# acg-team/ProGraphMSA

Measured on AMD Instinct MI355X. Metric: DP cell-updates/sec (GCUPS) + wall-clock on 256 seqs × 1000 aa, WAG, higher is better.
Workload: dtype f32

## Files before the change

include/pgm_hip.h:

```cpp
#ifndef PGM_HIP_H_
#define PGM_HIP_H_

#include <stdint.h>
#include <stddef.h>

#ifdef __cplusplus
extern "C" {
#endif

#define PGM_OK 0
#define PGM_ERR_INVALID 1
#define PGM_ERR_DEVICE 2
#define PGM_ERR_BACKTRACK 3
#define PGM_ERR_NOMEM 4

#define PGM_GAP 0xFFFFFFFFu


typedef struct pgm_graph {
    uint32_t n;
    uint32_t dim;
    const double *sites;
    const int32_t *e_rowptr;
    const uint32_t *e_col;
    const float *e_val;
    const int32_t *r_rowptr;
    const uint32_t *r_col;
    const uint32_t *r_units;
} pgm_graph;

typedef struct pgm_model {
    const double *M;
    const double *pi;
} pgm_model;

typedef struct pgm_scores {
    float gap_init, gap_extend, match_init, end_match, end_gap, end_skip;
    float start_gap, start_init, repeat_init, repeat_ext;
} pgm_scores;

typedef struct pgm_align_out {
    float score;
    uint32_t n_tr_indels;
    uint32_t len;
    int32_t status;
    uint32_t *map1;
    uint32_t *map2;
} pgm_align_out;

typedef struct pgm_ctx pgm_ctx;
typedef struct pgm_align_batch pgm_align_batch;

int pgm_device_count(void);
int pgm_ctx_create(int device, pgm_ctx **out);
void pgm_ctx_destroy(pgm_ctx *ctx);
const char *pgm_last_error(void);
int pgm_ctx_device_info(pgm_ctx *ctx, char *name, size_t name_len, int *cu_count);

int pgm_align_graphs_batch(pgm_ctx *ctx, uint32_t njobs, const pgm_graph *const *g1,
                           const pgm_graph *const *g2, const pgm_model *const *model,
                           const pgm_scores *scores, pgm_align_out *out);

int pgm_align_batch_create(pgm_ctx *ctx, uint32_t njobs, const pgm_graph *const *g1,
                           const pgm_graph *const *g2, const pgm_model *const *model,
                           const pgm_scores *scores, pgm_align_batch **out);
#define PGM_BATCH_KEEP_MATRICES 1u
int pgm_align_batch_create_ex(pgm_ctx *ctx, uint32_t njobs, const pgm_graph *const *g1,
                              const pgm_graph *const *g2, const pgm_model *const *model,
                              const pgm_scores *scores, uint32_t flags, pgm_align_batch **out);
typedef struct pgm_site_ref {
    const double *dev_sites;
    const uint32_t *node_map;
    uint32_t ncols;
} pgm_site_ref;
int pgm_align_batch_create_res(pgm_ctx *ctx, uint32_t njobs, const pgm_graph *const *g1,
                               const pgm_graph *const *g2, const pgm_model *const *model,
                               const pgm_scores *scores, uint32_t flags, const pgm_site_ref *res1,
                               const pgm_site_ref *res2, pgm_align_batch **out);
int pgm_align_graphs_batch_res(pgm_ctx *ctx, uint32_t njobs, const pgm_graph *const *g1,
                               const pgm_graph *const *g2, const pgm_model *const *model,
                               const pgm_scores *scores, const pgm_site_ref *res1,
                               const pgm_site_ref *res2, pgm_align_out *out);
int pgm_align_batch_run(pgm_ctx *ctx, pgm_align_batch *b);
int pgm_align_batch_fetch(pgm_ctx *ctx, pgm_align_batch *b, pgm_align_out *out);
void pgm_align_batch_destroy(pgm_ctx *ctx, pgm_align_batch *b);
uint64_t pgm_align_batch_cells(const pgm_align_batch *b);
int pgm_align_batch_time(pgm_ctx *ctx, pgm_align_batch *b, int reps, float *ms_prep,
                         float *ms_emission, float *ms_fill, float *ms_traceback);
int pgm_align_batch_stage_times(pgm_align_batch *b, int reset, float *ms_prep, float *ms_emission, float *ms_fill,
                                uint32_t *launches);
int pgm_align_batch_job_times(pgm_ctx *ctx, pgm_align_batch *b, uint64_t *ticks);
int pgm_align_batch_test_stall(pgm_align_batch *b, uint32_t job, uint32_t band, uint32_t spin_limit);
int pgm_test_cu_shares(uint32_t cus, double lean_cost, uint32_t nlean, double band_cost, uint32_t nbands, double rest_cost,
                       uint32_t nrest, uint32_t ncrit, double longest_chain, uint32_t *out4);
#define PGM_PLAN_HEAD 23
#define PGM_PLAN_DHEAD 9
#define PGM_PLAN_JOB 19
int pgm_test_batch_plan(uint32_t njobs, const pgm_graph *const *g1, const pgm_graph *const *g2, const pgm_model *const *model,
                        const pgm_scores *scores, uint32_t flags, const pgm_site_ref *res1, const pgm_site_ref *res2, uint32_t cus,
                        uint32_t *head, double *dhead, uint32_t *job_fields, uint32_t *items, uint32_t *bands, uint32_t *lean_list, int32_t *tblist);
int pgm_align_batch_read_matrices(pgm_ctx *ctx, pgm_align_batch *b, uint32_t job, float *M,
                                  float *X, float *Y, float *W, float *S);

int pgm_nw_pairs_batch(pgm_ctx *ctx, uint32_t dim, const int32_t *score, int32_t gap_open,
                       int32_t gap_extend, uint32_t nseq, const int8_t *syms,
                       const uint32_t *offs, uint32_t npairs, const uint32_t *pi,
                       const uint32_t *pj, int32_t *counts, uint32_t *gaps);
#define PGM_NW_REDUCED 1u
int pgm_nw_pairs_submit(pgm_ctx *ctx, uint32_t dim, const int32_t *score, int32_t gap_open,
                        int32_t gap_extend, uint32_t nseq, const int8_t *syms,
                        const uint32_t *offs, uint32_t npairs, const uint32_t *pi,
                        const uint32_t *pj, uint32_t flags, int32_t *counts, uint32_t *gaps, int *ticket);
int pgm_nw_pairs_wait(pgm_ctx *ctx, int ticket);
float pgm_nw_last_kernel_ms(pgm_ctx *ctx);
void *pgm_host_alloc(size_t bytes);
void pgm_host_free(void *p);

int pgm_csprofile_load(pgm_ctx *ctx, uint32_t K, uint32_t ncols, const double *lprofiles,
                       const double *centre, const double *priors);
int pgm_csprofile_create_batch(pgm_ctx *ctx, uint32_t nseq, const int8_t *syms,
                               const uint32_t *offs, const double *tau, const double *pi,
                               const double *p_uniform, double *out, const uint64_t *out_offs);
int pgm_csprofile_create_batch_res(pgm_ctx *ctx, uint32_t nseq, const int8_t *syms,
                                   const uint32_t *offs, const double *tau, const double *pi,
                                   const double *p_uniform, const double **dev);
float pgm_csprofile_last_kernel_ms(pgm_ctx *ctx);

typedef struct pgm_mldist_model {
    uint32_t dim;
    const double *Q, *V, *Vi, *sigma;
    double dist_max, var_max, var_min, cutoff_dist, min_dist, max_dist, indel_rate;
    int32_t mldist, mldist_gap;
} pgm_mldist_model;
int pgm_mldist_batch(pgm_ctx *ctx, const pgm_mldist_model *model, uint32_t npairs, const int32_t *counts,
                     const uint32_t *gaps, const double *seqlen, double *dist, double *var);

int pgm_prealigned_counts_batch(pgm_ctx *ctx, uint32_t dim, uint32_t nrows, uint32_t ncols, const int8_t *rows,
                                uint32_t npairs, const uint32_t *pi, const uint32_t *pj, int32_t *counts,
                                uint32_t *gaps);
int pgm_kmer_cosine(pgm_ctx *ctx, uint32_t nseq, uint32_t ncols, const int32_t *counts, double *cosine);
int pgm_kmer_cosine_multi(pgm_ctx *ctx, uint32_t nfam, const uint32_t *nseq, uint32_t ncols, const int32_t *counts, double *cosine);
int pgm_prealigned_counts_multi(pgm_ctx *ctx, uint32_t dim, uint32_t nfam, const uint32_t *nrows, const uint32_t *ncols,
                                const int8_t *rows, uint32_t npairs, const uint32_t *fam, const uint32_t *pi, const uint32_t *pj,
                                int32_t *counts, uint32_t *gaps);
int pgm_prealigned_counts_resampled(pgm_ctx *ctx, uint32_t dim, uint32_t nrows, uint32_t ncols, const int8_t *rows, uint32_t nrep,
                                    const uint32_t *cols, uint32_t npairs, const uint32_t *pi, const uint32_t *pj, int32_t *counts,
                                    uint32_t *gaps);
float pgm_dist_last_kernel_ms(pgm_ctx *ctx);

typedef struct pgm_merge_job {
    uint32_t dim, n1, n2, nnodes;
    const double *sites1, *sites2;
    const double *P1, *P2;
    const uint32_t *k1, *k2;
    const uint8_t *g2_with_P1;
    double *profiles;
} pgm_merge_job;
int pgm_merge_profiles_batch(pgm_ctx *ctx, uint32_t njobs, const pgm_merge_job *jobs);
#define PGM_MERGE_RESIDENT 1u
int pgm_merge_profiles_batch_ex(pgm_ctx *ctx, uint32_t njobs, const pgm_merge_job *jobs, uint32_t flags,
                                const double **dev_profiles);
int pgm_resident_reset(pgm_ctx *ctx);
int pgm_resident_onehot(pgm_ctx *ctx, uint32_t dim, uint32_t nseq, const int8_t *syms, const uint32_t *offs,
                        const double **dev);
int pgm_resident_import(pgm_ctx *ctx, pgm_ctx *src_ctx, const double *src, uint64_t count, const double **dst);
float pgm_merge_last_kernel_ms(pgm_ctx *ctx);


typedef struct pgm_gapmask_job {
    const uint64_t *src;
    const uint32_t *mapping;
    uint64_t *dst;
    uint32_t nrows, ncols_in, ncols_out;
} pgm_gapmask_job;
int pgm_gapmask_extend_batch(pgm_ctx *ctx, uint32_t njobs, const pgm_gapmask_job *jobs);

typedef struct pgm_parsimony_job {
    const uint64_t *masks;
    const uint32_t *children;
    uint32_t nleaves, ncols;
} pgm_parsimony_job;
int pgm_gap_parsimony_batch(pgm_ctx *ctx, uint32_t njobs, const pgm_parsimony_job *jobs, uint32_t *scores);
float pgm_parsimony_last_kernel_ms(pgm_ctx *ctx);

#define PGM_WLS_MAX_N 32768
int pgm_wls_load(pgm_ctx *ctx, uint32_t n, const double *D, const double *W);

#define PGM_WLS_OUT 20
typedef struct pgm_wls_job {
    const int8_t *label;
    const double *offset;
    uint32_t nsub;
} pgm_wls_job;
int pgm_wls_pair_sums_batch(pgm_ctx *ctx, uint32_t njobs, const pgm_wls_job *jobs, double *out);
float pgm_wls_last_kernel_ms(pgm_ctx *ctx);
uint32_t pgm_wls_last_launches(pgm_ctx *ctx);

typedef struct pgm_bionj_join { uint32_t index1, index2; double dist1, dist2; } pgm_bionj_join;
#define PGM_BIONJ_MAX_N 32768
int pgm_bionj(pgm_ctx *ctx, uint32_t n, const double *D, const double *V, pgm_bionj_join *joins, double *final_d);
int pgm_bionj_multi(pgm_ctx *ctx, uint32_t nfam, const uint32_t *n, const double *D, const double *V,
                    pgm_bionj_join *joins, double *final_d);
uint32_t pgm_bionj_last_launches(pgm_ctx *ctx);
float pgm_bionj_last_kernel_ms(pgm_ctx *ctx);

typedef struct pgm_bionj_pair { uint32_t index1, index2; } pgm_bionj_pair;
int pgm_bionj_plan(pgm_ctx *ctx, uint32_t n, const double *D, const double *V, const pgm_bionj_pair *plan,
                   pgm_bionj_join *joins, double *final_d);
int pgm_bionj_plan_multi(pgm_ctx *ctx, uint32_t nfam, const uint32_t *n, const double *D, const double *V,
                         const pgm_bionj_pair *plan, pgm_bionj_join *joins, double *final_d);

int pgm_msa_agreement(pgm_ctx *ctx, uint32_t nrows, uint32_t ncols, uint32_t nrep, const int32_t *where,
                      uint32_t *res_hits , uint32_t *pair_hits );
float pgm_agreement_last_kernel_ms(pgm_ctx *ctx);

int pgm_transfer_min(pgm_ctx *ctx, uint32_t nleaves, uint32_t nref, const uint64_t *ref ,
                     uint32_t nrep, const uint32_t *rep_off ,
                     const uint64_t *rep , uint32_t *phi );
float pgm_transfer_last_kernel_ms(pgm_ctx *ctx);

#define PGM_TRANSFER_NONE 0xffffffffu
int pgm_transfer_taxa(pgm_ctx *ctx, uint32_t nleaves, uint32_t nref, const uint64_t *ref , const uint32_t *thr ,
                      uint32_t nrep, const uint32_t *rep_off , const uint64_t *rep ,
                      uint32_t *phi , uint32_t *arg , uint32_t *moved ,
                      uint32_t *counted );

#ifdef __cplusplus
}
#endif
#endif
```

prographmsa_amd/__init__.py:

```python
import ctypes as C
import os

_HERE = os.path.dirname(os.path.abspath(__file__))
LIB_PATH = os.path.join(_HERE, "lib", "libpgm_hip.so")
PGMSA_PATH = os.path.join(_HERE, "bin", "pgmsa")

PGM_OK, PGM_ERR_INVALID, PGM_ERR_DEVICE, PGM_ERR_BACKTRACK, PGM_ERR_NOMEM = 0, 1, 2, 3, 4
PGM_GAP = 0xFFFFFFFF
PGM_BATCH_KEEP_MATRICES = 1
PGM_NW_REDUCED = 1
PGM_MERGE_RESIDENT = 1


class pgm_graph(C.Structure):
    _fields_ = [("n", C.c_uint32), ("dim", C.c_uint32), ("sites", C.POINTER(C.c_double)),
                ("e_rowptr", C.POINTER(C.c_int32)), ("e_col", C.POINTER(C.c_uint32)), ("e_val", C.POINTER(C.c_float)),
                ("r_rowptr", C.POINTER(C.c_int32)), ("r_col", C.POINTER(C.c_uint32)), ("r_units", C.POINTER(C.c_uint32))]


class pgm_model(C.Structure):
    _fields_ = [("M", C.POINTER(C.c_double)), ("pi", C.POINTER(C.c_double))]


class pgm_scores(C.Structure):
    _fields_ = [(n, C.c_float) for n in ("gap_init", "gap_extend", "match_init", "end_match", "end_gap", "end_skip",
                                         "start_gap", "start_init", "repeat_init", "repeat_ext")]


class pgm_mldist_model(C.Structure):
    _fields_ = [("dim", C.c_uint32), ("Q", C.POINTER(C.c_double)), ("V", C.POINTER(C.c_double)), ("Vi", C.POINTER(C.c_double)),
                ("sigma", C.POINTER(C.c_double))] + [(n, C.c_double) for n in ("dist_max", "var_max", "var_min", "cutoff_dist", "min_dist", "max_dist", "indel_rate")] \
        + [("mldist", C.c_int32), ("mldist_gap", C.c_int32)]


class pgm_merge_job(C.Structure):
    _fields_ = [("dim", C.c_uint32), ("n1", C.c_uint32), ("n2", C.c_uint32), ("nnodes", C.c_uint32),
                ("sites1", C.POINTER(C.c_double)), ("sites2", C.POINTER(C.c_double)), ("P1", C.POINTER(C.c_double)), ("P2", C.POINTER(C.c_double)),
                ("k1", C.POINTER(C.c_uint32)), ("k2", C.POINTER(C.c_uint32)), ("g2_with_P1", C.POINTER(C.c_uint8)), ("profiles", C.POINTER(C.c_double))]


class pgm_site_ref(C.Structure):
    _fields_ = [("dev_sites", C.POINTER(C.c_double)), ("node_map", C.POINTER(C.c_uint32)), ("ncols", C.c_uint32)]


class pgm_gapmask_job(C.Structure):
    _fields_ = [("src", C.POINTER(C.c_uint64)), ("mapping", C.POINTER(C.c_uint32)), ("dst", C.POINTER(C.c_uint64)),
                ("nrows", C.c_uint32), ("ncols_in", C.c_uint32), ("ncols_out", C.c_uint32)]


class pgm_parsimony_job(C.Structure):
    _fields_ = [("masks", C.POINTER(C.c_uint64)), ("children", C.POINTER(C.c_uint32)), ("nleaves", C.c_uint32), ("ncols", C.c_uint32)]


class pgm_wls_job(C.Structure):
    _fields_ = [("label", C.POINTER(C.c_int8)), ("offset", C.POINTER(C.c_double)), ("nsub", C.c_uint32)]


class pgm_bionj_join(C.Structure):
    _fields_ = [("index1", C.c_uint32), ("index2", C.c_uint32), ("dist1", C.c_double), ("dist2", C.c_double)]


class pgm_bionj_pair(C.Structure):
    _fields_ = [("index1", C.c_uint32), ("index2", C.c_uint32)]


class pgm_align_out(C.Structure):
    _fields_ = [("score", C.c_float), ("n_tr_indels", C.c_uint32), ("len", C.c_uint32), ("status", C.c_int32),
                ("map1", C.POINTER(C.c_uint32)), ("map2", C.POINTER(C.c_uint32))]


EXPORTS = [
    "pgm_device_count", "pgm_ctx_create", "pgm_ctx_destroy", "pgm_last_error", "pgm_ctx_device_info",
    "pgm_align_graphs_batch", "pgm_align_batch_create", "pgm_align_batch_create_ex", "pgm_align_batch_create_res", "pgm_align_graphs_batch_res", "pgm_align_batch_run", "pgm_align_batch_fetch",
    "pgm_align_batch_destroy", "pgm_align_batch_cells", "pgm_align_batch_test_stall", "pgm_test_cu_shares", "pgm_test_batch_plan", "pgm_align_batch_stage_times", "pgm_align_batch_job_times", "pgm_align_batch_time", "pgm_align_batch_read_matrices",
    "pgm_nw_pairs_batch", "pgm_nw_pairs_submit", "pgm_nw_pairs_wait", "pgm_nw_last_kernel_ms", "pgm_host_alloc", "pgm_host_free", "pgm_csprofile_load", "pgm_csprofile_create_batch", "pgm_csprofile_create_batch_res",
    "pgm_csprofile_last_kernel_ms", "pgm_mldist_batch", "pgm_prealigned_counts_batch", "pgm_kmer_cosine", "pgm_dist_last_kernel_ms",
    "pgm_kmer_cosine_multi", "pgm_prealigned_counts_multi", "pgm_prealigned_counts_resampled",
    "pgm_merge_profiles_batch", "pgm_merge_profiles_batch_ex", "pgm_resident_reset", "pgm_resident_onehot", "pgm_resident_import", "pgm_merge_last_kernel_ms",
    "pgm_gapmask_extend_batch", "pgm_gap_parsimony_batch", "pgm_parsimony_last_kernel_ms",
    "pgm_wls_load", "pgm_wls_pair_sums_batch", "pgm_wls_last_kernel_ms", "pgm_wls_last_launches",
    "pgm_bionj", "pgm_bionj_multi", "pgm_bionj_last_launches", "pgm_bionj_last_kernel_ms",
    "pgm_bionj_plan", "pgm_bionj_plan_multi",
    "pgm_msa_agreement", "pgm_agreement_last_kernel_ms",
    "pgm_transfer_min", "pgm_transfer_last_kernel_ms", "pgm_transfer_taxa",
]


def _load():
    if not os.path.exists(LIB_PATH):
        raise ImportError("libpgm_hip.so is not built (%s); run `python -c 'import __graft_entry__ as g; g.build()'` "
                          "— there is no CPU fallback for the hot path" % LIB_PATH)
    lib = C.CDLL(LIB_PATH)
    vp, u32, i32 = C.c_void_p, C.c_uint32, C.c_int32
    PG, PM = C.POINTER(C.POINTER(pgm_graph)), C.POINTER(C.POINTER(pgm_model))
    sig = {
        "pgm_device_count": (C.c_int, []),
        "pgm_ctx_create": (C.c_int, [C.c_int, C.POINTER(vp)]),
        "pgm_ctx_destroy": (None, [vp]),
        "pgm_last_error": (C.c_char_p, []),
        "pgm_ctx_device_info": (C.c_int, [vp, C.c_char_p, C.c_size_t, C.POINTER(C.c_int)]),
        "pgm_align_graphs_batch": (C.c_int, [vp, u32, PG, PG, PM, C.POINTER(pgm_scores), C.POINTER(pgm_align_out)]),
        "pgm_align_batch_create": (C.c_int, [vp, u32, PG, PG, PM, C.POINTER(pgm_scores), C.POINTER(vp)]),
        "pgm_align_batch_create_ex": (C.c_int, [vp, u32, PG, PG, PM, C.POINTER(pgm_scores), u32, C.POINTER(vp)]),
        "pgm_align_batch_create_res": (C.c_int, [vp, u32, PG, PG, PM, C.POINTER(pgm_scores), u32, C.POINTER(pgm_site_ref), C.POINTER(pgm_site_ref), C.POINTER(vp)]),
        "pgm_align_graphs_batch_res": (C.c_int, [vp, u32, PG, PG, PM, C.POINTER(pgm_scores), C.POINTER(pgm_site_ref), C.POINTER(pgm_site_ref), C.POINTER(pgm_align_out)]),
        "pgm_align_batch_run": (C.c_int, [vp, vp]),
        "pgm_align_batch_fetch": (C.c_int, [vp, vp, C.POINTER(pgm_align_out)]),
        "pgm_align_batch_destroy": (None, [vp, vp]),
        "pgm_align_batch_cells": (C.c_uint64, [vp]),
        "pgm_align_batch_test_stall": (C.c_int, [vp, u32, u32, u32]),
        "pgm_test_cu_shares": (C.c_int, [u32, C.c_double, u32, C.c_double, u32, C.c_double, u32, u32, C.c_double, C.POINTER(C.c_uint32)]),
        "pgm_test_batch_plan": (C.c_int, [u32, PG, PG, PM, C.POINTER(pgm_scores), u32, C.POINTER(pgm_site_ref), C.POINTER(pgm_site_ref), u32,
                                          C.POINTER(u32), C.POINTER(C.c_double)] + [C.POINTER(u32)] * 4 + [C.POINTER(i32)]),
        "pgm_align_batch_stage_times": (C.c_int, [vp, C.c_int] + [C.POINTER(C.c_float)] * 3 + [C.POINTER(u32)]),
        "pgm_align_batch_job_times": (C.c_int, [vp, vp, C.POINTER(C.c_uint64)]),
        "pgm_align_batch_time": (C.c_int, [vp, vp, C.c_int] + [C.POINTER(C.c_float)] * 4),
        "pgm_align_batch_read_matrices": (C.c_int, [vp, vp, u32] + [C.POINTER(C.c_float)] * 5),
        "pgm_nw_pairs_batch": (C.c_int, [vp, u32, C.POINTER(i32), i32, i32, u32, C.POINTER(C.c_int8), C.POINTER(u32), u32,
                                         C.POINTER(u32), C.POINTER(u32), C.POINTER(i32), C.POINTER(u32)]),
        "pgm_nw_pairs_submit": (C.c_int, [vp, u32, C.POINTER(i32), i32, i32, u32, C.POINTER(C.c_int8), C.POINTER(u32), u32,
                                          C.POINTER(u32), C.POINTER(u32), u32, C.POINTER(i32), C.POINTER(u32), C.POINTER(C.c_int)]),
        "pgm_nw_pairs_wait": (C.c_int, [vp, C.c_int]),
        "pgm_host_alloc": (vp, [C.c_size_t]),
        "pgm_host_free": (None, [vp]),
        "pgm_nw_last_kernel_ms": (C.c_float, [vp]),
        "pgm_csprofile_load": (C.c_int, [vp, u32, u32] + [C.POINTER(C.c_double)] * 3),
        "pgm_csprofile_create_batch": (C.c_int, [vp, u32, C.POINTER(C.c_int8), C.POINTER(u32)] + [C.POINTER(C.c_double)] * 4
                                       + [C.POINTER(C.c_uint64)]),
        "pgm_csprofile_create_batch_res": (C.c_int, [vp, u32, C.POINTER(C.c_int8), C.POINTER(u32)] + [C.POINTER(C.c_double)] * 3
                                           + [C.POINTER(C.POINTER(C.c_double))]),
        "pgm_csprofile_last_kernel_ms": (C.c_float, [vp]),
        "pgm_mldist_batch": (C.c_int, [vp, C.POINTER(pgm_mldist_model), u32, C.POINTER(i32), C.POINTER(u32)] + [C.POINTER(C.c_double)] * 3),
        "pgm_prealigned_counts_batch": (C.c_int, [vp, u32, u32, u32, C.POINTER(C.c_int8), u32, C.POINTER(u32), C.POINTER(u32), C.POINTER(i32), C.POINTER(u32)]),
        "pgm_kmer_cosine": (C.c_int, [vp, u32, u32, C.POINTER(i32), C.POINTER(C.c_double)]),
        "pgm_dist_last_kernel_ms": (C.c_float, [vp]),
        "pgm_kmer_cosine_multi": (C.c_int, [vp, u32, C.POINTER(u32), u32, C.POINTER(i32), C.POINTER(C.c_double)]),
        "pgm_prealigned_counts_multi": (C.c_int, [vp, u32, u32, C.POINTER(u32), C.POINTER(u32), C.POINTER(C.c_int8), u32, C.POINTER(u32), C.POINTER(u32),
                                                  C.POINTER(u32), C.POINTER(i32), C.POINTER(u32)]),
        "pgm_prealigned_counts_resampled": (C.c_int, [vp, u32, u32, u32, C.POINTER(C.c_int8), u32, C.POINTER(u32), u32, C.POINTER(u32), C.POINTER(u32),
                                                      C.POINTER(i32), C.POINTER(u32)]),
        "pgm_merge_profiles_batch": (C.c_int, [vp, u32, C.POINTER(pgm_merge_job)]),
        "pgm_merge_profiles_batch_ex": (C.c_int, [vp, u32, C.POINTER(pgm_merge_job), u32, C.POINTER(C.POINTER(C.c_double))]),
        "pgm_resident_reset": (C.c_int, [vp]),
        "pgm_resident_onehot": (C.c_int, [vp, u32, u32, C.POINTER(C.c_int8), C.POINTER(u32), C.POINTER(C.POINTER(C.c_double))]),
        "pgm_resident_import": (C.c_int, [vp, vp, C.POINTER(C.c_double), C.c_uint64, C.POINTER(C.POINTER(C.c_double))]),
        "pgm_merge_last_kernel_ms": (C.c_float, [vp]),
        "pgm_gapmask_extend_batch": (C.c_int, [vp, u32, C.POINTER(pgm_gapmask_job)]),
        "pgm_gap_parsimony_batch": (C.c_int, [vp, u32, C.POINTER(pgm_parsimony_job), C.POINTER(u32)]),
        "pgm_parsimony_last_kernel_ms": (C.c_float, [vp]),
        "pgm_wls_load": (C.c_int, [vp, u32, C.POINTER(C.c_double), C.POINTER(C.c_double)]),
        "pgm_wls_pair_sums_batch": (C.c_int, [vp, u32, C.POINTER(pgm_wls_job), C.POINTER(C.c_double)]),
        "pgm_wls_last_kernel_ms": (C.c_float, [vp]),
        "pgm_wls_last_launches": (C.c_uint32, [vp]),
        "pgm_bionj": (C.c_int, [vp, u32, C.POINTER(C.c_double), C.POINTER(C.c_double), C.POINTER(pgm_bionj_join), C.POINTER(C.c_double)]),
        "pgm_bionj_multi": (C.c_int, [vp, u32, C.POINTER(u32), C.POINTER(C.c_double), C.POINTER(C.c_double), C.POINTER(pgm_bionj_join), C.POINTER(C.c_double)]),
        "pgm_bionj_last_launches": (C.c_uint32, [vp]),
        "pgm_bionj_last_kernel_ms": (C.c_float, [vp]),
        "pgm_bionj_plan": (C.c_int, [vp, u32, C.POINTER(C.c_double), C.POINTER(C.c_double), C.POINTER(pgm_bionj_pair), C.POINTER(pgm_bionj_join), C.POINTER(C.c_double)]),
        "pgm_bionj_plan_multi": (C.c_int, [vp, u32, C.POINTER(u32), C.POINTER(C.c_double), C.POINTER(C.c_double), C.POINTER(pgm_bionj_pair), C.POINTER(pgm_bionj_join), C.POINTER(C.c_double)]),
        "pgm_msa_agreement": (C.c_int, [vp, u32, u32, u32, C.POINTER(i32), C.POINTER(u32), C.POINTER(u32)]),
        "pgm_agreement_last_kernel_ms": (C.c_float, [vp]),
        "pgm_transfer_min": (C.c_int, [vp, u32, u32, C.POINTER(C.c_uint64), u32, C.POINTER(u32), C.POINTER(C.c_uint64), C.POINTER(u32)]),
        "pgm_transfer_last_kernel_ms": (C.c_float, [vp]),
        "pgm_transfer_taxa": (C.c_int, [vp, u32, u32, C.POINTER(C.c_uint64), C.POINTER(u32), u32, C.POINTER(u32), C.POINTER(C.c_uint64),
                                        C.POINTER(u32), C.POINTER(u32), C.POINTER(u32), C.POINTER(u32)]),
    }
    for name, (res, args) in sig.items():
        fn = getattr(lib, name)
        fn.restype = res
        fn.argtypes = args
    return lib


lib = _load()


class PgmError(RuntimeError):
    pass


def check(rc, what="libpgm_hip"):
    if rc != PGM_OK:
        raise PgmError("%s failed (%d): %s" % (what, rc, lib.pgm_last_error().decode()))


class Context:

    def __init__(self, device=0):
        self.handle = C.c_void_p()
        check(lib.pgm_ctx_create(device, C.byref(self.handle)), "pgm_ctx_create")

    def device_info(self):
        buf = C.create_string_buffer(256)
        cu = C.c_int()
        check(lib.pgm_ctx_device_info(self.handle, buf, 256, C.byref(cu)))
        return buf.value.decode(), cu.value

    def prealigned_counts_resampled(self, dim, rows, cols, pi, pj):
        import numpy as np
        rows = np.ascontiguousarray(rows, np.int8)
        cols = np.ascontiguousarray(cols, np.uint32)
        pi = np.ascontiguousarray(pi, np.uint32)
        pj = np.ascontiguousarray(pj, np.uint32)
        nrep, npairs = cols.shape[0], len(pi)
        counts = np.zeros((nrep, npairs, dim * dim), np.int32)
        gaps = np.zeros((nrep, npairs), np.uint32)
        P = lambda a, t: a.ctypes.data_as(C.POINTER(t))
        check(lib.pgm_prealigned_counts_resampled(self.handle, dim, rows.shape[0], rows.shape[1], P(rows, C.c_int8), nrep, P(cols, C.c_uint32), npairs,
                                                  P(pi, C.c_uint32), P(pj, C.c_uint32), P(counts, C.c_int32), P(gaps, C.c_uint32)), "pgm_prealigned_counts_resampled")
        return counts, gaps

    def msa_agreement(self, where, res_hits=None, pair_hits=None):
        import numpy as np
        where = np.ascontiguousarray(where, np.int32)
        nrep, nrows, ncols = where.shape
        if res_hits is None: res_hits = np.zeros((nrows, ncols), np.uint32)
        if pair_hits is None: pair_hits = np.zeros((nrows, nrows), np.uint32)
        for o, shape in ((res_hits, (nrows, ncols)), (pair_hits, (nrows, nrows))):
            if o.dtype != np.uint32 or o.shape != shape or not o.flags.c_contiguous: raise ValueError("msa_agreement: output array of the wrong kind")
        P = lambda a, t: a.ctypes.data_as(C.POINTER(t))
        check(lib.pgm_msa_agreement(self.handle, nrows, ncols, nrep, P(where, C.c_int32), P(res_hits, C.c_uint32), P(pair_hits, C.c_uint32)), "pgm_msa_agreement")
        return res_hits, pair_hits

    def transfer_min(self, nleaves, ref, rep_off, rep, phi=None):
        import numpy as np
        words = (nleaves + 63) // 64
        ref = np.ascontiguousarray(ref, np.uint64)
        rep_off = np.ascontiguousarray(rep_off, np.uint32)
        rep = np.ascontiguousarray(rep, np.uint64).reshape(-1, words)
        if ref.ndim != 2 or ref.shape[1] != words or rep_off.ndim != 1 or len(rep_off) < 1 or rep.shape[0] != int(rep_off[-1]):
            raise ValueError("transfer_min: input array of the wrong shape")
        nref, nrep = ref.shape[0], len(rep_off) - 1
        if phi is None: phi = np.zeros((nref, nrep), np.uint32)
        if phi.dtype != np.uint32 or phi.shape != (nref, nrep) or not phi.flags.c_contiguous: raise ValueError("transfer_min: output array of the wrong kind")
        P = lambda a, t: a.ctypes.data_as(C.POINTER(t))
        check(lib.pgm_transfer_min(self.handle, nleaves, nref, P(ref, C.c_uint64), nrep, P(rep_off, C.c_uint32), P(rep, C.c_uint64) if rep.size else None,
                                   P(phi, C.c_uint32)), "pgm_transfer_min")
        return phi

    def transfer_taxa(self, nleaves, ref, thr, rep_off, rep, out=None):
        import numpy as np
        words = (nleaves + 63) // 64
        ref = np.ascontiguousarray(ref, np.uint64)
        thr = np.ascontiguousarray(thr, np.uint32)
        rep_off = np.ascontiguousarray(rep_off, np.uint32)
        rep = np.ascontiguousarray(rep, np.uint64).reshape(-1, words)
        if ref.ndim != 2 or ref.shape[1] != words or thr.shape != (ref.shape[0],) or rep_off.ndim != 1 or len(rep_off) < 1 or rep.shape[0] != int(rep_off[-1]):
            raise ValueError("transfer_taxa: input array of the wrong shape")
        nref, nrep = ref.shape[0], len(rep_off) - 1
        shapes = [(nref, nrep), (nref, nrep), (nref, nleaves), (nref,)]
        if out is None: out = tuple(np.zeros(s, np.uint32) for s in shapes)
        if len(out) != 4 or any(a.dtype != np.uint32 or a.shape != s or not a.flags.c_contiguous for a, s in zip(out, shapes)):
            raise ValueError("transfer_taxa: output array of the wrong kind")
        P = lambda a, t: a.ctypes.data_as(C.POINTER(t))
        check(lib.pgm_transfer_taxa(self.handle, nleaves, nref, P(ref, C.c_uint64), P(thr, C.c_uint32), nrep, P(rep_off, C.c_uint32),
                                    P(rep, C.c_uint64) if rep.size else None, *[P(a, C.c_uint32) for a in out]), "pgm_transfer_taxa")
        return tuple(out)

    def close(self):
        if self.handle:
            lib.pgm_ctx_destroy(self.handle)
            self.handle = C.c_void_p()

    def __del__(self):
        try:
            self.close()
        except Exception:
            pass
```

prographmsa_amd/csrc/pgm_align_kernels.h:

```cpp
#ifndef PGM_ALIGN_KERNELS_H_
#define PGM_ALIGN_KERNELS_H_

#include <hip/hip_runtime.h>
#include <math.h>
#include <type_traits>
#include "pgm_device.h"

#define PGM_NEG_INF (-INFINITY)

__device__ __forceinline__ float pgm_ls_log_add(float x, float add) {
    const float a = 2.44247459618085927548717403238913328776812604856113966238617812902399112761292613763080658235564f;
    const float b = -4.2040783745848554315883301529007786406310628696382695994938550046831869207082846248658671f;
    const float c = -0.72123729809042963774358701619456664388406302428056983119308906451199556380646306f;
    const uint32_t bits = __float_as_uint(x);
    const float e = (float)((int32_t)(bits >> 23) - 126);
    const float d = __uint_as_float(((bits << 9) >> 9) ^ 0x3f000000u);
    float t = __fdiv_rn(b, __fsub_rn(d, c));
    const float u = __fadd_rn(e, a);
    t = __fadd_rn(t, add);
    t = __fadd_rn(t, u);
    return t;
}

__device__ __forceinline__ float pgm_emission_finish(float num, float ay, float bx, float match_init) {
    float q = __fdiv_rn(num, __fmul_rn(ay, bx));
    if (q != q) q = __uint_as_float(0xFFC00000u);
    return pgm_ls_log_add(q, match_init);
}

template <int DMAX, int NODES>
__global__ void __launch_bounds__(NODES) pgm_prep_kernel(const PgmJob *__restrict__ jobs, int *__restrict__ sync, uint32_t sync_ints) {
    extern __shared__ float prep_lds[];
    {
        const uint32_t nthreads = gridDim.x * gridDim.y * gridDim.z * NODES;
        const uint32_t gid = ((blockIdx.z * gridDim.y + blockIdx.y) * gridDim.x + blockIdx.x) * NODES + threadIdx.x;
        for (uint32_t i = gid; i < sync_ints; i += nthreads) sync[i] = 0;
    }
    const PgmJob &J = jobs[blockIdx.x];
    const bool first = blockIdx.y == 0;
    const uint32_t n = first ? J.n1 : J.n2;
    const uint32_t v0 = blockIdx.z * NODES;
    if (v0 >= n) return;
    if (J.tabhdr && J.tabhdr[0] == 0) {
        const uint32_t nc = J.dim + 2u;
        bool any = n - 1u >= v0 && n - 1u < v0 + (uint32_t)NODES;
        for (uint32_t c = 0; c < nc; ++c) {
            const uint32_t r = (uint32_t)J.tabhdr[1u + (first ? 0u : nc) + c];
            any = any || (r != 0u && r - 1u >= v0 && r - 1u < v0 + (uint32_t)NODES);
        }
        if (!any) return;
    }
    const uint32_t D = J.dim, DP = J.dp, ST = D + 1;
    float *Mf = prep_lds;
    float *pif = prep_lds + D * D;
    float *nl = pif + D;
    const uint32_t nn = min((uint32_t)NODES, n - v0);
    {
        const int32_t *pp = first ? J.pp1 : J.pp2;
        const uint32_t *pc = first ? J.pc1 : J.pc2, *pu = first ? J.pu1 : J.pu2;
        const float *pv = first ? J.pv1 : J.pv2;
        PgmTbNode *rec = (first ? J.tb1 : J.tb2) + v0;
        for (uint32_t i = threadIdx.x; i < nn * PGM_TB_PK; i += NODES) {
            const uint32_t node = i / PGM_TB_PK, k = i % PGM_TB_PK;
            const int32_t eb = pp[v0 + node];
            const uint32_t cnt = (uint32_t)(pp[v0 + node + 1] - eb);
            const int32_t e = cnt == 0u ? 0 : eb + (int32_t)min(k, cnt - 1u);
            if (k == 0) rec[node].cnt = cnt;
            rec[node].c[k] = pc[e]; rec[node].v[k] = pv[e]; rec[node].u[k] = pu[e];
        }
    }
    if (!first) for (uint32_t i = threadIdx.x; i < D * D; i += NODES) Mf[i] = (float)J.M[i];
    for (uint32_t i = threadIdx.x; i < D; i += NODES) pif[i] = (float)J.pi[i];
    const double *sites = first ? J.sites1 : J.sites2;
    const uint32_t *smap = first ? J.smap1 : J.smap2;
    float *dst = (first ? J.g1f : J.t2) + (size_t)DP * v0;
    for (uint32_t i = threadIdx.x; i < nn * D; i += NODES) {
        const uint32_t node = v0 + i / D;
        const float g = (float)sites[(size_t)D * (smap ? smap[node] : node) + i % D];
        nl[(i / D) * ST + (i % D)] = g;
        if (first && DP == D) dst[i] = g;
    }
    __syncthreads();
    const uint32_t v = threadIdx.x;
    float g[DMAX];
    float acc = 0.0f;
    if (v < nn) {
#pragma unroll
        for (int k = 0; k < DMAX; ++k) g[k] = ((uint32_t)k < D) ? nl[v * ST + k] : 0.0f;
        float l0 = 0.0f, l1 = 0.0f, l2 = 0.0f, l3 = 0.0f;
        const uint32_t aligned = D / 4u * 4u;
#pragma unroll
        for (int k = 0; k + 3 < DMAX; k += 4) {
            if ((uint32_t)k < aligned) {
                l0 = __fadd_rn(l0, __fmul_rn(g[k], pif[k]));
                l1 = __fadd_rn(l1, __fmul_rn(g[k + 1], pif[k + 1]));
                l2 = __fadd_rn(l2, __fmul_rn(g[k + 2], pif[k + 2]));
                l3 = __fadd_rn(l3, __fmul_rn(g[k + 3], pif[k + 3]));
            }
        }
        acc = __fadd_rn(0.0f, __fadd_rn(__fadd_rn(l0, l2), __fadd_rn(l1, l3)));
#pragma unroll
        for (int k = 0; k < DMAX; ++k)
            if ((uint32_t)k >= aligned && (uint32_t)k < D) acc = __fadd_rn(acc, __fmul_rn(g[k], pif[k]));
        (first ? J.a1 : J.b2)[v0 + v] = acc;
    }
    if (first) {
        if (DP != D && v < nn) {
#pragma unroll
            for (int k = 0; k < DMAX; ++k) if ((uint32_t)k < DP) dst[(size_t)DP * v + k] = g[k];
        }
        return;
    }
    __syncthreads();
    if (v < nn) {
        for (uint32_t k = 0; k < D; ++k) {
            float t = 0.0f;
#pragma unroll
            for (int j = 0; j < DMAX; ++j)
                if ((uint32_t)j < D) t = __fadd_rn(t, __fmul_rn(Mf[j + D * k], g[j]));
            nl[v * ST + k] = t;
        }
    }
    __syncthreads();
    for (uint32_t i = threadIdx.x; i < nn * DP; i += NODES) {
        const uint32_t node = i / DP, k = i % DP;
        dst[i] = k < D ? nl[node * ST + k] : 0.0f;
    }
}

#define PGM_TAB_HDR 136
__global__ void __launch_bounds__(256) pgm_classify_kernel(const PgmJob *__restrict__ jobs) {
    const PgmJob &J = jobs[blockIdx.x];
    if (!J.tabhdr) return;
    const bool first = blockIdx.y == 0;
    const uint32_t n = first ? J.n1 : J.n2, D = J.dim;
    const double *sites = first ? J.sites1 : J.sites2;
    const uint32_t *smap = first ? J.smap1 : J.smap2;
    uint8_t *cls = (uint8_t *)(first ? J.cls1 : J.cls2);
    const float uni = (float)(1.0 / (double)D);
    for (uint32_t v = blockIdx.z * blockDim.x + threadIdx.x; v < n; v += gridDim.z * blockDim.x) {
        const double *col = sites + (size_t)D * (smap ? smap[v] : v);
        uint32_t nz = 0, sym = 0;
        bool same = true;
        float vs = 0.f;
        const float g0 = (float)col[0];
        for (uint32_t k = 0; k < D; ++k) {
            const float g = (float)col[k];
            if (g != 0.0f) { ++nz; sym = k; vs = g; }
            same = same && g == g0;
        }
        uint32_t c = 255u;
        if (nz == 0u) c = D + 1u;
        else if (nz == 1u && vs == 1.0f) c = sym;
        else if (same && g0 == uni) c = D;
        cls[v] = (uint8_t)c;
        if (c == 255u) atomicOr(J.tabhdr, 1);
        else atomicCAS(J.tabhdr + 1 + (first ? 0u : D + 2u) + c, 0, (int)v + 1);
    }
}

__device__ __forceinline__ size_t pgm_cell_index(const PgmJob &J, uint32_t y, uint32_t x) {
    const uint32_t b = y / PGM_ROWS, l = PGM_HALO + (y - b * PGM_ROWS);
    return ((size_t)b * J.tsteps + (x + l)) * 64u + l;
}
__device__ __forceinline__ float4 pgm_load_cell(const PgmJob &J, uint32_t y, uint32_t x) {
    return J.cells[pgm_cell_index(J, y, x)];
}

__device__ __forceinline__ float pgm_dpp_wave_shr1(float src, float lane0_value) {
    return __int_as_float(__builtin_amdgcn_update_dpp(__float_as_int(lane0_value), __float_as_int(src), 0x138, 0xf, 0xf, false));
}

#define PGM_GLOBAL __attribute__((address_space(1)))
typedef float pgm_v4f __attribute__((ext_vector_type(4)));
template <class T> __device__ __forceinline__ T pgm_gld(const T *p) { return *(const PGM_GLOBAL T *)(uintptr_t)p; }
#define PGM_EM_TB 4
template <int DP, int RB>
__global__ void __launch_bounds__(4 * PGM_ROWS) pgm_emission_skew_kernel(const PgmJob *__restrict__ jobs) {
    typedef float pgm_v2f __attribute__((ext_vector_type(2)));
    constexpr int NT = DP / 4;
    constexpr int COLS = 64 + PGM_EM_TB * PGM_BLOCK - PGM_HALO - 1;
    constexpr int STR = DP + 1;
    __shared__ pgm_v2f tp[(COLS + 1) * STR];
    __shared__ float bq[COLS];
    const PgmJob &J = jobs[blockIdx.z];
    const uint32_t tb0 = blockIdx.x * PGM_EM_TB;
    const uint32_t rsh = J.rshift, nvb = J.nb << rsh;
    if (tb0 >= J.nblk || 4u * RB * blockIdx.y >= nvb) return;
    if (J.tabhdr && pgm_gld(J.tabhdr) == 0) return;
    auto row_of = [&](uint32_t v, uint32_t lane_) { return ((((v >> rsh) << 6) + lane_) << rsh) | (v & ((1u << rsh) - 1u)); };
    auto sblock_of = [&](uint32_t v, uint32_t tb_) { return ((((size_t)(v >> rsh) * J.nblk + tb_) << rsh) | (v & ((1u << rsh) - 1u))); };
    const uint32_t t0 = tb0 * PGM_BLOCK;
    const int cbase = (int)t0 - 63;
    if ((DP == 20 || DP == 4) && RB == 1) {
        constexpr int TE = DP + 1;
        float *const tab = (float *)tp;
        static_assert(COLS * TE <= (COLS + 1) * STR * 2, "score table must fit the column staging area");
        static_assert(DP > 20 || TE <= 32, "row classes must fit As");
        __shared__ float As[32];
        const uint32_t fb0 = 4u * blockIdx.y + threadIdx.x / PGM_ROWS;
        const uint32_t fl = threadIdx.x % PGM_ROWS;
        const bool active = fb0 < nvb;
        int sym = DP;
        bool plain = true;
        float a_row = 0.f;
        if (active) {
            const uint32_t y = row_of(fb0, fl);
            const uint32_t yc = (y + 1 < J.n1) ? y : 0u;
            const float4 *src = (const float4 *)(J.g1f + (size_t)DP * yc);
            int nz = 0;
#pragma unroll
            for (int q = 0; q < NT; ++q) {
                const float4 v = src[q];
                const float vv[4] = {v.x, v.y, v.z, v.w};
#pragma unroll
                for (int u = 0; u < 4; ++u)
                    if (vv[u] != 0.0f) { ++nz; sym = 4 * q + u; plain = plain && vv[u] == 1.0f; }
            }
            plain = plain && nz <= 1;
            a_row = J.a1[yc];
        }
        if (threadIdx.x < 32) As[threadIdx.x] = 0.f;
        if (__syncthreads_and(plain ? 1 : 0)) {
            if (active) As[sym] = a_row;
            __syncthreads();
            const float mi = J.sc.match_init;
            constexpr int NE = (COLS * TE + 4 * PGM_ROWS - 1) / (4 * PGM_ROWS);
            float tt[NE], tb2[NE];
#pragma unroll
            for (int e = 0; e < NE; ++e) {
                const int i = (int)threadIdx.x + e * 4 * PGM_ROWS;
                const int ci = i / TE, k = i % TE, c = cbase + ci;
                const bool in = i < COLS * TE && c >= 0 && c <= (int)J.ncol;
                tb2[e] = in ? J.b2[c] : 0.f;
                tt[e] = (in && k < DP) ? J.t2[(size_t)DP * c + k] : 0.f;
            }
#pragma unroll
            for (int e = 0; e < NE; ++e) {
                const int i = (int)threadIdx.x + e * 4 * PGM_ROWS;
                if (i < COLS * TE) tab[i] = pgm_emission_finish(0.0f + tt[e], As[i % TE], tb2[e], mi);
            }
            __syncthreads();
            if (!active) return;
            PGM_GLOBAL pgm_v4f *const Sq = (PGM_GLOBAL pgm_v4f *)(uintptr_t)J.S;
            const int l = PGM_HALO + (int)fl;
#pragma unroll 1
            for (int w = 0; w < PGM_EM_TB; ++w) {
                const uint32_t tb = tb0 + w;
                if (tb >= J.nblk) break;
                float out[PGM_BLOCK];
#pragma unroll
                for (int i = 0; i < PGM_BLOCK; ++i) out[i] = tab[((int)(tb * PGM_BLOCK) + i - l - cbase) * TE + sym];
                PGM_GLOBAL pgm_v4f *dst = Sq + (sblock_of(fb0, tb) * 64u + (uint32_t)l) * (PGM_BLOCK / 4);
#pragma unroll
                for (int q = 0; q < PGM_BLOCK / 4; ++q) dst[q] = pgm_v4f{out[4 * q], out[4 * q + 1], out[4 * q + 2], out[4 * q + 3]};
            }
            return;
        }
    }
    const float4 *t2q = (const float4 *)J.t2;
    float *tpf = (float *)tp;
    for (int i = threadIdx.x; i < (COLS + 1) * NT; i += 4 * PGM_ROWS) {
        const int ci = i / NT, q = i % NT, c = cbase + ci;
        float4 v = make_float4(0.f, 0.f, 0.f, 0.f);
        if (c >= 0 && c <= (int)J.ncol) v = t2q[(size_t)NT * c + q];
        const float vv[4] = {v.x, v.y, v.z, v.w};
#pragma unroll
        for (int u = 0; u < 4; ++u) {
            const int k = 4 * q + u;
            if (ci < COLS) tpf[2 * (ci * STR + k)] = vv[u];
            if (ci > 0) tpf[2 * ((ci - 1) * STR + k) + 1] = vv[u];
        }
    }
    for (int i = threadIdx.x; i < COLS; i += 4 * PGM_ROWS) {
        const int col = cbase + i;
        bq[i] = (col >= 0 && col <= (int)J.ncol) ? J.b2[col] : 0.f;
    }
    __syncthreads();
    const uint32_t b0 = (4u * blockIdx.y + threadIdx.x / PGM_ROWS) * RB;
    const int l = PGM_HALO + (int)(threadIdx.x % PGM_ROWS);
    if (b0 >= nvb) return;
    float gy[RB][DP], ay[RB];
#pragma unroll
    for (int r = 0; r < RB; ++r) {
        const uint32_t y = row_of(b0 + (uint32_t)r, (uint32_t)(l - PGM_HALO));
        const uint32_t yc = (y + 1 < J.n1) ? y : 0u;
        const float4 *src = (const float4 *)(J.g1f + (size_t)DP * yc);
#pragma unroll
        for (int q = 0; q < NT; ++q) {
            const float4 v = src[q];
            gy[r][4 * q] = v.x; gy[r][4 * q + 1] = v.y; gy[r][4 * q + 2] = v.z; gy[r][4 * q + 3] = v.w;
        }
        ay[r] = J.a1[yc];
    }
    const float mi = J.sc.match_init;
    const uint32_t nblk = J.nblk;
    PGM_GLOBAL pgm_v4f *const Sq = (PGM_GLOBAL pgm_v4f *)(uintptr_t)J.S;
#pragma unroll 1
    for (int w = 0; w < PGM_EM_TB; ++w) {
        const uint32_t tb = tb0 + w;
        if (tb >= nblk) break;
        float out[RB][PGM_BLOCK];
#pragma unroll
        for (int i = 0; i < PGM_BLOCK; i += 2) {
            const int ci = (int)(tb * PGM_BLOCK) + i - l - cbase;
            const pgm_v2f *tc = tp + ci * STR;
            pgm_v2f acc[RB];
#pragma unroll
            for (int r = 0; r < RB; ++r) acc[r] = pgm_v2f{0.0f, 0.0f};
#pragma unroll
            for (int k = 0; k < DP; ++k) {
                const pgm_v2f tk = tc[k];
#pragma unroll
                for (int r = 0; r < RB; ++r) {
                    const pgm_v2f g = {gy[r][k], gy[r][k]};
                    acc[r] = acc[r] + g * tk;
                }
            }
#pragma unroll
            for (int r = 0; r < RB; ++r) {
                out[r][i] = pgm_emission_finish(acc[r].x, ay[r], bq[ci], mi);
                out[r][i + 1] = pgm_emission_finish(acc[r].y, ay[r], bq[ci + 1], mi);
            }
        }
#pragma unroll
        for (int r = 0; r < RB; ++r) {
            if (b0 + (uint32_t)r < nvb) {
                PGM_GLOBAL pgm_v4f *dst = Sq + (sblock_of(b0 + (uint32_t)r, tb) * 64u + (uint32_t)l) * (PGM_BLOCK / 4);
#pragma unroll
                for (int q = 0; q < PGM_BLOCK / 4; ++q) dst[q] = pgm_v4f{out[r][4 * q], out[r][4 * q + 1], out[r][4 * q + 2], out[r][4 * q + 3]};
            }
        }
    }
}

__device__ __forceinline__ int pgm_wave_max8(uint32_t v) {
    int m = __builtin_amdgcn_ballot_w64(v >= 8u) != 0 ? 8 : 0;
    m += __builtin_amdgcn_ballot_w64(v >= (uint32_t)(m + 4)) != 0 ? 4 : 0;
    m += __builtin_amdgcn_ballot_w64(v >= (uint32_t)(m + 2)) != 0 ? 2 : 0;
    m += __builtin_amdgcn_ballot_w64(v >= (uint32_t)(m + 1)) != 0 ? 1 : 0;
    return m;
}

__device__ __forceinline__ __amdgpu_buffer_rsrc_t pgm_band_rsrc(float4 *base, uint32_t bytes) {
    const uint64_t p = (uint64_t)base;
    const uint32_t lo = __builtin_amdgcn_readfirstlane((uint32_t)p), hi = __builtin_amdgcn_readfirstlane((uint32_t)(p >> 32));
    return __builtin_amdgcn_make_buffer_rsrc((void *)(((uint64_t)hi << 32) | lo), 0, __builtin_amdgcn_readfirstlane(bytes), 0x00020000);
}
__device__ __forceinline__ void pgm_store_cell_masked(__amdgpu_buffer_rsrc_t rsrc, uint32_t t, int lane, bool on, float Mv, float Xv, float Wv, float Yv) {
    typedef uint32_t pgm_v4u __attribute__((ext_vector_type(4)));
    pgm_v4u v;
    v.x = __float_as_uint(Mv); v.y = __float_as_uint(Xv); v.z = __float_as_uint(Wv); v.w = __float_as_uint(Yv);
    __builtin_amdgcn_raw_buffer_store_b128(v, rsrc, (on ? (uint32_t)lane * 16u : 0x80000000u) + t * 1024u, 0, 16);
}
__device__ __forceinline__ float4 pgm_gload4(const float4 *p) {
    const pgm_v4f v = *(const PGM_GLOBAL pgm_v4f *)(uintptr_t)p;
    return make_float4(v.x, v.y, v.z, v.w);
}
__device__ __forceinline__ float2 pgm_gload_cell_wy(const float4 *p) {
    const unsigned long long v = __hip_atomic_load((const PGM_GLOBAL unsigned long long *)(uintptr_t)p + 1, __ATOMIC_RELAXED, __HIP_MEMORY_SCOPE_AGENT);
    return make_float2(__uint_as_float((uint32_t)v), __uint_as_float((uint32_t)(v >> 32)));
}
__device__ __forceinline__ float2 pgm_load_cell_mx(const float4 *p) {
    const unsigned long long v = __hip_atomic_load((const PGM_GLOBAL unsigned long long *)(uintptr_t)p, __ATOMIC_RELAXED, __HIP_MEMORY_SCOPE_AGENT);
    return make_float2(__uint_as_float((uint32_t)v), __uint_as_float((uint32_t)(v >> 32)));
}
__device__ __forceinline__ float2 pgm_load_cell_wy(const float4 *p) {
    const unsigned long long v = __hip_atomic_load((const PGM_GLOBAL unsigned long long *)(uintptr_t)p + 1, __ATOMIC_RELAXED, __HIP_MEMORY_SCOPE_AGENT);
    return make_float2(__uint_as_float((uint32_t)v), __uint_as_float((uint32_t)(v >> 32)));
}

struct PgmPred {
    const int32_t *pp; const uint32_t *pc; const float *pv; const uint32_t *pu;
};
__device__ __forceinline__ float pgm_mark_value(const PgmPred &P, int32_t e) {
    const uint32_t u = P.pu[e];
    if (u == 0) return P.pv[e];
    const uint32_t units = u & 0x7fffffffu;
    if (units == 0) return INFINITY;
    return __fadd_rn(INFINITY, __fmul_rn(INFINITY, (float)(units - 1)));
}

struct PgmMapOut {
    uint32_t *m1, *m2;
    uint32_t len, cap;
    __device__ __forceinline__ void push(uint32_t y, uint32_t x) {
        if (len < cap) { m1[len] = y; m2[len] = x; }
        ++len;
    }
};

__device__ static void pgm_mark_alternative_path(const PgmJob &J, uint32_t start, uint32_t end, const PgmPred &P, PgmMapOut &mo, bool first) {
    const uint32_t len = end - start + 1;
    float *score = J.mark_score;
    uint32_t *prev = J.mark_prev;
    for (uint32_t i = 0; i < len; ++i) { score[i] = PGM_NEG_INF; prev[i] = 0xFFFFFFFFu; }
    score[0] = 0.0f;
    for (uint32_t i = 1; i < len; ++i) {
        const uint32_t real_ix = i + start;
        for (int32_t e = P.pp[real_ix]; e < P.pp[real_ix + 1]; ++e) {
            const uint32_t p = P.pc[e];
            if (p >= start && p <= end) {
                const uint32_t i2 = p - start;
                const float cand = __fsub_rn(score[i2], pgm_mark_value(P, e));
                if (score[i] <= cand) { score[i] = cand; prev[i] = i2; }
            }
        }
    }
    if (score[len - 1] > PGM_NEG_INF) {
        uint32_t i = prev[len - 1];
        while (i != 0) {
            if (first) mo.push(i + start, 0xFFFFFFFFu); else mo.push(0xFFFFFFFFu, i + start);
            i = prev[i];
        }
    }
}

__device__ __forceinline__ float pgm_emission_at(const PgmJob &J, uint32_t y, uint32_t x) {
    const uint32_t b = y / PGM_ROWS, l = PGM_HALO + (y - b * PGM_ROWS), t = x + l;
    return J.S[(((size_t)b * J.nblk + (t / PGM_BLOCK)) * 64u + l) * PGM_BLOCK + (t % PGM_BLOCK)];
}

#define PGM_TB_T 32
#define PGM_TB_BAND 6
#define PGM_TB_LK 4
struct PgmTbLds {
    float4 cell[PGM_TB_T * PGM_TB_T];
    float S[PGM_TB_T * PGM_TB_T];
    uint32_t p_cnt[2 * PGM_TB_T];
    uint32_t p_c[2 * PGM_TB_T * PGM_TB_PK];
    float p_v[2 * PGM_TB_T * PGM_TB_PK];
    uint32_t p_u[2 * PGM_TB_T * PGM_TB_PK];
    uint16_t succ[3 * PGM_TB_T * PGM_TB_T];
    uint32_t ty0, tx0;
    uint32_t ay, ax;
    int req;
    uint32_t len;
    int nbig;
    uint16_t big[128];
    uint16_t gtab[PGM_LK_NR][PGM_LK_W * PGM_LK_TAB] __attribute__((aligned(16)));
    uint2 mbuf[64];
    uint32_t grow, gcnt;
    uint32_t gnext[PGM_LK_NR];
};

#define PGM_LK_HW (PGM_LK_T + PGM_LK_H)
struct PgmLkLds {
    float4 cell[PGM_LK_HW * PGM_LK_HW];
    float S[PGM_LK_T * PGM_LK_T];
    uint32_t p_cnt[2 * PGM_LK_T];
    uint32_t p_c[2 * PGM_LK_T * PGM_TB_PK];
    float p_v[2 * PGM_LK_T * PGM_TB_PK];
    uint32_t p_u[2 * PGM_LK_T * PGM_TB_PK];
    uint16_t tab[PGM_LK_TAB] __attribute__((aligned(16)));
    int nbig;
    uint16_t big[PGM_LK_T * PGM_LK_T];
};
__device__ __forceinline__ uint16_t pgm_lk_code(uint32_t st, uint32_t dy, uint32_t dx) { return (uint16_t)(0x8000u | (st << 12) | (dy << 6) | dx); }

struct PgmPredView {
    uint32_t cnt;
    bool lds;
    uint32_t base;
};

__device__ static void pgm_traceback_publish(const PgmJob &J, const uint32_t len, const int tid, const int nthreads) {
    for (uint32_t i = (uint32_t)tid; i < len; i += (uint32_t)nthreads) {
        const uint32_t j = len - 1 - i;
        J.hmap1[i] = J.map1[j];
        J.hmap2[i] = J.map2[j];
    }
    __threadfence_system();
    __syncthreads();
    if (tid == 0) {
        const PgmJob::Result r = *J.result;
        J.hresult->score = r.score; J.hresult->n_tr_indels = r.n_tr_indels; J.hresult->len = r.len;
        __threadfence_system();
        __hip_atomic_store(&J.hresult->status, r.status, __ATOMIC_RELEASE, __HIP_MEMORY_SCOPE_SYSTEM);
    }
}

__device__ __attribute__((noinline)) static void pgm_traceback_job(const PgmJob &J, PgmTbLds &T, const int tid, const int nthreads,
                                         int *lq, int *lq_ids, const uint32_t jid) {
    constexpr uint32_t TT = PGM_TB_T;
    const uint32_t n1 = J.n1, n2 = J.n2;

    const PgmPred P1 = {J.pp1, J.pc1, J.pv1, J.pu1};
    const PgmPred P2 = {J.pp2, J.pc2, J.pv2, J.pu2};

    const bool loader = tid >= 64;
    auto stage = [&]() {
        const uint32_t ty0 = T.ty0, tx0 = T.tx0;
        constexpr uint32_t NT = 64u * PGM_WAVES;
        constexpr int NC = (int)((TT * TT) / NT), NP = (int)((2 * TT * PGM_TB_PK) / NT);
        static_assert(NC * NT == TT * TT && NP * NT == 2 * TT * PGM_TB_PK, "tile staging: whole rounds of the workgroup");
        float4 cv[NC];
        float sv[NC];
        uint32_t cslot[NC];
#pragma unroll
        for (int u = 0; u < NC; ++u) {
            const uint32_t i = (uint32_t)tid + NT * u;
            const uint32_t half = TT * (TT + 1u) / 2u;
            const bool up = i < half;
            const uint32_t m = up ? i : TT * TT - 1u - i;
            uint32_t d = (uint32_t)((sqrtf(8.0f * (float)m + 1.0f) - 1.0f) * 0.5f);
            while (d * (d + 1u) / 2u > m) --d;
            while ((d + 1u) * (d + 2u) / 2u <= m) ++d;
            const uint32_t k = m - d * (d + 1u) / 2u;
            const uint32_t ly = up ? k : TT - 1u - k, lx = up ? d - k : TT - 1u - (d - k);
            cslot[u] = ly * TT + lx;
            const uint32_t yy = min(ty0 + ly, n1 - 2), xx = min(tx0 + lx, n2 - 2);
            cv[u] = J.cells[pgm_cell_index(J, yy, xx)];
            const uint32_t ys = min(ty0 + i / TT, n1 - 2), xs = min(tx0 + i % TT, n2 - 2);
            sv[u] = pgm_emission_at(J, ys, xs);
        }
        uint32_t cnt[NP], ec[NP], eu[NP];
        float ev[NP];
#pragma unroll
        for (int u = 0; u < NP; ++u) {
            const uint32_t i = (uint32_t)tid + NT * u, slot = i / PGM_TB_PK, k = i % PGM_TB_PK;
            const bool row = slot < TT;
            const uint32_t v = min(row ? ty0 + slot : tx0 + (slot - TT), (row ? n1 : n2) - 1);
            const PgmTbNode *r = (row ? J.tb1 : J.tb2) + v;
            cnt[u] = r->cnt; ec[u] = r->c[k]; ev[u] = r->v[k]; eu[u] = r->u[k];
        }
#pragma unroll
        for (int u = 0; u < NC; ++u) {
            const uint32_t i = (uint32_t)tid + NT * u;
            T.cell[cslot[u]] = cv[u];
            T.S[i] = sv[u];
        }
        for (uint32_t i = (uint32_t)tid; i < 3u * TT * TT / 2u; i += NT) ((uint32_t *)T.succ)[i] = 0u;
        if (tid == 0) T.nbig = 0;
#pragma unroll
        for (int u = 0; u < NP; ++u) {
            const uint32_t i = (uint32_t)tid + NT * u, slot = i / PGM_TB_PK, k = i % PGM_TB_PK;
            const bool row = slot < TT;
            const bool inr = (row ? ty0 + slot : tx0 + (slot - TT)) < (row ? n1 : n2);
            if (k == 0) T.p_cnt[slot] = inr ? cnt[u] : 0xFFFFFFFFu;
            T.p_c[i] = ec[u]; T.p_v[i] = ev[u]; T.p_u[i] = eu[u];
        }
    };
    const pgm_scores sc = J.sc;
    const int band = J.has_extras ? PGM_TB_BAND : PGM_TB_BAND / 2;
    auto links = [&]() {
        const uint32_t ty0 = T.ty0, tx0 = T.tx0;
        const int adiag = (int)(T.ay - ty0) - (int)(T.ax - tx0);
        const uint32_t NDIAG = 2u * (uint32_t)band + 1u;
        for (uint32_t task = (uint32_t)tid; task < 3u * NDIAG * TT; task += (uint32_t)nthreads) {
            const uint32_t lx = task % TT, st_task = task / (NDIAG * TT);
            const int lyi = (int)lx + adiag + (int)((task / TT) % NDIAG) - band;
            if (lyi < 0 || lyi >= (int)TT) continue;
            const uint32_t ly = (uint32_t)lyi, ci = ly * TT + lx, y = ty0 + ly, x = tx0 + lx;
            uint16_t lm = 0, lxs = 0, lys = 0;
            if (y + 1 < n1 && x + 1 < n2 && (y | x) != 0u) {
                const float4 c0 = T.cell[ci];
                const uint32_t cy = T.p_cnt[ly], cx = T.p_cnt[TT + lx];
                auto pick = [&](const float4 &c, uint32_t yp, uint32_t xp) -> uint16_t {
                    uint32_t st;
                    if ((yp | xp) == 0u) st = 0u;
                    else if (c.z == c.x) st = 0u;
                    else if (c.z == c.w) st = 2u;
                    else if (c.z == c.y) st = 1u;
                    else return (uint16_t)0;
                    return (uint16_t)(0x8000u | (st << 10) | ((yp - ty0) << 5) | (xp - tx0));
                };
                const int doff = (int)((task / TT) % NDIAG) - band;
                if (st_task == 0u && doff >= -1 && doff <= 1 && (cy > PGM_TB_LK || cx > PGM_TB_LK) && cy <= PGM_TB_PK && cx <= PGM_TB_PK && cy != 0u && cx != 0u && c0.x > PGM_NEG_INF) {
                    const int slot = __hip_atomic_fetch_add(&T.nbig, 1, __ATOMIC_RELAXED, __HIP_MEMORY_SCOPE_WORKGROUP);
                    if (slot < 128) T.big[slot] = (uint16_t)ci;
                }
                if (st_task == 0u && cy <= PGM_TB_LK && cx <= PGM_TB_LK && cy != 0u && cx != 0u && c0.x > PGM_NEG_INF) {
                    const float S = T.S[ci];
                    uint32_t yp[PGM_TB_LK], xp[PGM_TB_LK];
                    float yv[PGM_TB_LK], xv[PGM_TB_LK];
                    bool ok = true;
#pragma unroll
                    for (int k = 0; k < PGM_TB_LK; ++k) {
                        yp[k] = T.p_c[ly * PGM_TB_PK + k]; yv[k] = T.p_v[ly * PGM_TB_PK + k];
                        xp[k] = T.p_c[(TT + lx) * PGM_TB_PK + k]; xv[k] = T.p_v[(TT + lx) * PGM_TB_PK + k];
                        ok = ok && ((uint32_t)k >= cy || yp[k] >= ty0) && ((uint32_t)k >= cx || xp[k] >= tx0);
                    }
                    float wz[PGM_TB_LK][PGM_TB_LK];
#pragma unroll
                    for (int ky = 0; ky < PGM_TB_LK; ++ky)
#pragma unroll
                        for (int kx = 0; kx < PGM_TB_LK; ++kx)
                            wz[ky][kx] = T.cell[min((yp[ky] - ty0) * TT + (xp[kx] - tx0), TT * TT - 1u)].z;
                    float best = INFINITY;
                    uint32_t wy = 0, wx = 0, wky = 0, wkx = 0;
#pragma unroll
                    for (int ky = 0; ky < PGM_TB_LK; ++ky)
#pragma unroll
                        for (int kx = 0; kx < PGM_TB_LK; ++kx) {
                            const float d = fabsf(__fsub_rn(c0.x, __fsub_rn(__fsub_rn(__fadd_rn(wz[ky][kx], S), yv[ky]), xv[kx])));
                            if ((uint32_t)ky < cy && (uint32_t)kx < cx && best > d) { best = d; wy = yp[ky]; wx = xp[kx]; wky = ky; wkx = kx; }
                        }
                    bool rep_edge = false;
                    float4 wc = c0;
                    if (ok && best < INFINITY) {
                        rep_edge = (T.p_u[ly * PGM_TB_PK + wky] | T.p_u[(TT + lx) * PGM_TB_PK + wkx]) != 0u;
                        wc = T.cell[(wy - ty0) * TT + (wx - tx0)];
                    }
                    if (ok && best < INFINITY && !rep_edge) lm = pick(wc, wy, wx);
                }
                if (st_task == 2u && cy == 1u && c0.w > PGM_NEG_INF) {
                    float best = INFINITY;
                    bool ok = true, rep_edge = false, open = false;
                    uint32_t wy = 0;
                    float4 wc = c0;
                    for (uint32_t k = 0; k < cy; ++k) {
                        const uint32_t yp = T.p_c[ly * PGM_TB_PK + k];
                        if (yp < ty0) { ok = false; break; }
                        const float yv = T.p_v[ly * PGM_TB_PK + k];
                        const float4 c = T.cell[(yp - ty0) * TT + lx];
                        const bool ru = T.p_u[ly * PGM_TB_PK + k] != 0u;
                        float d = fabsf(__fsub_rn(c0.w, __fsub_rn(__fadd_rn(c.w, sc.gap_extend), yv)));
                        if (best > d) { best = d; wy = yp; wc = c; rep_edge = ru; open = false; }
                        d = fabsf(__fsub_rn(c0.w, __fsub_rn(__fadd_rn(c.z, sc.gap_init), yv)));
                        if (best > d) { best = d; wy = yp; wc = c; rep_edge = ru; open = true; }
                    }
                    if (ok && best < INFINITY && !rep_edge)
                        lys = open ? pick(wc, wy, x) : (uint16_t)(0x8000u | (2u << 10) | ((wy - ty0) << 5) | lx);
                }
                if (st_task == 1u && cx == 1u && c0.y > PGM_NEG_INF) {
                    float best = INFINITY;
                    bool ok = true, rep_edge = false, open = false;
                    uint32_t wx = 0;
                    float4 wc = c0;
                    for (uint32_t k = 0; k < cx; ++k) {
                        const uint32_t xp = T.p_c[(TT + lx) * PGM_TB_PK + k];
                        if (xp < tx0) { ok = false; break; }
                        const float xv = T.p_v[(TT + lx) * PGM_TB_PK + k];
                        const float4 c = T.cell[ly * TT + (xp - tx0)];
                        const bool ru = T.p_u[(TT + lx) * PGM_TB_PK + k] != 0u;
// ... 1960 lines not shown
```

prographmsa_amd/csrc/pgm_capi.hip:

```cpp
#include <hip/hip_runtime.h>

#include <algorithm>
#include <cmath>
#include <cstdio>
#include <thread>
#include <atomic>
#include <chrono>
#include <queue>
#include <cstdlib>
#include <cstring>
#include <numeric>
#include <mutex>
#include <string>
#include <unordered_set>
#include <vector>
#include <sys/mman.h>

#include "pgm_align_kernels.h"
#include "pgm_crit_kernels.h"
#include "pgm_nw_kernels.h"
#include "pgm_csprofile_kernels.h"
#include "pgm_dist_kernels.h"
#include "pgm_merge_kernels.h"
#include "pgm_parsimony_kernels.h"
#include "pgm_wls_kernels.h"
#include "pgm_bionj_kernels.h"
#include "pgm_agreement_kernels.h"
#include "pgm_transfer_kernels.h"
#include "pgm_pool.h"
#include "pgm_plan.h"
static_assert(kC3Bytes == PGM_C3_BYTES, "pgm_plan.h plans the LDS of a crit3 sweep with PGM_C3_BYTES");

static thread_local std::string g_err;
static int fail(int code, const std::string &m) { g_err = m; return code; }
#define HIPCHK(x)                                                                                   \
    do {                                                                                            \
        hipError_t e_ = (x);                                                                        \
        if (e_ != hipSuccess)                                                                       \
            return fail(PGM_ERR_DEVICE, std::string(#x) + ": " + hipGetErrorString(e_));            \
    } while (0)

struct PgmNwState;
struct pgm_ctx {
    int device = 0;
    PgmNwState *nw = nullptr;
    int nw_per_cu = 0;
    struct ResChunk { uint8_t *p; size_t cap; };
    std::vector<ResChunk> res_chunks;
    size_t res_chunk = 0, res_off = 0;
    hipStream_t stream = nullptr;
    hipStream_t stream2 = nullptr;
    hipStream_t stream3 = nullptr;
    hipStream_t stream4 = nullptr;
    enum { C_IN, C_WORK, C_CELLS, C_OUT, C_S, C_HOST, C_HIN, C_SMALL, C_SLOTS };
    void *cache_ptr[C_SLOTS] = {};
    size_t cache_bytes[C_SLOTS] = {};
    hipDeviceProp_t prop;
    float nw_ms = 0, cs_ms = 0, ml_ms = 0, merge_ms = 0, pars_ms = 0, wls_ms = 0;
    uint32_t wls_n = 0, wls_launches = 0;
    float bionj_ms = 0;
    float agree_ms = 0;
    float transfer_ms = 0;
    uint32_t bionj_launches = 0;
    enum { SC_DEV = 36, SC_HOST = 4 };
    void *sc_dev[SC_DEV] = {};
    size_t sc_dev_bytes[SC_DEV] = {};
    void *sc_host[SC_HOST] = {};
    size_t sc_host_bytes[SC_HOST] = {};
    hipEvent_t sc_ev[2] = {nullptr, nullptr};
    uint32_t csK = 0, csC = 0;
    double *cs_lprofiles = nullptr, *cs_centre = nullptr, *cs_priors = nullptr;
};

static pgm_pool::Pool &lib_pool() {
    static pgm_pool::Pool pool(std::max(1u, std::min(16u, std::thread::hardware_concurrency())));
    return pool;
}

static std::mutex g_pinned_mu;
static std::unordered_set<void *> g_pinned_registered;
static hipError_t pinned_alloc(size_t bytes, void **out) {
    const size_t H = (size_t)2 << 20, len = (std::max<size_t>(bytes, 1) + H - 1) / H * H;
    void *p = getenv("PGM_PINNED_MALLOC") ? nullptr : aligned_alloc(H, len);
    if (p) {
        (void)madvise(p, len, MADV_HUGEPAGE);
        (void)lib_pool().run(len / H, len >= 8 * H ? 16u : 1u, [&](size_t c) { for (size_t o = 0; o < H; o += 4096) ((volatile char *)p)[c * H + o] = 0; });
        if (hipHostRegister(p, len, hipHostRegisterDefault) == hipSuccess) {
            std::lock_guard<std::mutex> g(g_pinned_mu);
            g_pinned_registered.insert(p);
            *out = p;
            return hipSuccess;
        }
        (void)hipGetLastError();
        free(p);
    }
    return hipHostMalloc(out, bytes, hipHostMallocDefault);
}
static void pinned_free(void *p) {
    if (!p) return;
    bool reg;
    { std::lock_guard<std::mutex> g(g_pinned_mu); reg = g_pinned_registered.erase(p) != 0; }
    if (reg) { (void)hipHostUnregister(p); free(p); }
    else (void)hipHostFree(p);
}
static void slot_free(int slot, void *p) {
    if (slot == pgm_ctx::C_HIN) pinned_free(p);
    else if (slot == pgm_ctx::C_HOST) (void)hipHostFree(p);
    else (void)hipFree(p);
}

struct pgm_align_batch {
    uint32_t njobs = 0;
    uint64_t cells = 0;
    uint32_t maxdim = 0, maxnb = 0, maxn = 0, maxnblk = 0;
    std::vector<PgmJob> jobs;
    std::vector<uint32_t> order;
    BatchSchedule sched;
    uint8_t *d_in = nullptr;
    uint8_t *d_work = nullptr;
    uint8_t *d_cells = nullptr;
    uint8_t *d_out = nullptr;
    uint8_t *d_S = nullptr;
    uint8_t *d_small = nullptr;
    size_t in_bytes = 0, work_bytes = 0, cell_bytes = 0, out_bytes = 0, s_bytes = 0, small_bytes = 0;
    size_t cap[8] = {0, 0, 0, 0, 0, 0, 0, 0};
    uint8_t *h_out = nullptr;
    uint8_t *h_in = nullptr;
    int *h_flag = nullptr;
    int *d_sync = nullptr;
    size_t sync_ints = 0;
    uint32_t lq_off = 0;
    PgmJob *d_jobs = nullptr;
    uint32_t *d_order = nullptr;
    PgmItem *d_items = nullptr;
    uint32_t *d_lean = nullptr;
    PgmItem *d_bands = nullptr;
    int2 *d_tblist = nullptr;
    unsigned long long *d_times = nullptr;
    int *d_tabhdr = nullptr;
    hipEvent_t ev_fork = nullptr, ev_join = nullptr;
    hipEvent_t ev_join_b = nullptr, ev_join_c = nullptr;
    uint32_t test_spin_limit = 0, test_stall_job = 0xFFFFFFFFu, test_stall_band = 0;
    double acc_ms[3] = {0, 0, 0};
    uint32_t acc_n = 0;
    bool ev_pending = false;
    std::vector<size_t> res_off, map1_off, map2_off;
    hipEvent_t ev[5] = {nullptr, nullptr, nullptr, nullptr, nullptr};
};
static const struct BatchBuffer { int slot; size_t reserve_mb; uint8_t *pgm_align_batch::*ptr; size_t pgm_align_batch::*bytes; } kBatchBuffers[6] = {
    {pgm_ctx::C_IN, 128, &pgm_align_batch::d_in, &pgm_align_batch::in_bytes}, {pgm_ctx::C_WORK, 256, &pgm_align_batch::d_work, &pgm_align_batch::work_bytes},
    {pgm_ctx::C_CELLS, 2048, &pgm_align_batch::d_cells, &pgm_align_batch::cell_bytes}, {pgm_ctx::C_OUT, 8, &pgm_align_batch::d_out, &pgm_align_batch::out_bytes},
    {pgm_ctx::C_S, 1024, &pgm_align_batch::d_S, &pgm_align_batch::s_bytes}, {pgm_ctx::C_SMALL, 4, &pgm_align_batch::d_small, &pgm_align_batch::small_bytes}};

extern "C" {

const char *pgm_last_error(void) { return g_err.c_str(); }

int pgm_device_count(void) {
    int n = 0;
    if (hipGetDeviceCount(&n) != hipSuccess) return 0;
    return n;
}

__global__ void pgm_warm_kernel() {}

int pgm_ctx_create(int device, pgm_ctx **out) {
    if (!out) return fail(PGM_ERR_INVALID, "null out");
    *out = nullptr;
    int n = 0;
    HIPCHK(hipGetDeviceCount(&n));
    if (device < 0 || device >= n) return fail(PGM_ERR_DEVICE, "no such HIP device");
    HIPCHK(hipSetDevice(device));
    pgm_ctx *c = new pgm_ctx;
    c->device = device;
    HIPCHK(hipGetDeviceProperties(&c->prop, device));
    HIPCHK(hipStreamCreateWithFlags(&c->stream, hipStreamNonBlocking));
    HIPCHK(hipStreamCreateWithFlags(&c->stream2, hipStreamNonBlocking));
    HIPCHK(hipStreamCreateWithFlags(&c->stream3, hipStreamNonBlocking));
    {
        int lo = 0, hi = 0;
        if (hipDeviceGetStreamPriorityRange(&lo, &hi) != hipSuccess) { (void)hipGetLastError(); lo = hi = 0; }
        if (hipStreamCreateWithPriority(&c->stream4, hipStreamNonBlocking, hi) != hipSuccess) {
            (void)hipGetLastError();
            HIPCHK(hipStreamCreateWithFlags(&c->stream4, hipStreamNonBlocking));
        }
    }
    hipLaunchKernelGGL(pgm_warm_kernel, dim3(1), dim3(64), 0, c->stream);
    HIPCHK(hipGetLastError());
    HIPCHK(hipStreamSynchronize(c->stream));
    {
        void *h = nullptr, *d = nullptr;
        const size_t wb = (size_t)1 << 20;
        if (hipHostMalloc(&h, wb, hipHostMallocDefault) == hipSuccess && hipMalloc(&d, wb) == hipSuccess) {
            (void)hipMemcpyAsync(d, h, wb, hipMemcpyHostToDevice, c->stream);
            (void)hipMemcpyAsync(h, d, wb, hipMemcpyDeviceToHost, c->stream);
            (void)hipStreamSynchronize(c->stream);
        }
        if (h) (void)hipHostFree(h);
        if (d) (void)hipFree(d);
    }
    (void)lib_pool().run(64, 16u, [](size_t) {});
    {
        void *p = nullptr;
        const size_t sb = (size_t)128 << 20;
        if (!getenv("PGM_NO_STAGING_RESERVE") && pinned_alloc(sb, &p) == hipSuccess) { c->cache_ptr[pgm_ctx::C_HIN] = p; c->cache_bytes[pgm_ctx::C_HIN] = sb; }
        else (void)hipGetLastError();
        const size_t rb = (size_t)8 << 20;
        if (!getenv("PGM_NO_STAGING_RESERVE") && hipHostMalloc(&p, rb, hipHostMallocDefault) == hipSuccess) { c->cache_ptr[pgm_ctx::C_HOST] = p; c->cache_bytes[pgm_ctx::C_HOST] = rb; }
        else (void)hipGetLastError();
        if (!getenv("PGM_NO_STAGING_RESERVE") && !getenv("PGM_NO_DEVICE_RESERVE")) {
            for (const BatchBuffer &e : kBatchBuffers) {
                void *d = nullptr;
                if (hipMalloc(&d, e.reserve_mb << 20) == hipSuccess) { c->cache_ptr[e.slot] = d; c->cache_bytes[e.slot] = e.reserve_mb << 20; }
                else { (void)hipGetLastError(); break; }
            }
        }
    }
    *out = c;
    return PGM_OK;
}

static void nw_state_free(PgmNwState *st);
void pgm_ctx_destroy(pgm_ctx *ctx) {
    if (!ctx) return;
    (void)hipSetDevice(ctx->device);
    nw_state_free(ctx->nw);
    for (auto &c : ctx->res_chunks) if (c.p) (void)hipFree(c.p);
    if (ctx->cs_lprofiles) (void)hipFree(ctx->cs_lprofiles);
    if (ctx->cs_centre) (void)hipFree(ctx->cs_centre);
    if (ctx->cs_priors) (void)hipFree(ctx->cs_priors);
    for (int k = 0; k < pgm_ctx::SC_DEV; ++k) if (ctx->sc_dev[k]) (void)hipFree(ctx->sc_dev[k]);
    for (int k = 0; k < pgm_ctx::SC_HOST; ++k) if (ctx->sc_host[k]) pinned_free(ctx->sc_host[k]);
    for (int k = 0; k < 2; ++k) if (ctx->sc_ev[k]) (void)hipEventDestroy(ctx->sc_ev[k]);
    for (int k = 0; k < pgm_ctx::C_SLOTS; ++k)
        if (ctx->cache_ptr[k]) slot_free(k, ctx->cache_ptr[k]);
    if (ctx->stream4) (void)hipStreamDestroy(ctx->stream4);
    if (ctx->stream3) (void)hipStreamDestroy(ctx->stream3);
    if (ctx->stream2) (void)hipStreamDestroy(ctx->stream2);
    if (ctx->stream) (void)hipStreamDestroy(ctx->stream);
    delete ctx;
}

int pgm_ctx_device_info(pgm_ctx *ctx, char *name, size_t name_len, int *cu_count) {
    if (!ctx) return fail(PGM_ERR_INVALID, "null ctx");
    if (name && name_len) snprintf(name, name_len, "%s (%s)", ctx->prop.name, ctx->prop.gcnArchName);
    if (cu_count) *cu_count = ctx->prop.multiProcessorCount;
    return PGM_OK;
}

}

namespace {
static hipError_t cache_take(pgm_ctx *ctx, int slot, size_t bytes, void **out, size_t *got) {
    if (ctx->cache_ptr[slot] && ctx->cache_bytes[slot] >= bytes) {
        *out = ctx->cache_ptr[slot]; *got = ctx->cache_bytes[slot];
        ctx->cache_ptr[slot] = nullptr; ctx->cache_bytes[slot] = 0;
        return hipSuccess;
    }
    if (ctx->cache_ptr[slot]) {
        slot_free(slot, ctx->cache_ptr[slot]);
        ctx->cache_ptr[slot] = nullptr; ctx->cache_bytes[slot] = 0;
    }
    *got = bytes;
    if (slot == pgm_ctx::C_HIN) return pinned_alloc(bytes, out);
    return slot == pgm_ctx::C_HOST ? hipHostMalloc(out, bytes, hipHostMallocDefault) : hipMalloc(out, bytes);
}
static void cache_give(pgm_ctx *ctx, int slot, void *p, size_t bytes) {
    if (!p) return;
    if (ctx && (!ctx->cache_ptr[slot] || ctx->cache_bytes[slot] < bytes)) {
        if (ctx->cache_ptr[slot]) slot_free(slot, ctx->cache_ptr[slot]);
        ctx->cache_ptr[slot] = p; ctx->cache_bytes[slot] = bytes;
    } else {
        slot_free(slot, p);
    }
}

static hipError_t scratch_dev(pgm_ctx *ctx, int slot, size_t bytes, void **out) {
    bytes = std::max<size_t>(bytes, 16);
    if (ctx->sc_dev_bytes[slot] < bytes) {
        if (ctx->sc_dev[slot]) (void)hipFree(ctx->sc_dev[slot]);
        ctx->sc_dev[slot] = nullptr; ctx->sc_dev_bytes[slot] = 0;
        const size_t want = bytes + bytes / 4;
        hipError_t e = hipMalloc(&ctx->sc_dev[slot], want);
        if (e != hipSuccess) return e;
        ctx->sc_dev_bytes[slot] = want;
    }
    *out = ctx->sc_dev[slot];
    return hipSuccess;
}
static hipError_t scratch_host(pgm_ctx *ctx, int slot, size_t bytes, void **out) {
    bytes = std::max<size_t>(bytes, 16);
    if (ctx->sc_host_bytes[slot] < bytes) {
        if (ctx->sc_host[slot]) pinned_free(ctx->sc_host[slot]);
        ctx->sc_host[slot] = nullptr; ctx->sc_host_bytes[slot] = 0;
        const size_t want = bytes + bytes / 4;
        hipError_t e = pinned_alloc(want, &ctx->sc_host[slot]);
        if (e != hipSuccess) return e;
        ctx->sc_host_bytes[slot] = want;
    }
    *out = ctx->sc_host[slot];
    return hipSuccess;
}
static hipError_t scratch_events(pgm_ctx *ctx) {
    for (int k = 0; k < 2; ++k)
        if (!ctx->sc_ev[k]) { hipError_t e = hipEventCreate(&ctx->sc_ev[k]); if (e != hipSuccess) return e; }
    return hipSuccess;
}

static hipError_t classify_lean_jobs(pgm_ctx *ctx, pgm_align_batch *b) {
    if (!b->d_tabhdr || b->njobs == 0) return hipSuccess;
    hipError_t e = hipMemsetAsync(b->d_tabhdr, 0, 4 * (size_t)PGM_TAB_HDR * b->njobs, ctx->stream);
    if (e != hipSuccess) return e;
    hipLaunchKernelGGL(pgm_classify_kernel, dim3(b->njobs, 2, (b->maxn + 1023) / 1024), dim3(256), 0, ctx->stream, b->d_jobs);
    return hipGetLastError();
}

#define PGM_STATUS_PENDING 0x7ffffff0
struct PrepTier { uint32_t tier, threads; size_t lds; };
static PrepTier prep_tier(uint32_t maxdim) {
    const uint32_t tier = alphabet_tier(maxdim), threads = tier == 64u ? 64u : 256u;
    return {tier, threads, ((size_t)maxdim * maxdim + maxdim + threads * ((size_t)maxdim + 1)) * sizeof(float)};
}
static hipError_t launch_all(pgm_ctx *ctx, pgm_align_batch *b, bool timed) {
    hipStream_t s = ctx->stream;
    const BatchSchedule &S = b->sched;
    hipError_t e;
    for (uint32_t i = 0; i < b->njobs; ++i) ((PgmJob::Result *)(b->h_out + b->res_off[i]))->status = PGM_STATUS_PENDING;
    if (timed && (e = hipEventRecord(b->ev[0], s)) != hipSuccess) return e;
    const PrepTier T = prep_tier(b->maxdim);
    const dim3 pg(b->njobs, 2, (b->maxn + T.threads - 1) / T.threads);
    if (T.tier == 4) hipLaunchKernelGGL((pgm_prep_kernel<4, 256>), pg, dim3(256), T.lds, s, b->d_jobs, b->d_sync, (uint32_t)b->sync_ints);
    else if (T.tier == 20) hipLaunchKernelGGL((pgm_prep_kernel<20, 256>), pg, dim3(256), T.lds, s, b->d_jobs, b->d_sync, (uint32_t)b->sync_ints);
    else hipLaunchKernelGGL((pgm_prep_kernel<64, 64>), pg, dim3(64), T.lds, s, b->d_jobs, b->d_sync, (uint32_t)b->sync_ints);
    if ((e = hipGetLastError()) != hipSuccess) return e;
    if (timed && (e = hipEventRecord(b->ev[1], s)) != hipSuccess) return e;
    const dim3 eg((b->maxnblk + PGM_EM_TB - 1) / PGM_EM_TB, (b->maxnb + 3) / 4, b->njobs);
    if (T.tier == 4) hipLaunchKernelGGL((pgm_emission_skew_kernel<4, 1>), eg, dim3(4 * PGM_ROWS), 0, s, b->d_jobs);
    else if (T.tier == 20) hipLaunchKernelGGL((pgm_emission_skew_kernel<20, 1>), eg, dim3(4 * PGM_ROWS), 0, s, b->d_jobs);
    else hipLaunchKernelGGL((pgm_emission_skew_kernel<64, 1>), eg, dim3(4 * PGM_ROWS), 0, s, b->d_jobs);
    if ((e = hipGetLastError()) != hipSuccess) return e;
    if (timed && (e = hipEventRecord(b->ev[2], s)) != hipSuccess) return e;
    const uint32_t spin_limit = b->test_spin_limit ? b->test_spin_limit : PGM_SPIN_LIMIT, stall_job = b->test_stall_job, stall_band = b->test_stall_band;
    const bool fork = S.nlean != 0;
    const bool bandk = S.nbands != 0;
    const bool tbk = (S.nitems != 0 || bandk) && (S.ntb + S.ntb_c + S.ntb_b) != 0;
    const bool critk = S.ncrit != 0;
    if ((fork || bandk || critk) && (e = hipEventRecord(b->ev_fork, s)) != hipSuccess) return e;
    if (critk && (e = hipStreamWaitEvent(ctx->stream4, b->ev_fork, 0)) != hipSuccess) return e;
    if (fork && (e = hipStreamWaitEvent(ctx->stream2, b->ev_fork, 0)) != hipSuccess) return e;
    if (bandk && (e = hipStreamWaitEvent(ctx->stream3, b->ev_fork, 0)) != hipSuccess) return e;
    const uint32_t nrest = S.nitems - S.ncrit;
    hipStream_t sc = critk ? s : ctx->stream4, sr = critk ? ctx->stream4 : s;
    auto sweep = [&](hipStream_t st, uint32_t workers, const PgmItem *list, uint32_t n, bool c3, uint32_t ticket_off) {
        if (c3) hipLaunchKernelGGL(pgm_crit_kernel, dim3(workers), dim3(64 * PGM_C3_WAVES), 0, st, b->d_jobs, list, n, b->d_sync, spin_limit, stall_job, stall_band, ticket_off);
        else hipLaunchKernelGGL(pgm_fill_kernel, dim3(workers), dim3(64 * PGM_WAVES), 0, st, b->d_jobs, list, n, b->d_sync, spin_limit, stall_job, stall_band, ticket_off);
    };
    auto tracebacks = [&](hipStream_t st, uint32_t workers, uint32_t first, uint32_t n, uint32_t lq_off, uint32_t sybase) {
        hipLaunchKernelGGL(pgm_tb_kernel, dim3(workers), dim3(64 * PGM_WAVES), 0, st, b->d_jobs, b->d_tblist + first, n, b->d_sync, b->test_spin_limit, lq_off, sybase, 1u);
    };
    if (critk) sweep(sc, S.ncrit_workers, b->d_items, S.ncrit, S.crit_c3, (uint32_t)PGM_SY_CRIT_TICKET);
    if (nrest != 0) sweep(sr, S.nworkers, b->d_items + S.ncrit, nrest, S.rest_c3, 1u);
    if ((e = hipGetLastError()) != hipSuccess) return e;
    if (fork) {
        hipLaunchKernelGGL((pgm_lean_kernel<2>), dim3(S.nlean_workers), dim3(64 * PGM_WAVES), 0, ctx->stream2, b->d_jobs, b->d_lean, S.nlean, b->d_sync, spin_limit);
        if ((e = hipGetLastError()) != hipSuccess) return e;
    }
    const uint32_t njp = (b->njobs + 3u) / 4u * 4u;
    if (bandk) {
        hipLaunchKernelGGL(pgm_band_kernel, dim3(S.nband_workers), dim3(64 * PGM_WAVES), 0, ctx->stream3, b->d_jobs, b->d_bands, S.nbands_narrow, S.nbands, S.nband_workers - S.nwide_workers, b->d_sync, spin_limit, stall_job, stall_band);
        if ((e = hipGetLastError()) != hipSuccess) return e;
        if (tbk && S.ntb_b) tracebacks(ctx->stream3, S.ntb_b_workers, S.ntb + S.ntb_c, S.ntb_b, b->lq_off + njp, 8u);
        if ((e = hipGetLastError()) != hipSuccess) return e;
        if ((e = hipEventRecord(b->ev_join_b, ctx->stream3)) != hipSuccess) return e;
    }
    if (critk) {
        if (tbk && S.ntb_c) tracebacks(sc, S.ncrit_workers, S.ntb, S.ntb_c, b->lq_off + 2 * njp, 16u);
        if ((e = hipGetLastError()) != hipSuccess) return e;
    }
    if (tbk && S.ntb) {
        tracebacks(sr, S.ntb_workers, 0u, S.ntb, b->lq_off, 0u);
        if ((e = hipGetLastError()) != hipSuccess) return e;
    }
    if (critk && (e = hipEventRecord(b->ev_join_c, ctx->stream4)) != hipSuccess) return e;
    if (bandk && (e = hipStreamWaitEvent(s, b->ev_join_b, 0)) != hipSuccess) return e;
    if (critk && (e = hipStreamWaitEvent(s, b->ev_join_c, 0)) != hipSuccess) return e;
    if (fork && ((e = hipEventRecord(b->ev_join, ctx->stream2)) != hipSuccess || (e = hipStreamWaitEvent(s, b->ev_join, 0)) != hipSuccess)) return e;
    if (timed && (e = hipEventRecord(b->ev[3], s)) != hipSuccess) return e;
    if (timed && (e = hipEventRecord(b->ev[4], s)) != hipSuccess) return e;
    return hipSuccess;
}
struct SmallLayout { size_t sync, jobs, order, items, lean, tblist, bands, times, tabhdr, total_bands; bool any_lean; };
static SmallLayout layout_small(pgm_align_batch *b) {
    SmallLayout s;
    const uint32_t njobs = b->njobs;
    s.total_bands = 0; s.any_lean = false;
    for (const PgmJob &J : b->jobs) { s.total_bands += J.nb; s.any_lean = s.any_lean || (J.lean && !J.keep_cells); }
    DevLayout SM;
    s.sync = SM.take(b->sync_ints * sizeof(int)); s.jobs = SM.take(sizeof(PgmJob) * std::max(1u, njobs));
    s.order = SM.take(4 * (size_t)std::max(1u, njobs)); s.items = SM.take(sizeof(PgmItem) * std::max<size_t>(1, s.total_bands));
    s.lean = SM.take(4 * (size_t)std::max(1u, njobs)); s.tblist = SM.take(8 * (size_t)std::max(1u, njobs));
    s.bands = SM.take(sizeof(PgmItem) * std::max<size_t>(1, s.total_bands)); s.times = SM.take(16 * (size_t)std::max(1u, njobs) + 16);
    s.tabhdr = SM.take(s.any_lean ? 4 * (size_t)PGM_TAB_HDR * njobs : 16);
    b->small_bytes = SM.bytes;
    return s;
}

static double now_ms() { return std::chrono::duration<double, std::milli>(std::chrono::steady_clock::now().time_since_epoch()).count(); }

struct BatchAlloc {
    std::atomic<int> state{0};
    hipError_t err = hipSuccess, host_err = hipSuccess;
    uint8_t *h_out_dev = nullptr;
    double ms_dev = 0, ms_host = 0, ms_slot[6] = {0, 0, 0, 0, 0, 0};
};
static void take_batch_buffers(pgm_ctx *ctx, pgm_align_batch *b, SmallLayout sm, BatchAlloc *A) {
    const double ta0 = now_ms();
    hipError_t e2 = hipSetDevice(ctx->device);
    double tprev = ta0;
    for (int k = 0; k < 6 && e2 == hipSuccess; ++k) {
        const BatchBuffer &s = kBatchBuffers[k];
        e2 = cache_take(ctx, s.slot, b->*s.bytes, (void **)&(b->*s.ptr), &b->cap[s.slot]);
        const double t = now_ms(); A->ms_slot[k] = t - tprev; tprev = t;
    }
    if (e2 == hipSuccess) {
        b->d_sync = (int *)(b->d_small + sm.sync);
        b->d_jobs = (PgmJob *)(b->d_small + sm.jobs);
        b->d_order = (uint32_t *)(b->d_small + sm.order);
        b->d_items = (PgmItem *)(b->d_small + sm.items);
        b->d_lean = (uint32_t *)(b->d_small + sm.lean);
        b->d_tblist = (int2 *)(b->d_small + sm.tblist);
        b->d_bands = (PgmItem *)(b->d_small + sm.bands);
        b->d_times = (unsigned long long *)(b->d_small + sm.times);
        b->d_tabhdr = sm.any_lean ? (int *)(b->d_small + sm.tabhdr) : nullptr;
    }
    A->err = e2;
    A->state.store(e2 == hipSuccess ? 1 : -1, std::memory_order_release);
    A->ms_dev = now_ms() - ta0;
    if (e2 == hipSuccess) {
        hipError_t e3 = cache_take(ctx, pgm_ctx::C_HOST, b->out_bytes + 64, (void **)&b->h_out, &b->cap[pgm_ctx::C_HOST]);
        if (e3 == hipSuccess) b->h_flag = (int *)(b->h_out + (b->out_bytes + 15) / 16 * 16);
        if (e3 == hipSuccess) e3 = hipHostGetDevicePointer((void **)&A->h_out_dev, b->h_out, 0);
        A->host_err = e3;
    }
    A->ms_host = now_ms() - ta0 - A->ms_dev;
}

struct CreateGuard {
    pgm_ctx *ctx;
    pgm_align_batch *b;
    std::thread alloc;
    ~CreateGuard() { if (alloc.joinable()) alloc.join(); if (b) pgm_align_batch_destroy(ctx, b); }
    pgm_align_batch *release() { pgm_align_batch *r = b; b = nullptr; return r; }
};

static void bind_job_pointers(pgm_align_batch *b, const std::vector<JobOff> &off, const pgm_site_ref *res1, const pgm_site_ref *res2, uint8_t *h_out_dev) {
    for (uint32_t i = 0; i < b->njobs; ++i) {
        PgmJob &J = b->jobs[i];
        const JobOff &o = off[i];
        uint8_t *in = b->d_in, *w = b->d_work, *ob = b->d_out;
        J.sites1 = site_ref_of(res1, i) ? res1[i].dev_sites : (const double *)(in + o.s1.sites);
        J.sites2 = site_ref_of(res2, i) ? res2[i].dev_sites : (const double *)(in + o.s2.sites);
        J.smap1 = o.s1.has_smap ? (const uint32_t *)(in + o.s1.smap) : nullptr;
        J.smap2 = o.s2.has_smap ? (const uint32_t *)(in + o.s2.smap) : nullptr;
        J.M = (const double *)(in + o.M); J.pi = (const double *)(in + o.pi);
        J.ni1 = (const PgmNode2 *)(in + o.s1.ni); J.ni2 = (const PgmNode2 *)(in + o.s2.ni);
        J.xp1 = (const int32_t *)(in + o.s1.xp); J.xp2 = (const int32_t *)(in + o.s2.xp);
        J.xc1 = (const uint32_t *)(in + o.s1.xc); J.xc2 = (const uint32_t *)(in + o.s2.xc);
        J.xv1 = (const float *)(in + o.s1.xv); J.xv2 = (const float *)(in + o.s2.xv);
        J.fp1 = (const int32_t *)(in + o.s1.fp); J.fe1 = (const uint2 *)(in + o.s1.fe);
        J.ov2 = (const uint2 *)(in + o.s2.ov);
        J.pp1 = (const int32_t *)(in + o.s1.pp); J.pp2 = (const int32_t *)(in + o.s2.pp);
        J.pc1 = (const uint32_t *)(in + o.s1.pc); J.pc2 = (const uint32_t *)(in + o.s2.pc);
        J.pv1 = (const float *)(in + o.s1.pv); J.pv2 = (const float *)(in + o.s2.pv);
        J.pu1 = (const uint32_t *)(in + o.s1.pu); J.pu2 = (const uint32_t *)(in + o.s2.pu);
        J.g1f = (float *)(w + o.g1f); J.a1 = (float *)(w + o.a1);
        J.t2 = (float *)(w + o.t2); J.b2 = (float *)(w + o.aux2);
        J.map1 = (uint32_t *)(ob + o.map1); J.map2 = (uint32_t *)(ob + o.map2);
        J.mark_score = (float *)(w + o.ms); J.mark_prev = (uint32_t *)(w + o.mp);
        J.tb1 = (PgmTbNode *)(w + o.tb1); J.tb2 = (PgmTbNode *)(w + o.tb2);
        J.result = (PgmJob::Result *)(ob + o.res);
        J.hmap1 = (uint32_t *)(h_out_dev + o.map1); J.hmap2 = (uint32_t *)(h_out_dev + o.map2);
        J.hresult = (PgmJob::Result *)(h_out_dev + o.res);
        J.cells = (float4 *)(b->d_cells + o.cells);
        J.codes = (uint32_t *)(w + o.codes);
        J.endcell = (float4 *)(w + o.endcell);
        if (J.lean && !J.keep_cells && b->d_tabhdr) { J.cls1 = w + o.cls; J.cls2 = w + o.cls + J.n1; J.tabhdr = b->d_tabhdr + (size_t)PGM_TAB_HDR * i; }
        else { J.cls1 = nullptr; J.cls2 = nullptr; J.tabhdr = nullptr; }
        J.S = (float *)(b->d_S + o.S);
        J.prog = b->d_sync + o.prog;
        J.ltab = (uint16_t *)(w + o.ltab); J.lready = b->d_sync + o.lready; J.lrows = o.lrows; J.lcols = o.lcols;
        J.times = b->d_times + 2 * (size_t)i;
    }
}

static std::vector<uint32_t> size_order(const std::vector<PgmJob> &jobs) {
    std::vector<uint32_t> order(jobs.size());
    std::iota(order.begin(), order.end(), 0u);
    std::stable_sort(order.begin(), order.end(), [&](uint32_t x, uint32_t y) { return (uint64_t)jobs[x].n1 * jobs[x].n2 > (uint64_t)jobs[y].n1 * jobs[y].n2; });
    return order;
}
}

extern "C" {

int pgm_test_cu_shares(uint32_t cus, double lean_cost, uint32_t nlean, double band_cost, uint32_t nbands, double rest_cost, uint32_t nrest,
                       uint32_t ncrit, double longest_chain, uint32_t *out4) {
    if (!out4) return fail(PGM_ERR_INVALID, "null argument");
    const CuShares r = cu_shares(cus, lean_cost, nlean, band_cost, nbands, rest_cost, nrest, ncrit, longest_chain);
    out4[0] = r.lean; out4[1] = r.band; out4[2] = r.crit; out4[3] = r.rest;
    return PGM_OK;
}

int pgm_test_batch_plan(uint32_t njobs, const pgm_graph *const *g1, const pgm_graph *const *g2, const pgm_model *const *model,
                        const pgm_scores *scores, uint32_t flags, const pgm_site_ref *res1, const pgm_site_ref *res2, uint32_t cus,
                        uint32_t *head, double *dhead, uint32_t *job_fields, uint32_t *items, uint32_t *bands, uint32_t *lean_list, int32_t *tblist) {
    if (!head || !dhead || !items || !bands || (njobs && (!g1 || !g2 || !model || !scores || !job_fields || !lean_list || !tblist))) return fail(PGM_ERR_INVALID, "null argument");
    std::vector<char> two_chains(njobs, 0);
    for (uint32_t i = 0; i < njobs; ++i) two_chains[i] = job_is_two_chains(g1[i], g2[i]) ? 1 : 0;
    std::vector<PgmJob> jobs;
    BatchSizes Z;
    const int invalid = plan_sizes(njobs, g1, g2, model, scores, flags, res1, res2, two_chains, cus, jobs, Z);
    if (invalid >= 0) return fail(PGM_ERR_INVALID, "invalid job " + std::to_string(invalid));
    std::vector<uint8_t> image(std::max<size_t>(Z.in_base[njobs], 16));
    for (uint32_t i = 0; i < njobs; ++i)
        if (!plan_flatten_job(image.data(), Z.in_base[i], Z.in_base[i + 1], g1[i], g2[i], model[i], site_ref_of(res1, i), site_ref_of(res2, i), Z.pro, jobs[i], Z.off[i]))
            return fail(PGM_ERR_INVALID, "invalid graph in job " + std::to_string(i));
    const BatchSchedule S = plan_schedule(jobs, size_order(jobs), cus);
    const uint32_t h[PGM_PLAN_HEAD] = {njobs ? Z.pro.batch_dp : 0u, Z.pro.promote_bands, S.nitems, S.ncrit, S.nbands, S.nbands_narrow, S.nlean, S.ntb, S.ntb_c, S.ntb_b,
                                       S.nworkers, S.nlean_workers, S.nband_workers, S.nwide_workers, S.ncrit_workers, S.ntb_workers, S.ntb_b_workers,
                                       S.crit_c3, S.rest_c3, S.capacity, (uint32_t)S.total_b, (uint32_t)S.total, (uint32_t)S.total_c};
    const double d[PGM_PLAN_DHEAD] = {S.rsweep, S.t_goal, S.lean_cost, S.band_cost, S.band_end, S.other_cost, S.fill_end, S.crit_end, Z.pro.longest_crit_chain};
    memcpy(head, h, sizeof h);
    memcpy(dhead, d, sizeof d);
    for (uint32_t i = 0; i < njobs; ++i) {
        const PgmJob &J = jobs[i];
        const uint32_t f[PGM_PLAN_JOB] = {J.lean, J.has_extras, J.mode2, J.hD, J.hDX, J.slot_bytes, J.aux_off, J.ov_off, J.rh_off, J.c3_off, J.nov2, J.has_far, J.long1, J.long2,
                                          J.crit3, J.far_slack, J.nslots, Z.off[i].s1.ngeneric + Z.off[i].s2.ngeneric, Z.off[i].s1.nkill + Z.off[i].s2.nkill};
        memcpy(job_fields + (size_t)PGM_PLAN_JOB * i, f, sizeof f);
    }
    if (S.nitems) memcpy(items, S.items.data(), sizeof(PgmItem) * S.nitems);
    if (S.nbands) memcpy(bands, S.bands.data(), sizeof(PgmItem) * S.nbands);
    if (S.nlean) memcpy(lean_list, S.lean_list.data(), 4 * (size_t)S.nlean);
    if (S.ntb + S.ntb_c + S.ntb_b) memcpy(tblist, S.tblist.data(), 8 * (size_t)(S.ntb + S.ntb_c + S.ntb_b));
    return PGM_OK;
}

int pgm_align_batch_create(pgm_ctx *ctx, uint32_t njobs, const pgm_graph *const *g1, const pgm_graph *const *g2,
                           const pgm_model *const *model, const pgm_scores *scores, pgm_align_batch **out) {
    return pgm_align_batch_create_ex(ctx, njobs, g1, g2, model, scores, 0u, out);
}

int pgm_align_batch_create_ex(pgm_ctx *ctx, uint32_t njobs, const pgm_graph *const *g1, const pgm_graph *const *g2,
                              const pgm_model *const *model, const pgm_scores *scores, uint32_t flags, pgm_align_batch **out) {
    return pgm_align_batch_create_res(ctx, njobs, g1, g2, model, scores, flags, nullptr, nullptr, out);
}

int pgm_align_batch_create_res(pgm_ctx *ctx, uint32_t njobs, const pgm_graph *const *g1, const pgm_graph *const *g2,
                               const pgm_model *const *model, const pgm_scores *scores, uint32_t flags,
                               const pgm_site_ref *res1, const pgm_site_ref *res2, pgm_align_batch **out) {
    if (!ctx || !out || (njobs && (!g1 || !g2 || !model || !scores))) return fail(PGM_ERR_INVALID, "null argument");
    *out = nullptr;
    HIPCHK(hipSetDevice(ctx->device));
    const double tcs = now_ms();
    const bool cprof = getenv("PGM_HOST_PROFILE") != nullptr;
    const uint32_t cus = (uint32_t)ctx->prop.multiProcessorCount;
    BatchAlloc A;
    CreateGuard G{ctx, new pgm_align_batch, {}};
    pgm_align_batch *b = G.b;
    b->njobs = njobs;
    std::vector<char> two_chains(njobs, 0);
    (void)lib_pool().run(njobs, njobs >= 16 ? 16u : 1u, [&](size_t i) { two_chains[i] = job_is_two_chains(g1[i], g2[i]) ? 1 : 0; });
    BatchSizes Z;
    const int invalid = plan_sizes(njobs, g1, g2, model, scores, flags, res1, res2, two_chains, cus, b->jobs, Z);
    if (invalid >= 0) return fail(PGM_ERR_INVALID, "invalid job " + std::to_string(invalid));
    const std::vector<size_t> &in_base = Z.in_base;
    b->maxdim = Z.maxdim; b->maxnb = Z.maxnb; b->maxn = Z.maxn; b->maxnblk = Z.maxnblk; b->cells = Z.cells;
    b->res_off.resize(njobs); b->map1_off.resize(njobs); b->map2_off.resize(njobs);
    for (uint32_t i = 0; i < njobs; ++i) { b->res_off[i] = Z.off[i].res; b->map1_off[i] = Z.off[i].map1; b->map2_off[i] = Z.off[i].map2; }
    b->in_bytes = std::max<size_t>(in_base[njobs], 16);
    b->work_bytes = std::max<size_t>(Z.L.W.bytes, 16);
    b->cell_bytes = std::max<size_t>(Z.L.C.bytes, 16);
    b->out_bytes = std::max<size_t>(Z.L.O.bytes, 16);
    b->s_bytes = std::max<size_t>(Z.L.SL.bytes, 16);
    b->lq_off = (uint32_t)Z.L.sync_ints;
    b->sync_ints = Z.L.sync_ints + 3 * (((size_t)njobs + 3) / 4 * 4);
    const double tc0 = now_ms();
    const SmallLayout sm = layout_small(b);
    G.alloc = std::thread(take_batch_buffers, ctx, b, sm, &A);
    hipError_t e;
    if ((e = cache_take(ctx, pgm_ctx::C_HIN, b->in_bytes, (void **)&b->h_in, &b->cap[pgm_ctx::C_HIN])) != hipSuccess)
        return fail(PGM_ERR_DEVICE, std::string("hipHostMalloc: ") + hipGetErrorString(e));
    const double tc1 = now_ms();
    std::atomic<int> bad(-1), upload_err((int)hipSuccess);
    const uint32_t chunk_jobs = (uint32_t)std::max<size_t>(1, ((size_t)8 << 20) / std::max<size_t>(1, in_base[njobs] / std::max(1u, njobs)));
    std::vector<std::atomic<uint32_t>> chunk_done((njobs + chunk_jobs - 1) / chunk_jobs + 1);
    for (auto &cd : chunk_done) cd.store(0);
    (void)lib_pool().run(njobs, 16, [&](size_t job_index) {
        const uint32_t i = (uint32_t)job_index;
        if (!plan_flatten_job(b->h_in, in_base[i], in_base[i + 1], g1[i], g2[i], model[i], site_ref_of(res1, i), site_ref_of(res2, i), Z.pro, b->jobs[i], Z.off[i])) { bad.store((int)i); return; }
        const uint32_t c = i / chunk_jobs, c0 = c * chunk_jobs, c1 = std::min(njobs, c0 + chunk_jobs);
        if (chunk_done[c].fetch_add(1, std::memory_order_acq_rel) + 1 == c1 - c0) {
            int st;
            while ((st = A.state.load(std::memory_order_acquire)) == 0) std::this_thread::yield();
            if (st == 1) {
                (void)hipSetDevice(ctx->device);
                const hipError_t eu = hipMemcpyAsync(b->d_in + in_base[c0], b->h_in + in_base[c0], in_base[c1] - in_base[c0], hipMemcpyHostToDevice, ctx->stream);
                if (eu != hipSuccess) upload_err.store((int)eu);
            }
        }
    });
    if (bad.load() >= 0) return fail(PGM_ERR_INVALID, "invalid graph in job " + std::to_string(bad.load()));
    const double tc2 = now_ms();
    G.alloc.join();
    const double tc3 = now_ms();
    if (A.err != hipSuccess) return fail(A.err == hipErrorOutOfMemory ? PGM_ERR_NOMEM : PGM_ERR_DEVICE, std::string("hipMalloc: ") + hipGetErrorString(A.err));
    if (A.host_err != hipSuccess) return fail(PGM_ERR_DEVICE, std::string("hipHostMalloc: ") + hipGetErrorString(A.host_err));
    bind_job_pointers(b, Z.off, res1, res2, A.h_out_dev);
    b->order = size_order(b->jobs);
    b->sched = plan_schedule(b->jobs, b->order, cus);
    const BatchSchedule &S = b->sched;
    if (cprof && njobs)
        fprintf(stderr, "    work lists: longest chain of sweeps %.0f us, goal %.0f us; lean %zu jobs %.0f us-worker on %u CUs; bands %zu, %.0f us-worker on %u CUs (simulated end %.0f us); items %zu, %.0f us-worker on %u CUs (simulated end %.0f us), of the longest chains %zu on %u CUs (%.0f us)\n",
                S.rsweep, S.t_goal, (size_t)S.nlean, S.lean_cost, S.nlean_workers, S.total_b, S.band_cost, S.nband_workers, S.band_end, S.total, S.other_cost, S.capacity, S.fill_end, S.total_c, S.ncrit_workers, S.crit_end);
    const double tc4 = now_ms();
    if (S.nitems > std::max<size_t>(1, sm.total_bands)) return fail(PGM_ERR_DEVICE, "work list longer than the number of bands");
    if ((e = (hipError_t)upload_err.load()) != hipSuccess ||
        (e = hipMemcpyAsync(b->d_tblist, S.tblist.data(), 8 * S.tblist.size(), hipMemcpyHostToDevice, ctx->stream)) != hipSuccess ||
        (e = hipMemcpyAsync(b->d_jobs, b->jobs.data(), sizeof(PgmJob) * njobs, hipMemcpyHostToDevice, ctx->stream)) != hipSuccess ||
        (e = hipMemcpyAsync(b->d_order, b->order.data(), 4 * (size_t)njobs, hipMemcpyHostToDevice, ctx->stream)) != hipSuccess ||
        (e = hipMemcpyAsync(b->d_items, S.items.data(), sizeof(PgmItem) * S.items.size(), hipMemcpyHostToDevice, ctx->stream)) != hipSuccess ||
        (e = hipMemcpyAsync(b->d_lean, S.lean_list.data(), 4 * S.lean_list.size(), hipMemcpyHostToDevice, ctx->stream)) != hipSuccess ||
        (e = hipMemcpyAsync(b->d_bands, S.bands.data(), sizeof(PgmItem) * S.bands.size(), hipMemcpyHostToDevice, ctx->stream)) != hipSuccess ||
        (e = classify_lean_jobs(ctx, b)) != hipSuccess ||
        (e = hipStreamSynchronize(ctx->stream)) != hipSuccess)
        return fail(PGM_ERR_DEVICE, std::string("upload: ") + hipGetErrorString(e));
    for (int k = 0; k < 5; ++k) (void)hipEventCreate(&b->ev[k]);
    (void)hipEventCreateWithFlags(&b->ev_fork, hipEventDisableTiming);
    (void)hipEventCreateWithFlags(&b->ev_join, hipEventDisableTiming);
    (void)hipEventCreateWithFlags(&b->ev_join_b, hipEventDisableTiming);
    (void)hipEventCreateWithFlags(&b->ev_join_c, hipEventDisableTiming);
    if (cprof)
        fprintf(stderr, "    create: sizes %.2f ms, pinned input block %.2f, flatten %.2f, wait for the allocations %.2f (device %.2f, pinned results %.2f), work list %.2f, upload of %.1f MB %.2f\n",
                tc0 - tcs, tc1 - tc0, tc2 - tc1, tc3 - tc2, A.ms_dev, A.ms_host, tc4 - tc3, b->in_bytes / 1e6, now_ms() - tc4);
    if (cprof)
        fprintf(stderr, "    device buffers: inputs %.1f MB %.2f ms, work %.1f MB %.2f, cells %.1f MB %.2f, results %.1f MB %.2f, S %.1f MB %.2f, small %.2f\n",
                b->in_bytes / 1e6, A.ms_slot[0], b->work_bytes / 1e6, A.ms_slot[1], b->cell_bytes / 1e6, A.ms_slot[2], b->out_bytes / 1e6, A.ms_slot[3], b->s_bytes / 1e6, A.ms_slot[4], A.ms_slot[5]);
    *out = G.release();
    return PGM_OK;
}

int pgm_align_batch_run(pgm_ctx *ctx, pgm_align_batch *b) {
    if (!ctx || !b) return fail(PGM_ERR_INVALID, "null argument");
    if (b->njobs == 0) return PGM_OK;
    HIPCHK(hipSetDevice(ctx->device));
    HIPCHK(launch_all(ctx, b, true));
    b->ev_pending = true;
    return PGM_OK;
}

int pgm_align_batch_time(pgm_ctx *ctx, pgm_align_batch *b, int reps, float *ms_prep, float *ms_emission, float *ms_fill,
                         float *ms_traceback) {
    if (!ctx || !b || reps <= 0) return fail(PGM_ERR_INVALID, "bad argument");
    HIPCHK(hipSetDevice(ctx->device));
    double acc[4] = {0, 0, 0, 0};
    for (int r = 0; r < reps && b->njobs; ++r) {
        HIPCHK(launch_all(ctx, b, true));
        b->ev_pending = false;
        HIPCHK(hipEventSynchronize(b->ev[4]));
        for (int k = 0; k < 4; ++k) {
            float ms = 0;
            HIPCHK(hipEventElapsedTime(&ms, b->ev[k], b->ev[k + 1]));
            acc[k] += ms;
        }
    }
    if (ms_prep) *ms_prep = (float)(acc[0] / reps);
    if (ms_emission) *ms_emission = (float)(acc[1] / reps);
    if (ms_fill) *ms_fill = (float)(acc[2] / reps);
    if (ms_traceback) *ms_traceback = (float)(acc[3] / reps);
    return PGM_OK;
}

int pgm_align_batch_job_times(pgm_ctx *ctx, pgm_align_batch *b, uint64_t *ticks) {
    if (!ctx || !b || !ticks) return fail(PGM_ERR_INVALID, "null argument");
    HIPCHK(hipSetDevice(ctx->device));
    HIPCHK(hipStreamSynchronize(ctx->stream));
    if (b->njobs) HIPCHK(hipMemcpy(ticks, b->d_times, 16 * (size_t)b->njobs, hipMemcpyDeviceToHost));
    return PGM_OK;
}

int pgm_align_batch_fetch(pgm_ctx *ctx, pgm_align_batch *b, pgm_align_out *out) {
    if (!ctx || !b || (b->njobs && !out)) return fail(PGM_ERR_INVALID, "null argument");
    HIPCHK(hipSetDevice(ctx->device));
    if (b->njobs == 0) { HIPCHK(hipStreamSynchronize(ctx->stream)); return PGM_OK; }
    int rc = PGM_OK;
    HIPCHK(hipMemcpyAsync(b->h_flag, b->d_sync, sizeof(int), hipMemcpyDeviceToHost, ctx->stream));
    std::vector<uint8_t> copied(b->njobs, 0);
    auto collect = [&]() -> int {
        uint32_t n = 0;
        for (uint32_t i = 0; i < b->njobs; ++i) {
            if (copied[i]) { ++n; continue; }
            const PgmJob::Result *hr = (const PgmJob::Result *)(b->h_out + b->res_off[i]);
            const int32_t st = __atomic_load_n(&hr->status, __ATOMIC_ACQUIRE);
            if (st == PGM_STATUS_PENDING) continue;
            if (!out[i].map1 || !out[i].map2) return -1;
            const uint32_t len = hr->len;
            if (len > b->jobs[i].n1 + b->jobs[i].n2) return -2;
            out[i].score = hr->score; out[i].n_tr_indels = hr->n_tr_indels; out[i].len = len; out[i].status = st;
            memcpy(out[i].map1, b->h_out + b->map1_off[i], 4 * (size_t)len);
            memcpy(out[i].map2, b->h_out + b->map2_off[i], 4 * (size_t)len);
            copied[i] = 1; ++n;
        }
        return (int)n;
    };
    for (;;) {
        const int n = collect();
        if (n < 0) { (void)hipStreamSynchronize(ctx->stream); return fail(n == -1 ? PGM_ERR_INVALID : PGM_ERR_DEVICE, n == -1 ? "null mapping buffer" : "corrupt result length"); }
        if ((uint32_t)n == b->njobs) break;
        const hipError_t q = hipStreamQuery(ctx->stream);
        if (q == hipSuccess) break;
        if (q != hipErrorNotReady) return fail(PGM_ERR_DEVICE, std::string("fill kernel: ") + hipGetErrorString(q));
    }
    HIPCHK(hipStreamSynchronize(ctx->stream));
    if (b->ev_pending) {
        b->ev_pending = false;
        float ms[3] = {0, 0, 0};
        bool ok = true;
        for (int k = 0; k < 3; ++k) ok = ok && hipEventElapsedTime(&ms[k], b->ev[k], b->ev[k + 1]) == hipSuccess;
        if (ok) { for (int k = 0; k < 3; ++k) b->acc_ms[k] += ms[k]; ++b->acc_n; }
        else (void)hipGetLastError();
    }
    const int aborted = *b->h_flag;
    if (aborted) return fail(PGM_ERR_DEVICE, "fill kernel: a band hand-off timed out");
    for (uint32_t i = 0; i < b->njobs; ++i) {
        PgmJob::Result res;
        memcpy(&res, b->h_out + b->res_off[i], sizeof res);
        if (res.status == PGM_STATUS_PENDING) return fail(PGM_ERR_DEVICE, "fill kernel: a job's result record was never written");
        if (res.status != PGM_OK) rc = res.status;
        if (copied[i]) continue;
        out[i].score = res.score;
        out[i].n_tr_indels = res.n_tr_indels;
        out[i].len = res.len;
        out[i].status = res.status;
        if (res.status != PGM_OK) rc = res.status;
        if (!out[i].map1 || !out[i].map2) return fail(PGM_ERR_INVALID, "null mapping buffer");
        if (res.len > b->jobs[i].n1 + b->jobs[i].n2) return fail(PGM_ERR_DEVICE, "corrupt result length");
        memcpy(out[i].map1, b->h_out + b->map1_off[i], 4 * (size_t)res.len);
        memcpy(out[i].map2, b->h_out + b->map2_off[i], 4 * (size_t)res.len);
    }
    if (rc != PGM_OK) g_err = "backtracking failed";
    return rc;
}

void pgm_align_batch_destroy(pgm_ctx *ctx, pgm_align_batch *b) {
    if (!b) return;
    if (ctx) { (void)hipSetDevice(ctx->device); (void)hipStreamSynchronize(ctx->stream); }
    if (ctx && ctx->stream2) (void)hipStreamSynchronize(ctx->stream2);
    if (ctx && ctx->stream3) (void)hipStreamSynchronize(ctx->stream3);
    if (ctx && ctx->stream4) (void)hipStreamSynchronize(ctx->stream4);
    for (int k = 0; k < 5; ++k)
        if (b->ev[k]) (void)hipEventDestroy(b->ev[k]);
    if (b->ev_fork) (void)hipEventDestroy(b->ev_fork);
    if (b->ev_join) (void)hipEventDestroy(b->ev_join);
    if (b->ev_join_b) (void)hipEventDestroy(b->ev_join_b);
    if (b->ev_join_c) (void)hipEventDestroy(b->ev_join_c);
    for (const BatchBuffer &e : kBatchBuffers) cache_give(ctx, e.slot, b->*e.ptr, b->cap[e.slot]);
    cache_give(ctx, pgm_ctx::C_HOST, b->h_out, b->cap[pgm_ctx::C_HOST]);
    cache_give(ctx, pgm_ctx::C_HIN, b->h_in, b->cap[pgm_ctx::C_HIN]);
    delete b;
}

uint64_t pgm_align_batch_cells(const pgm_align_batch *b) { return b ? b->cells : 0; }

int pgm_align_batch_stage_times(pgm_align_batch *b, int reset, float *ms_prep, float *ms_emission, float *ms_fill, uint32_t *launches) {
    if (!b) return fail(PGM_ERR_INVALID, "null batch");
    const double n = b->acc_n ? (double)b->acc_n : 1.0;
    if (ms_prep) *ms_prep = (float)(b->acc_ms[0] / n);
    if (ms_emission) *ms_emission = (float)(b->acc_ms[1] / n);
    if (ms_fill) *ms_fill = (float)(b->acc_ms[2] / n);
    if (launches) *launches = b->acc_n;
    if (reset) { b->acc_ms[0] = b->acc_ms[1] = b->acc_ms[2] = 0; b->acc_n = 0; }
    return PGM_OK;
}

int pgm_align_batch_test_stall(pgm_align_batch *b, uint32_t job, uint32_t band, uint32_t spin_limit) {
    if (!b) return fail(PGM_ERR_INVALID, "null batch");
    b->test_stall_job = job; b->test_stall_band = band; b->test_spin_limit = spin_limit;
    return PGM_OK;
}

int pgm_align_graphs_batch(pgm_ctx *ctx, uint32_t njobs, const pgm_graph *const *g1, const pgm_graph *const *g2,
                           const pgm_model *const *model, const pgm_scores *scores, pgm_align_out *out) {
    return pgm_align_graphs_batch_res(ctx, njobs, g1, g2, model, scores, nullptr, nullptr, out);
}

int pgm_align_graphs_batch_res(pgm_ctx *ctx, uint32_t njobs, const pgm_graph *const *g1, const pgm_graph *const *g2,
                               const pgm_model *const *model, const pgm_scores *scores, const pgm_site_ref *res1, const pgm_site_ref *res2,
                               pgm_align_out *out) {
    pgm_align_batch *b = nullptr;
    const bool prof = getenv("PGM_HOST_PROFILE") != nullptr;
    const auto t0 = std::chrono::steady_clock::now();
    int rc = pgm_align_batch_create_res(ctx, njobs, g1, g2, model, scores, 0u, res1, res2, &b);
    if (rc != PGM_OK) return rc;
    const auto t1 = std::chrono::steady_clock::now();
    {
        static std::mutex device_turn[64];
        std::lock_guard<std::mutex> turn(device_turn[(unsigned)ctx->device % 64u]);
        rc = pgm_align_batch_run(ctx, b);
        if (rc == PGM_OK) rc = pgm_align_batch_fetch(ctx, b, out);
    }
    const auto t2 = std::chrono::steady_clock::now();
    pgm_align_batch_destroy(ctx, b);
    if (prof)
        fprintf(stderr, "  pgm_align_graphs_batch: %u jobs, create (flatten, allocate, upload, work list) %.2f ms, run + fetch %.2f ms, destroy %.2f ms\n", njobs,
                std::chrono::duration<double, std::milli>(t1 - t0).count(), std::chrono::duration<double, std::milli>(t2 - t1).count(),
                std::chrono::duration<double, std::milli>(std::chrono::steady_clock::now() - t2).count());
    return rc;
}

int pgm_align_batch_read_matrices(pgm_ctx *ctx, pgm_align_batch *b, uint32_t job, float *M, float *X, float *Y, float *W, float *S) {
    if (!ctx || !b || job >= b->njobs) return fail(PGM_ERR_INVALID, "bad argument");
    HIPCHK(hipSetDevice(ctx->device));
    HIPCHK(hipStreamSynchronize(ctx->stream));
    const PgmJob &J = b->jobs[job];
    const size_t N = (size_t)J.n1 * J.n2;
    if ((M || X || Y || W) && !J.keep_cells)
        return fail(PGM_ERR_INVALID, "the DP matrices of a chain-only job are only kept for a batch created with PGM_BATCH_KEEP_MATRICES");
    if (S && J.tabhdr) {
        int bad = 1;
        HIPCHK(hipMemcpy(&bad, J.tabhdr, sizeof(int), hipMemcpyDeviceToHost));
        if (bad == 0) return fail(PGM_ERR_INVALID, "the score matrix of a job of two sequence graphs is only stored for a batch created with PGM_BATCH_KEEP_MATRICES");
    }
    if (M || X || Y || W) {
        const uint32_t sh = J.rshift, R = 1u << sh;
        const size_t ncell = (size_t)J.nb * J.tsteps * 64u * R;
        std::vector<float4> cells(ncell);
        HIPCHK(hipMemcpy(cells.data(), J.cells, ncell * sizeof(float4), hipMemcpyDeviceToHost));
        float *dst[4] = {M, X, Y, W};
        for (int k = 0; k < 4; ++k)
            if (dst[k]) std::fill(dst[k], dst[k] + N, -INFINITY);
        for (uint32_t y = 0; y + 1 < J.n1; ++y)
            for (uint32_t x = 0; x < J.ncol; ++x) {
                const uint32_t bb = y >> (6u + sh), w = y & ((64u << sh) - 1u), l = w >> sh, r = w & (R - 1u);
                const float4 c = cells[((((size_t)bb * J.tsteps + (x + l)) << sh) | r) * 64u + l];
                const size_t i = (size_t)y + (size_t)J.n1 * x;
                if (M) M[i] = c.x;
                if (X) X[i] = c.y;
                if (Y) Y[i] = c.w;
                if (W) W[i] = c.z;
            }
    }
    if (S) {
        const uint32_t sh = J.rshift, R = 1u << sh;
        const size_t ns = (size_t)J.nb * J.nblk * 64u * PGM_BLOCK * R;
        std::vector<float> sk(ns);
        HIPCHK(hipMemcpy(sk.data(), J.S, ns * sizeof(float), hipMemcpyDeviceToHost));
        std::fill(S, S + N, 0.0f);
        for (uint32_t y = 0; y + 1 < J.n1; ++y)
            for (uint32_t x = 0; x < J.ncol; ++x) {
                const uint32_t bb = y >> (6u + sh), w = y & ((64u << sh) - 1u), l = w >> sh, r = w & (R - 1u), t = x + l;
                S[(size_t)y + (size_t)J.n1 * x] = sk[(((((size_t)bb * J.nblk + t / PGM_BLOCK) << sh) | r) * 64u + l) * PGM_BLOCK + t % PGM_BLOCK];
            }
    }
    return PGM_OK;
}

}

#include "pgm_nw_capi.inc"
#include "pgm_csprofile_capi.inc"
#include "pgm_dist_capi.inc"
#include "pgm_merge_capi.inc"
#include "pgm_parsimony_capi.inc"
#include "pgm_wls_capi.inc"
#include "pgm_bionj_capi.inc"
#include "pgm_agreement_capi.inc"
#include "pgm_transfer_capi.inc"
#include "pgm_transfer_taxa_capi.inc"
```

prographmsa_amd/csrc/pgm_device.h:

```cpp
#ifndef PGM_DEVICE_H_
#define PGM_DEVICE_H_

#include <stdint.h>
#include "../../include/pgm_hip.h"

#define PGM_MAX_DIM 64
#define PGM_HALO 0
#define PGM_ROWS 64
#define PGM_VL 16
#define PGM_BLOCK 8
#define PGM_NRING 128
#define PGM_KF 4
#define PGM_KF8 8
#define PGM_DCAP 28
#define PGM_PF 4
#define PGM_REMOTE_MAX 128
#define PGM_WAVES 8
#define PGM_WIDE_WAVES 4
#define PGM_POOL 163584
#define PGM_CPARTS 3
#define PGM_AUX_RES 0
#define PGM_AUX_SBLK 3072
#define PGM_AUX_EL 9216
#define PGM_AUX_CNT 13312
#define PGM_AUX_BYTES 13328

#define PGM_NF_COUNT 15u
#define PGM_NF_GENERIC 16u
#define PGM_NF_KILL 32u
#define PGM_NF_NLONG(f) (((f) >> 16) & 3u)
#define PGM_NF_NOV(f) (((f) >> 20) & 31u)
#define PGM_NF_OVI(f) (((f) >> 25) & 127u)
#define PGM_OV_ENT 16
#define PGM_OV_REC 128
#define PGM_NLONG 3
struct PgmNode2 {
    float cc, c2, c3;
    uint32_t flags;
    uint32_t fd[PGM_KF8];
    float fc[PGM_KF8];
};

#define PGM_TB_PK 8
struct PgmTbNode {
    uint32_t cnt;
    uint32_t c[PGM_TB_PK];
    float v[PGM_TB_PK];
    uint32_t u[PGM_TB_PK];
    uint32_t pad[7];
};

struct PgmJob {
    uint32_t n1, n2;
    uint32_t dim, dp;
    uint32_t nb;
    uint32_t ncol;
    uint32_t tsteps;
    uint32_t maxn;
    uint32_t has_extras;
    uint32_t has_far;
    uint32_t mode2;
    uint32_t far_slack;
    uint32_t aux_off;
    uint32_t hD, hDX;
    uint32_t slot_bytes;
    uint32_t nslots;
    uint32_t rshift;
    uint32_t lean;
    uint32_t crit3;
    uint32_t c3_off;
    uint32_t long1, long2;
    pgm_scores sc;

    const double *sites1, *sites2;
    const uint32_t *smap1, *smap2;
    const double *M, *pi;
    const PgmNode2 *ni1, *ni2;
    const int32_t *xp1, *xp2;
    const uint32_t *xc1, *xc2;
    const float *xv1, *xv2;
    const int32_t *fp1;
    const uint2 *fe1;
    const uint2 *ov2;
    uint32_t nov2, ov_off;
    uint32_t rh_off;
    const int32_t *pp1, *pp2;
    const uint32_t *pc1, *pc2;
    const float *pv1, *pv2;
    const uint32_t *pu1, *pu2;

    PgmTbNode *tb1, *tb2;
    float *g1f;
    float *a1;
    float *t2;
    float *b2;

    float *S;
    uint32_t nblk;
    const uint8_t *cls1, *cls2;
    int *tabhdr;

    uint32_t *codes;
    float4 *endcell;
    uint32_t keep_cells;

    uint16_t *ltab;
    int *lready;
    uint32_t lrows, lcols;

    unsigned long long *times;

    float4 *cells;
    int *prog;

    uint32_t *map1, *map2;
    float *mark_score;
    uint32_t *mark_prev;
    struct Result { float score; uint32_t n_tr_indels; uint32_t len; int32_t status; } *result;
    uint32_t *hmap1, *hmap2;
    Result *hresult;
};


#define PGM_SY_BAND_TICKET 3
#define PGM_SY_CRIT_TICKET 4
#define PGM_SY_WIDE_TICKET 5
#define PGM_SY_LQ_N 32
#define PGM_SY_TB_DONE 33
#define PGM_SY_TBQ_N 34
#define PGM_LK_W 4u
#define PGM_LK_T 32u
#define PGM_LK_NR 4u
#define PGM_LK_MIN_ROWS 1216u
#define PGM_LK_H 16u
#define PGM_LK_TAB (3u * PGM_LK_T * PGM_LK_T)
__host__ __device__ inline uint32_t pgm_lk_first(uint32_t n1, uint32_t n2, uint32_t lcols, uint32_t r) {
    const uint32_t w = lcols < PGM_LK_W ? lcols : PGM_LK_W;
    const uint64_t xc = ((uint64_t)(PGM_LK_T * r + PGM_LK_T / 2u) * (n2 - 1u)) / (n1 - 1u);
    const uint32_t g = (uint32_t)(xc / PGM_LK_T);
    const uint32_t lo = g >= w / 2u ? g - w / 2u : 0u;
    return lo + w > lcols ? lcols - w : lo;
}

struct PgmItem {
    uint32_t job, band;
    uint32_t prio, count;
};

#endif
```

prographmsa_amd/csrc/pgm_plan.h:

```cpp
#ifndef PGM_PLAN_H_
#define PGM_PLAN_H_

#include <hip/hip_vector_types.h>

#include <algorithm>
#include <cmath>
#include <cstring>
#include <numeric>
#include <queue>
#include <vector>

#include "pgm_device.h"

namespace {

constexpr double kTauChain = 0.45;
constexpr double kTauExtras = 0.65;
constexpr double kTauMode2 = 0.6;
constexpr double kTauCrit = 0.42;
constexpr double kTauLean = 0.34;
constexpr double kEager = 0.7;
constexpr double kLag = PGM_ROWS + 3.0 * PGM_BLOCK;
constexpr double kLagCritEst = 80.0;
constexpr double kLagWideEst = 78.0;
constexpr uint32_t kNarrowSlot = PGM_POOL / PGM_WAVES / 16 * 16;
constexpr uint32_t kWideSlot = PGM_POOL / PGM_WIDE_WAVES / 16 * 16;
constexpr uint32_t kMode2MinBands = 20u, kMode2MinHd = 32u;
constexpr uint32_t kC3Bytes = 4096 + 6 * 2048;
constexpr uint32_t kOvBytes = 8u * PGM_OV_REC * PGM_OV_ENT;
inline uint32_t row_bands(uint32_t n) { return (n - 1 + PGM_ROWS - 1) / PGM_ROWS; }
inline uint32_t alphabet_tier(uint32_t dim) { return dim <= 4 ? 4u : dim <= 20 ? 20u : 64u; }

struct Arena {
    uint8_t *base = nullptr;
    size_t off = 0, end = 0;
    bool overflow = false;
    size_t put(const void *src, size_t bytes, size_t align = 16) {
        const size_t o = (off + align - 1) / align * align;
        if (o + bytes > end) { overflow = true; return 0; }
        off = o + bytes;
        if (src && bytes) memcpy(base + o, src, bytes);
        return o;
    }
};
struct DevLayout {
    size_t bytes = 0;
    size_t take(size_t b, size_t align = 256) {
        size_t off = (bytes + align - 1) / align * align;
        bytes = off + b;
        return off;
    }
};

struct SideOff {
    size_t sites, ni, xp, xc, xv, pp, pc, pv, pu, fp, fe, ov;
    size_t smap = 0;
    bool has_smap = false;
    uint32_t nodes_with_extras;
    uint32_t has_long;
    uint32_t maxd_cap;
    uint32_t maxd_kf8;
    uint32_t far_nodes;
    uint32_t maxd;
    uint32_t far_dmin;
    uint32_t remote;
    uint32_t nov;
    uint32_t ngeneric;
    uint32_t nkill;
    std::vector<uint32_t> cp, cd;
    std::vector<float> cv;
};

static int flatten_side(const pgm_graph *g, const pgm_scores &sc, Arena &A, SideOff &o, const pgm_site_ref *res = nullptr) {
    const uint32_t n = g->n;
    const bool resident = res && res->dev_sites;
    if (n < 2 || (!g->sites && !resident) || !g->e_rowptr) return PGM_ERR_INVALID;
    static thread_local std::vector<float> xv, pv;
    static thread_local std::vector<int32_t> xp, pp;
    static thread_local std::vector<uint32_t> xc, pc, pu;
    static thread_local std::vector<PgmNode2> ni;
    xv.clear(); pv.clear(); xc.clear(); pc.clear(); pu.clear();
    xp.assign(n + 1, 0); pp.assign(n + 1, 0);
    ni.resize(n);
    o.nodes_with_extras = 0; o.has_long = 0; o.maxd_cap = 1; o.maxd_kf8 = 1; o.nkill = 0;
    o.cp.assign(n + 1, 0); o.cd.clear(); o.cv.clear();
    for (uint32_t v = 0; v < n; ++v) {
        PgmNode2 &I = ni[v];
        memset(&I, 0, sizeof I);
        I.cc = I.c2 = I.c3 = INFINITY;
        for (int k = 0; k < PGM_KF8; ++k) I.fc[k] = INFINITY;
        auto place = [&](uint32_t from, float val) {
            const uint32_t d = v - from;
            if (d == 1 && I.cc == INFINITY && val != INFINITY) { I.cc = val; return; }
            xc.push_back(from); xv.push_back(val);
            if (val == INFINITY) return;
            if (d <= (uint32_t)PGM_DCAP) o.maxd_cap = std::max(o.maxd_cap, d); else o.has_long = 1;
            if (d == 2 && I.c2 == INFINITY) { I.c2 = val; return; }
            if (d == 3 && I.c3 == INFINITY) { I.c3 = val; return; }
            o.cd.push_back(d); o.cv.push_back(val);
        };
        const int32_t eb = g->e_rowptr[v], ee = g->e_rowptr[v + 1];
        if (eb > ee || eb < 0) return PGM_ERR_INVALID;
        for (int32_t e = eb; e < ee; ++e) {
            const uint32_t from = g->e_col[e];
            if (from >= v) return PGM_ERR_INVALID;
            const float c = g->e_val[e];
            const float val = (c == 0) ? INFINITY : c + 10000.0f;
            pc.push_back(from); pv.push_back(val); pu.push_back(0u);
            place(from, val);
        }
        if (g->r_rowptr) {
            if (g->r_rowptr[v] > g->r_rowptr[v + 1] || g->r_rowptr[v] < 0) return PGM_ERR_INVALID;
            for (int32_t e = g->r_rowptr[v]; e < g->r_rowptr[v + 1]; ++e) {
                const uint32_t from = g->r_col[e];
                if (from >= v) return PGM_ERR_INVALID;
                const uint32_t units = g->r_units[e];
                const float val = (units == 0) ? INFINITY : sc.repeat_init + sc.repeat_ext * (float)(units - 1);
                pc.push_back(from); pv.push_back(val); pu.push_back(0x80000000u | units);
                place(from, val);
            }
        }
        xp[v + 1] = (int32_t)xc.size();
        pp[v + 1] = (int32_t)pc.size();
        o.cp[v + 1] = (uint32_t)o.cd.size();
        {
            uint32_t dm = I.c3 != INFINITY ? 3u : (I.c2 != INFINITY ? 2u : 1u);
            bool small = o.cp[v + 1] - o.cp[v] <= (uint32_t)PGM_KF8;
            for (uint32_t k = o.cp[v]; k < o.cp[v + 1] && small; ++k) { if (o.cd[k] > (uint32_t)PGM_DCAP) small = false; else dm = std::max(dm, o.cd[k]); }
            if (small) o.maxd_kf8 = std::max(o.maxd_kf8, dm);
        }
        if (v > 0 && v + 1 < n && pp[v + 1] == pp[v]) { I.flags |= PGM_NF_KILL; ++o.nkill; }
        o.nodes_with_extras += (xp[v + 1] > xp[v]);
    }
    if (xc.empty()) { xc.push_back(0); xv.push_back(0); }
    if (pc.empty()) { pc.push_back(0); pv.push_back(0); pu.push_back(0); }
    o.smap = 0; o.has_smap = false;
    if (resident) {
        if (res->ncols == 0 || (!res->node_map && n > res->ncols)) return PGM_ERR_INVALID;
        if (res->node_map) for (uint32_t v = 0; v < n; ++v) if (res->node_map[v] >= res->ncols) return PGM_ERR_INVALID;
        o.sites = 0;
        if (res->node_map) { o.smap = A.put(res->node_map, 4 * (size_t)n); o.has_smap = true; }
    } else o.sites = A.put(g->sites, sizeof(double) * (size_t)g->dim * n);
    o.ni = A.put(ni.data(), sizeof(PgmNode2) * ni.size());
    o.xp = A.put(xp.data(), 4 * xp.size());
    o.xc = A.put(xc.data(), 4 * xc.size());
    o.xv = A.put(xv.data(), 4 * xv.size());
    o.pp = A.put(pp.data(), 4 * pp.size());
    o.pc = A.put(pc.data(), 4 * pc.size());
    o.pv = A.put(pv.data(), 4 * pv.size());
    o.pu = A.put(pu.data(), 4 * pu.size());
    o.fp = A.put(nullptr, 4 * ((size_t)n + 1));
    o.fe = A.put(nullptr, 8 * std::max<size_t>(1, o.cd.size()));
    o.ov = A.put(nullptr, 8 * (size_t)PGM_OV_REC * PGM_OV_ENT);
    return PGM_OK;
}

static void finalize_side(uint8_t *base, uint32_t n, SideOff &o, int side, bool mode2, bool allow_long, bool allow_ov) {
    PgmNode2 *ni = (PgmNode2 *)(base + o.ni);
    int32_t *fp = (int32_t *)(base + o.fp);
    uint2 *fe = (uint2 *)(base + o.fe), *ov = (uint2 *)(base + o.ov);
    o.nov = 0;
    o.far_nodes = 0; o.maxd = 1; o.far_dmin = PGM_DCAP + 1; o.remote = 0; o.ngeneric = 0;
    uint32_t band_entries = 0, band_remote = 0, nfe = 0;
    fp[0] = 0;
    for (uint32_t v = 0; v < n; ++v) {
        PgmNode2 &I = ni[v];
        const uint32_t kill = I.flags & PGM_NF_KILL;
        const uint32_t c0 = o.cp[v], c1 = o.cp[v + 1], nc = c1 - c0;
        if (side == 0 && (v & 63u) == 0) { band_entries = 0; band_remote = 0; }
        uint32_t dmax = 1, nloc = 0, nrem = 0, novf = 0, ovi = 0;
        if (I.c2 != INFINITY) dmax = 2;
        if (I.c3 != INFINITY) dmax = 3;
        bool generic = false;
        if (!mode2) {
            if (nc > (uint32_t)PGM_KF) generic = true;
            for (uint32_t k = c0; k < c1 && !generic; ++k) {
                if (o.cd[k] > (uint32_t)PGM_DCAP) { generic = true; break; }
                I.fd[nloc] = o.cd[k]; I.fc[nloc] = o.cv[k]; ++nloc;
                dmax = std::max(dmax, o.cd[k]);
                o.far_dmin = std::min(o.far_dmin, o.cd[k]);
            }
        } else if (side == 0) {
            const uint32_t lane = v & 63u;
            for (uint32_t k = c0; k < c1; ++k) nrem += (o.cd[k] > (uint32_t)PGM_DCAP || o.cd[k] > lane + (uint32_t)PGM_VL);
            if (band_entries + nc > 512u || band_remote + nrem > (uint32_t)PGM_REMOTE_MAX || nc > 255u || (nrem && !allow_long)) generic = true;
            else {
                for (uint32_t k = c0; k < c1; ++k) {
                    const uint32_t d = o.cd[k];
                    const bool rem = d > (uint32_t)PGM_DCAP || d > lane + (uint32_t)PGM_VL;
                    fe[nfe++] = make_uint2(d | (rem ? 0x80000000u : 0u), __builtin_bit_cast(uint32_t, o.cv[k]));
                    if (!rem) { dmax = std::max(dmax, d); o.far_dmin = std::min(o.far_dmin, d); ++nloc; }
                }
                band_entries += nc; band_remote += nrem;
            }
        } else {
            for (uint32_t k = c0; k < c1; ++k) nrem += o.cd[k] > (uint32_t)PGM_DCAP;
            const uint32_t nl_all = nc - nrem, ring_cap = (uint32_t)PGM_KF8 - std::min(nrem, (uint32_t)PGM_KF8);
            novf = nl_all > ring_cap ? nl_all - ring_cap : 0u;
            if (nrem > (uint32_t)PGM_NLONG || (nrem && !allow_long) || novf > (uint32_t)PGM_OV_ENT || (novf && (o.nov >= (uint32_t)PGM_OV_REC || !allow_ov))) generic = true;
            else {
                uint2 *rec = ov + (size_t)o.nov * PGM_OV_ENT;
                uint32_t nl = 0, no = 0;
                for (uint32_t k = c0; k < c1; ++k) {
                    const uint32_t d = o.cd[k];
                    if (d > (uint32_t)PGM_DCAP) { I.fd[PGM_KF8 - 1 - nl] = d; I.fc[PGM_KF8 - 1 - nl] = o.cv[k]; ++nl; continue; }
                    if (nloc < ring_cap) { I.fd[nloc] = d; I.fc[nloc] = o.cv[k]; ++nloc; }
                    else rec[no++] = make_uint2(d, __builtin_bit_cast(uint32_t, o.cv[k]));
                    dmax = std::max(dmax, d); o.far_dmin = std::min(o.far_dmin, d);
                }
                if (novf) { ovi = o.nov++; for (; no < (uint32_t)PGM_OV_ENT; ++no) rec[no] = make_uint2(1u, __builtin_bit_cast(uint32_t, (float)INFINITY)); }
            }
        }
        fp[v + 1] = (int32_t)nfe;
        if (generic) {
            I.c2 = I.c3 = INFINITY;
            for (int k = 0; k < PGM_KF8; ++k) { I.fd[k] = 0; I.fc[k] = INFINITY; }
            I.flags = PGM_NF_GENERIC | (1u << 8) | kill;
            ++o.ngeneric;
        } else {
            const bool rows2 = mode2 && side == 0;
            I.flags = (rows2 ? 0u : nloc) | (dmax << 8) | kill | ((mode2 && side == 1) ? (nrem << 16) | (novf << 20) | (ovi << 25) : 0u);
            o.maxd = std::max(o.maxd, dmax);
            o.far_nodes += (nloc + nrem) != 0;
            o.remote += nrem;
        }
    }
}

struct JobOff { SideOff s1, s2; size_t M, pi, g1f, a1, t2, aux2, map1, map2, ms, mp, res, cells, tb1, tb2, S, prog, codes, endcell, ltab, lready, cls; uint32_t lrows, lcols; };
struct BatchLayout { DevLayout W, C, O, SL; size_t sync_ints = 64; };
static void layout_job(BatchLayout &L, uint32_t n1, uint32_t n2, uint32_t dp, uint32_t rshift, bool lean, bool keep, JobOff &o) {
    const uint32_t R = 1u << rshift, rows = PGM_ROWS * R;
    const uint32_t nb = (n1 - 1 + rows - 1) / rows, tsteps = (n2 - 1) + 63;
    const uint32_t nblk = (tsteps + PGM_BLOCK - 1) / PGM_BLOCK, maxn = std::max(n1, n2);
    o.g1f = L.W.take(sizeof(float) * (size_t)dp * n1);
    o.a1 = L.W.take(sizeof(float) * n1);
    o.t2 = L.W.take(sizeof(float) * (size_t)dp * n2);
    o.aux2 = L.W.take(sizeof(float) * (size_t)n2);
    o.map1 = L.O.take(4 * (size_t)(n1 + n2), 16);
    o.map2 = L.O.take(4 * (size_t)(n1 + n2), 16);
    o.tb1 = L.W.take(sizeof(PgmTbNode) * (size_t)n1);
    o.tb2 = L.W.take(sizeof(PgmTbNode) * (size_t)n2);
    o.ms = L.W.take(4 * (size_t)maxn);
    o.mp = L.W.take(4 * (size_t)maxn);
    o.res = L.O.take(sizeof(PgmJob::Result), 16);
    o.cells = L.C.take(keep ? sizeof(float4) * (size_t)nb * tsteps * 64u * R : 16, 1024);
    o.codes = L.W.take(lean ? 4 * (size_t)nb * nblk * 64u * R : 16);
    o.endcell = L.W.take(16, 16);
    o.cls = L.W.take((lean && !keep) ? (size_t)n1 + n2 : 16, 16);
    o.S = L.SL.take(sizeof(float) * (size_t)nb * nblk * 64u * PGM_BLOCK * R, 1024);
    o.prog = L.sync_ints;
    L.sync_ints += (nb + 3) / 4 * 4;
    o.lrows = (!lean && n1 - 1 >= PGM_LK_MIN_ROWS && n2 - 1 >= 4 * PGM_LK_T) ? (n1 - 1 + PGM_LK_T - 1) / PGM_LK_T : 0u;
    o.lcols = (n2 - 1 + PGM_LK_T - 1) / PGM_LK_T;
    o.ltab = L.W.take(std::max<size_t>((size_t)o.lrows * PGM_LK_W * PGM_LK_TAB * 2, 16), 256);
    o.lready = L.sync_ints;
    L.sync_ints += ((size_t)o.lrows + 2 + 3) / 4 * 4;
}
static bool graph_is_chain(const pgm_graph *g) {
    if (g->r_rowptr && g->r_rowptr[g->n] != 0) return false;
    if (g->e_rowptr[0] != 0 || g->e_rowptr[1] != 0) return false;
    for (uint32_t v = 1; v < g->n; ++v) {
        const int32_t eb = g->e_rowptr[v], ee = g->e_rowptr[v + 1];
        if (eb < 0 || ee - eb != 1 || g->e_col[eb] != v - 1 || g->e_val[eb] == 0.0f) return false;
    }
    return true;
}


static size_t side_bound_bytes(size_t n, size_t dim, size_t E) {
    E = std::max<size_t>(E, 1);
    return n * dim * 8 + n * sizeof(PgmNode2) + 3 * (n + 1) * 4 + E * 28 + 8 * (size_t)PGM_OV_REC * PGM_OV_ENT + 16 * 16;
}
static size_t model_bound_bytes(size_t dim) { return (dim * dim + dim) * 8 + 64; }

static const pgm_site_ref *site_ref_of(const pgm_site_ref *r, uint32_t i) { return (r && r[i].dev_sites) ? &r[i] : nullptr; }
static bool job_is_two_chains(const pgm_graph *a, const pgm_graph *c) {
    return a && c && a->n >= 2 && c->n >= 2 && a->e_rowptr && c->e_rowptr && a->e_col && c->e_col && a->e_val && c->e_val && graph_is_chain(a) && graph_is_chain(c);
}

struct BatchPrologue {
    uint32_t batch_dp = 4u;
    double longest_crit_chain = 0.0;
    uint32_t promote_bands = 0xffffffffu;
};
static BatchPrologue plan_batch_prologue(const std::vector<PgmJob> &jobs, uint32_t cus) {
    BatchPrologue P;
    uint32_t batch_dim = 0;
    double crit_load = 0.0;
    for (const PgmJob &J : jobs) {
        batch_dim = std::max(batch_dim, J.dim);
        P.longest_crit_chain = std::max(P.longest_crit_chain, ((double)(row_bands(J.n1) - 1) * kLagCritEst + (double)(J.n2 - 1 + 63)) * kTauCrit);
        if (!J.lean) crit_load += (double)row_bands(J.n1) * (double)(J.n2 - 1 + 63) * kTauCrit;
    }
    P.batch_dp = alphabet_tier(batch_dim);
    if (crit_load <= 1.25 * (double)cus * P.longest_crit_chain) P.promote_bands = 8u;
    return P;
}

struct BatchSizes {
    BatchPrologue pro;
    BatchLayout L;
    std::vector<JobOff> off;
    std::vector<size_t> in_base;
    uint32_t maxdim = 0, maxnb = 0, maxn = 0, maxnblk = 0;
    uint64_t cells = 0;
};
static int plan_sizes(uint32_t njobs, const pgm_graph *const *g1, const pgm_graph *const *g2, const pgm_model *const *model, const pgm_scores *scores,
                      uint32_t flags, const pgm_site_ref *res1, const pgm_site_ref *res2, const std::vector<char> &two_chains, uint32_t cus,
                      std::vector<PgmJob> &jobs, BatchSizes &Z) {
    auto side_bound = [](const pgm_graph *g, const pgm_site_ref *res) -> size_t {
        const size_t n = g->n;
        size_t E = (size_t)std::max(0, g->e_rowptr ? g->e_rowptr[n] : 0);
        if (g->r_rowptr) E += (size_t)std::max(0, g->r_rowptr[n]);
        const size_t full = side_bound_bytes(n, g->dim, E);
        return (res && res->dev_sites) ? full - n * g->dim * 8 + n * 4 + 16 : full;
    };
    jobs.resize(njobs);
    Z.off.resize(njobs);
    Z.in_base.assign(njobs + 1, 0);
    for (uint32_t i = 0; i < njobs; ++i) {
        const pgm_graph *a = g1[i], *c = g2[i];
        if (!a || !c || !model[i] || a->dim != c->dim || a->dim == 0 || a->dim > PGM_MAX_DIM || a->n < 2 || c->n < 2 || !model[i]->M || !model[i]->pi ||
            (!a->sites && !site_ref_of(res1, i)) || !a->e_rowptr || (!c->sites && !site_ref_of(res2, i)) || !c->e_rowptr)
            return (int)i;
        PgmJob &J = jobs[i];
        memset(&J, 0, sizeof J);
        J.n1 = a->n; J.n2 = c->n; J.dim = a->dim;
        J.ncol = c->n - 1;
        J.tsteps = J.ncol + 63;
        constexpr uint32_t lean_rshift = 1u;
        J.lean = (two_chains[i] && ((uint64_t)J.tsteps * 1024u << lean_rshift) < (1ull << 30)) ? 1u : 0u;
        J.rshift = J.lean ? lean_rshift : 0u;
        J.nb = (a->n - 1 + (PGM_ROWS << J.rshift) - 1) / (PGM_ROWS << J.rshift);
        J.nblk = (J.tsteps + PGM_BLOCK - 1) / PGM_BLOCK;
        J.maxn = std::max(a->n, c->n);
        J.sc = scores[i];
        J.keep_cells = (!J.lean || (flags & PGM_BATCH_KEEP_MATRICES)) ? 1u : 0u;
        Z.maxnblk = std::max(Z.maxnblk, J.nblk);
        Z.maxn = std::max(Z.maxn, J.maxn);
        Z.maxdim = std::max(Z.maxdim, a->dim);
        Z.maxnb = std::max(Z.maxnb, J.nb << J.rshift);
        Z.cells += (uint64_t)(a->n - 2) * (c->n - 2);
        Z.in_base[i + 1] = Z.in_base[i] + side_bound(a, site_ref_of(res1, i)) + side_bound(c, site_ref_of(res2, i)) + model_bound_bytes(a->dim);
    }
    Z.pro = plan_batch_prologue(jobs, cus);
    for (uint32_t i = 0; i < njobs; ++i) {
        PgmJob &J = jobs[i];
        J.dp = Z.pro.batch_dp;
        layout_job(Z.L, J.n1, J.n2, J.dp, J.rshift, J.lean != 0, J.keep_cells != 0, Z.off[i]);
    }
    return -1;
}

static bool plan_job_sweep(PgmJob &J, uint8_t *base, SideOff &s1, SideOff &s2, const BatchPrologue &P) {
    J.has_extras = (s1.nodes_with_extras + s2.nodes_with_extras) > 0 ? 1u : 0u;
    if (J.lean && J.has_extras) return false;
    uint32_t hD = 16, hDX = 4;
    while (hD < s1.maxd_kf8 + s2.maxd_kf8 + (uint32_t)PGM_BLOCK) hD *= 2;
    while (hDX < s2.maxd_kf8 + 1) hDX *= 2;
    auto slot_head = [&](bool mode2) { return 2u * hD * (64u + PGM_VL) * 4u + hDX * 64u * 4u + PGM_NRING * (mode2 ? 80u : 48u); };
    const uint32_t nb_job = row_bands(J.n1);
    const bool allow_long = (uint64_t)J.nb * J.tsteps * 1024u < (1ull << 32);
    const bool has_long = (s1.has_long | s2.has_long) != 0 && allow_long;
    const double far_density = 0.5 * ((double)s1.cp[J.n1] / J.n1 + (double)s2.cp[J.n2] / J.n2);
    const double chain_wide = ((double)(nb_job - 1) * kLagWideEst + (double)(J.n2 - 1 + 63)) * (0.7 + 10.0 * far_density);
    const bool fits_wide = slot_head(false) <= kWideSlot && chain_wide <= 0.9 * P.longest_crit_chain;
    J.mode2 = (J.has_extras && ((hD >= kMode2MinHd && !fits_wide) || nb_job >= kMode2MinBands || nb_job >= P.promote_bands || has_long)) ? 1u : 0u;
    const bool mode2 = J.mode2 != 0;
    if (mode2) {
        while (hD < s1.maxd_cap + s2.maxd_cap + (uint32_t)PGM_BLOCK) hD *= 2;
        while (hDX < s2.maxd_cap + 1) hDX *= 2;
    }
    const uint32_t aux_bytes = mode2 ? (uint32_t)PGM_AUX_BYTES : 0u;
    finalize_side(base, J.n1, s1, 0, mode2, allow_long, false);
    finalize_side(base, J.n2, s2, 1, mode2, allow_long, slot_head(mode2) + aux_bytes + kOvBytes <= (uint32_t)PGM_POOL);
    J.nov2 = mode2 ? s2.nov : 0u;
    J.has_far = (s1.far_nodes + s2.far_nodes) > 0 ? 1u : 0u;
    J.long1 = (mode2 && s1.remote) ? 1u : 0u;
    J.long2 = (mode2 && s2.remote) ? 1u : 0u;
    const bool c3 = mode2 && !J.long1 && !J.long2 && J.nov2 == 0 && s1.ngeneric + s2.ngeneric == 0 && s1.nkill + s2.nkill == 0 &&
                    slot_head(true) + aux_bytes + kC3Bytes <= (uint32_t)PGM_POOL;
    if (c3 && hDX < 8u) hDX = 8u;
    J.hD = hD; J.hDX = hDX;
    J.slot_bytes = slot_head(mode2);
    J.aux_off = J.slot_bytes;
    J.slot_bytes += aux_bytes;
    J.ov_off = J.slot_bytes;
    if (J.nov2) J.slot_bytes += kOvBytes;
    J.rh_off = J.slot_bytes;
    if (J.long1 | J.long2) J.slot_bytes += 3u * 32u * 64u * 4u;
    J.c3_off = J.slot_bytes;
    J.crit3 = (c3 && J.slot_bytes + kC3Bytes <= (uint32_t)PGM_POOL) ? 1u : 0u;
    if (J.crit3) J.slot_bytes += kC3Bytes;
    J.far_slack = std::max(1u, std::min(4u, std::min(s1.far_dmin, s2.far_dmin)));
    J.nslots = mode2 ? 1u : std::max(1u, std::min((uint32_t)PGM_WAVES, (uint32_t)PGM_POOL / J.slot_bytes));
    if (J.lean) J.nslots = PGM_WAVES;
    return true;
}

static bool plan_flatten_job(uint8_t *base, size_t lo, size_t hi, const pgm_graph *a, const pgm_graph *c, const pgm_model *m,
                             const pgm_site_ref *r1, const pgm_site_ref *r2, const BatchPrologue &P, PgmJob &J, JobOff &o) {
    Arena A;
    A.base = base; A.off = lo; A.end = hi;
    if (flatten_side(a, J.sc, A, o.s1, r1) != PGM_OK || flatten_side(c, J.sc, A, o.s2, r2) != PGM_OK) return false;
    if (!plan_job_sweep(J, base, o.s1, o.s2, P)) return false;
    o.M = A.put(m->M, sizeof(double) * J.dim * J.dim);
    o.pi = A.put(m->pi, sizeof(double) * J.dim);
    return !A.overflow;
}


struct CuShares { uint32_t lean, band, crit, rest, rest_need; double t_goal, fl, fb; };
static CuShares cu_shares(uint32_t cus, double lean_cost, uint32_t nlean, double band_cost, uint32_t nbands, double rest_cost, uint32_t nrest, uint32_t ncrit, double rsweep) {
    CuShares r = {0u, 0u, 0u, 0u, 0u, 0.0, 1.0, 1.0};
    cus = std::max(1u, cus);
    const uint32_t queues = (nlean != 0) + (nbands != 0) + (nrest != 0);
    if (ncrit != 0 && cus > queues) r.crit = std::min(std::min(ncrit, cus / 2u), cus - queues);
    const uint32_t cap = std::max(1u, cus - r.crit);
    const double sum = (nlean ? lean_cost : 0.0) + (nbands ? band_cost : 0.0) + (nrest ? rest_cost : 0.0);
    const double t_par = std::max(1e-3, sum / cap);
    r.t_goal = std::max(std::max(rsweep, t_par), 1e-3);
    const double w = std::min(1.0, std::max(0.0, (rsweep / t_par - 1.0) / 0.5));
    r.fl = 1.0 - 0.4 * w; r.fb = 1.0 - 0.25 * w;
    auto need = [](double cost, double t, uint32_t most) { return (uint32_t)std::min<double>(most, std::max(1.0, std::ceil(cost / t))); };
    const uint32_t band_most = (nbands + PGM_WAVES - 1) / PGM_WAVES;
    uint32_t lean = nlean ? need(lean_cost, r.fl * r.t_goal, nlean) : 0u, band = nbands ? need(band_cost, r.fb * r.t_goal, band_most) : 0u;
    uint32_t rest = nrest ? need(rest_cost, r.t_goal, nrest) : 0u;
    if (lean + band + rest > cap) {
        const double scale = (double)cap / (double)(lean + band + rest);
        auto cut = [&](uint32_t v) { return v ? std::max(1u, (uint32_t)std::floor(v * scale)) : 0u; };
        lean = cut(lean); band = cut(band); rest = cut(rest);
        while (lean + band + rest > cap) {
            uint32_t *big = &rest; if (band > *big) big = &band; if (lean > *big) big = &lean;
            if (*big <= 1u) break;
            --*big;
        }
    }
    r.rest_need = rest;
    const uint32_t left = cap > lean + band + rest ? cap - lean - band - rest : 0u;
    if (nrest) rest = std::min(nrest, rest + left);
    else if (nbands) band = std::min(band_most, band + left);
    else if (nlean) lean = std::min(nlean, lean + left);
    r.lean = lean; r.band = band; r.rest = rest;
    return r;
}

struct BatchSchedule {
    std::vector<PgmItem> items;
    std::vector<PgmItem> bands;
    std::vector<uint32_t> lean_list;
    std::vector<int2> tblist;
    uint32_t nitems = 0, nbands = 0, nlean = 0;
    uint32_t ncrit = 0, nbands_narrow = 0, ntb = 0, ntb_c = 0, ntb_b = 0;
    uint32_t nworkers = 0, nlean_workers = 0, nband_workers = 0, nwide_workers = 0, ncrit_workers = 0, ntb_workers = 0, ntb_b_workers = 0;
    bool crit_c3 = false, rest_c3 = false;
    double rsweep = 0, t_goal = 0, lean_cost = 0, band_cost = 0, band_end = 0, other_cost = 0, fill_end = 0, crit_end = 0;
    size_t total_b = 0, total = 0, total_c = 0;
    uint32_t capacity = 0;
};

struct SimItem { double rem, dur, gap; uint32_t job, band, count; };
static double simulate_workers(const std::vector<std::vector<SimItem>> &pj, size_t count, uint32_t workers, double rmax, std::vector<PgmItem> &out) {
    out.clear();
    double end = 0.0;
    typedef std::pair<double, uint32_t> TE;
    std::priority_queue<double, std::vector<double>, std::greater<double>> free_at;
    for (uint32_t w = 0; w < std::max(1u, workers); ++w) free_at.push(0.0);
    std::priority_queue<TE> ready;
    std::priority_queue<TE, std::vector<TE>, std::greater<TE>> pending;
    std::vector<uint32_t> next(pj.size(), 0);
    for (uint32_t i = 0; i < pj.size(); ++i) if (!pj[i].empty()) ready.push({pj[i][0].rem, i});
    out.reserve(count);
    double now = 0.0;
    while (out.size() < count) {
        now = std::max(now, free_at.top());
        while (!pending.empty() && pending.top().first <= now) {
            const uint32_t j = pending.top().second; pending.pop();
            ready.push({pj[j][next[j]].rem, j});
        }
        if (ready.empty()) { now = pending.top().first; continue; }
        const uint32_t j = ready.top().second; ready.pop();
        const SimItem &it = pj[j][next[j]];
        out.push_back(PgmItem{it.job, it.band, it.rem > 0.6 * rmax ? 3u : (it.rem > 0.35 * rmax ? 2u : (it.rem > 0.2 * rmax ? 1u : 0u)), it.count});
        free_at.pop();
        free_at.push(now + it.dur);
        end = std::max(end, now + it.dur);
        if (++next[j] < pj[j].size()) pending.push({pj[j][next[j]].rem > kEager * rmax ? now : now + it.gap, j});
    }
    return end;
}

static uint32_t wide_share(uint32_t cus, size_t total_b, size_t total_w, double wide_cost, double band_cost) {
    if (total_w == 0) return 0u;
    if (total_b == 0) return cus;
    const uint32_t w = (uint32_t)std::lround(cus * wide_cost / band_cost);
    return std::max(1u, std::min(cus > 1u ? cus - 1u : 1u, w));
}

static BatchSchedule plan_schedule(const std::vector<PgmJob> &jobs, const std::vector<uint32_t> &order, uint32_t cus) {
    BatchSchedule S;
    const uint32_t njobs = (uint32_t)jobs.size();
    S.capacity = cus;
    if (njobs) {
        std::vector<std::vector<SimItem>> per_job(njobs), per_job_b(njobs), per_job_c(njobs), per_job_w(njobs);
        std::vector<double> chain_of(njobs, 0.0);
        size_t total = 0, total_b = 0, total_w = 0;
        double rmax = 1.0, rsweep = 1.0;
        for (uint32_t q = 0; q < njobs; ++q) {
            const uint32_t i = order[q];
            const PgmJob &J = jobs[i];
            const double tau = J.crit3 ? kTauCrit : (J.mode2 ? kTauMode2 : (J.has_extras ? kTauExtras : kTauChain));
            const double tb = (J.has_extras ? 0.3 : 0.2) * (double)(J.n1 + J.n2);
            if (J.lean) {
                const double rounds = std::ceil((double)J.nb / PGM_WAVES), first = std::min<double>(J.nb, PGM_WAVES);
                S.lean_cost += kTauLean * (rounds * J.tsteps + (first - 1.0) * 72.0) + 0.04 * (double)(J.n1 + J.n2);
                S.lean_list.push_back(i);
                continue;
            }
            const bool narrow = !J.mode2 && J.slot_bytes <= kNarrowSlot;
            const bool wide = !J.mode2 && !narrow && J.slot_bytes <= kWideSlot;
            const bool per_band = narrow || wide;
            if (!per_band) chain_of[i] = tau * ((double)(J.nb - 1) * kLag + J.tsteps);
            const uint32_t group = per_band ? 1u : J.nslots;
            for (uint32_t band = 0; band < J.nb; band += group) {
                const uint32_t cnt = std::min(group, J.nb - band);
                SimItem it;
                it.rem = tau * ((double)(J.nb - 1 - band) * kLag + J.tsteps) + tb;
                it.dur = tau * ((double)(cnt - 1) * kLag + J.tsteps);
                it.gap = tau * (double)cnt * kLag;
                it.job = i; it.band = band; it.count = cnt;
                (wide ? per_job_w : (narrow ? per_job_b : per_job))[i].push_back(it);
                rmax = std::max(rmax, it.rem);
                rsweep = std::max(rsweep, it.rem - tb);
            }
            total += per_job[i].size();
            total_b += per_job_b[i].size();
            total_w += per_job_w[i].size();
        }
        double band_cost = 0.0, crit_cost = 0.0, wide_cost = 0.0, other_cost = 0.0;
        for (uint32_t i = 0; i < njobs; ++i) {
            for (const SimItem &it : per_job[i]) other_cost += it.dur;
            for (const SimItem &it : per_job_b[i]) band_cost += it.dur / PGM_WAVES;
            for (const SimItem &it : per_job_w[i]) wide_cost += it.dur / PGM_WIDE_WAVES;
        }
        band_cost += wide_cost;
        auto in_crit = [&](uint32_t i) { return !per_job[i].empty() && chain_of[i] >= 0.85 * rsweep; };
        size_t total_c = 0;
        if (total != 0) {
            uint32_t ncj = 0, nrestj = 0;
            for (uint32_t i = 0; i < njobs; ++i) if (!per_job[i].empty()) { if (in_crit(i)) ++ncj; else ++nrestj; }
            if (ncj != 0 && nrestj != 0)
                for (uint32_t i = 0; i < njobs; ++i)
// ... 99 lines not shown
```

Measured before the change: 81.32.

## Compute emissions per unique profile-column class and scatter from LDS table

```diff
diff --git a/include/pgm_hip.h b/include/pgm_hip.h
--- a/include/pgm_hip.h
+++ b/include/pgm_hip.h
@@ -99,6 +99,8 @@
 int pgm_test_batch_plan(uint32_t njobs, const pgm_graph *const *g1, const pgm_graph *const *g2, const pgm_model *const *model,
                         const pgm_scores *scores, uint32_t flags, const pgm_site_ref *res1, const pgm_site_ref *res2, uint32_t cus,
                         uint32_t *head, double *dhead, uint32_t *job_fields, uint32_t *items, uint32_t *bands, uint32_t *lean_list, int32_t *tblist);
+int pgm_align_batch_emission_classes(pgm_ctx *ctx, pgm_align_batch *b, uint32_t job, uint32_t *U1, uint32_t *U2, uint32_t *eligible,
+                                     uint32_t *bands_per_group, uint16_t *cls1, uint16_t *cls2);
 int pgm_align_batch_read_matrices(pgm_ctx *ctx, pgm_align_batch *b, uint32_t job, float *M,
                                   float *X, float *Y, float *W, float *S);
 
diff --git a/prographmsa_amd/__init__.py b/prographmsa_amd/__init__.py
--- a/prographmsa_amd/__init__.py
+++ b/prographmsa_amd/__init__.py
@@ -72,7 +72,7 @@
 EXPORTS = [
     "pgm_device_count", "pgm_ctx_create", "pgm_ctx_destroy", "pgm_last_error", "pgm_ctx_device_info",
     "pgm_align_graphs_batch", "pgm_align_batch_create", "pgm_align_batch_create_ex", "pgm_align_batch_create_res", "pgm_align_graphs_batch_res", "pgm_align_batch_run", "pgm_align_batch_fetch",
-    "pgm_align_batch_destroy", "pgm_align_batch_cells", "pgm_align_batch_test_stall", "pgm_test_cu_shares", "pgm_test_batch_plan", "pgm_align_batch_stage_times", "pgm_align_batch_job_times", "pgm_align_batch_time", "pgm_align_batch_read_matrices",
+    "pgm_align_batch_destroy", "pgm_align_batch_cells", "pgm_align_batch_test_stall", "pgm_test_cu_shares", "pgm_test_batch_plan", "pgm_align_batch_stage_times", "pgm_align_batch_job_times", "pgm_align_batch_time", "pgm_align_batch_read_matrices", "pgm_align_batch_emission_classes",
     "pgm_nw_pairs_batch", "pgm_nw_pairs_submit", "pgm_nw_pairs_wait", "pgm_nw_last_kernel_ms", "pgm_host_alloc", "pgm_host_free", "pgm_csprofile_load", "pgm_csprofile_create_batch", "pgm_csprofile_create_batch_res",
     "pgm_csprofile_last_kernel_ms", "pgm_mldist_batch", "pgm_prealigned_counts_batch", "pgm_kmer_cosine", "pgm_dist_last_kernel_ms",
     "pgm_kmer_cosine_multi", "pgm_prealigned_counts_multi", "pgm_prealigned_counts_resampled",
@@ -116,6 +116,7 @@
         "pgm_align_batch_job_times": (C.c_int, [vp, vp, C.POINTER(C.c_uint64)]),
         "pgm_align_batch_time": (C.c_int, [vp, vp, C.c_int] + [C.POINTER(C.c_float)] * 4),
         "pgm_align_batch_read_matrices": (C.c_int, [vp, vp, u32] + [C.POINTER(C.c_float)] * 5),
+        "pgm_align_batch_emission_classes": (C.c_int, [vp, vp, u32] + [C.POINTER(u32)] * 4 + [C.POINTER(C.c_uint16)] * 2),
         "pgm_nw_pairs_batch": (C.c_int, [vp, u32, C.POINTER(i32), i32, i32, u32, C.POINTER(C.c_int8), C.POINTER(u32), u32,
                                          C.POINTER(u32), C.POINTER(u32), C.POINTER(i32), C.POINTER(u32)]),
         "pgm_nw_pairs_submit": (C.c_int, [vp, u32, C.POINTER(i32), i32, i32, u32, C.POINTER(C.c_int8), C.POINTER(u32), u32,
diff --git a/prographmsa_amd/csrc/pgm_align_kernels.h b/prographmsa_amd/csrc/pgm_align_kernels.h
--- a/prographmsa_amd/csrc/pgm_align_kernels.h
+++ b/prographmsa_amd/csrc/pgm_align_kernels.h
@@ -159,6 +159,82 @@
     }
 }
 
+__device__ __forceinline__ uint32_t pgm_gc_word(const double *col, uint32_t k) { return __float_as_uint((float)col[k]); }
+__global__ void __launch_bounds__(256) pgm_classify_general_kernel(const PgmJob *__restrict__ jobs, uint32_t lds_budget) {
+    constexpr uint32_t HASH = 2u * PGM_GC_MAXN, EMPTY = 0xFFFFFFFFu, PER = PGM_GC_MAXN / 256u;
+    __shared__ uint32_t slots[HASH];
+    __shared__ uint16_t slot_of[PGM_GC_MAXN];
+    __shared__ uint16_t id_of[PGM_GC_MAXN];
+    __shared__ uint32_t scan[256];
+    __shared__ uint32_t nclasses[2];
+    const PgmJob &J = jobs[blockIdx.x];
+    if (!J.ghdr) return;
+    const uint32_t tid = threadIdx.x;
+    if (J.tabhdr && J.tabhdr[0] == 0) {
+        if (tid < 4) J.ghdr[tid] = 0;
+        return;
+    }
+    const uint32_t D = J.dim;
+    for (int side = 0; side < 2; ++side) {
+        const bool first = side == 0;
+        const uint32_t n = first ? J.n1 - 1u : J.n2;
+        const double *sites = first ? J.sites1 : J.sites2;
+        const uint32_t *smap = first ? J.smap1 : J.smap2;
+        uint16_t *cls = (uint16_t *)(first ? J.gcls1 : J.gcls2 + PGM_GC_PAD), *rep = (uint16_t *)(first ? J.grep1 : J.grep2);
+        for (uint32_t i = tid; i < HASH; i += 256u) slots[i] = EMPTY;
+        __syncthreads();
+        for (uint32_t v = tid; v < n; v += 256u) {
+            const double *col = sites + (size_t)D * (smap ? smap[v] : v);
+            uint32_t h = 2166136261u;
+            for (uint32_t k = 0; k < D; ++k) h = (h ^ pgm_gc_word(col, k)) * 16777619u;
+            uint32_t s = (h ^ (h >> 15)) & (HASH - 1u);
+            for (;;) {
+                const uint32_t cur = atomicCAS(&slots[s], EMPTY, v);
+                if (cur == EMPTY) break;
+                const double *other = sites + (size_t)D * (smap ? smap[cur] : cur);
+                bool same = true;
+                for (uint32_t k = 0; k < D && same; ++k) same = pgm_gc_word(col, k) == pgm_gc_word(other, k);
+                if (same) { atomicMin(&slots[s], v); break; }
+                s = (s + 1u) & (HASH - 1u);
+            }
+            slot_of[v] = (uint16_t)s;
+        }
+        __syncthreads();
+        uint32_t cnt = 0;
+        for (uint32_t v = PER * tid; v < min(n, PER * tid + PER); ++v) cnt += slots[slot_of[v]] == v ? 1u : 0u;
+        scan[tid] = cnt;
+        __syncthreads();
+        for (uint32_t d = 1; d < 256u; d <<= 1) {
+            const uint32_t add = tid >= d ? scan[tid - d] : 0u;
+            __syncthreads();
+            scan[tid] += add;
+            __syncthreads();
+        }
+        uint32_t id = scan[tid] - cnt;
+        const uint32_t U = scan[255];
+        for (uint32_t v = PER * tid; v < min(n, PER * tid + PER); ++v)
+            if (slots[slot_of[v]] == v) { id_of[v] = (uint16_t)id; rep[id] = (uint16_t)v; ++id; }
+        __syncthreads();
+        for (uint32_t v = tid; v < n; v += 256u) cls[v] = id_of[slots[slot_of[v]]];
+        if (first) {
+            if (tid == 0) cls[n] = id_of[slots[slot_of[0]]];
+        } else {
+            for (uint32_t i = tid; i < PGM_GC_PAD + PGM_GC_TAIL; i += 256u) cls[i < PGM_GC_PAD ? (int)i - (int)PGM_GC_PAD : (int)(n + i - PGM_GC_PAD)] = (uint16_t)U;
+        }
+        if (tid == 0) nclasses[side] = U;
+        __syncthreads();
+    }
+    if (tid == 0) {
+        const uint32_t U1 = nclasses[0], U2 = nclasses[1], C = U2 + 1u;
+        uint32_t sel = 0;
+        for (uint32_t g = 4; g >= 1u && sel == 0u; g >>= 1) {
+            const uint64_t L = min(64u * g, U1), e = L * C;
+            if (e * 4u <= lds_budget && 2u * e <= (uint64_t)64u * g * (J.n2 + 63u)) sel = g;
+        }
+        J.ghdr[0] = (int)sel; J.ghdr[1] = (int)U1; J.ghdr[2] = (int)U2; J.ghdr[3] = 0;
+    }
+}
+
 __device__ __forceinline__ size_t pgm_cell_index(const PgmJob &J, uint32_t y, uint32_t x) {
     const uint32_t b = y / PGM_ROWS, l = PGM_HALO + (y - b * PGM_ROWS);
     return ((size_t)b * J.tsteps + (x + l)) * 64u + l;
@@ -188,6 +264,7 @@
     const uint32_t rsh = J.rshift, nvb = J.nb << rsh;
     if (tb0 >= J.nblk || 4u * RB * blockIdx.y >= nvb) return;
     if (J.tabhdr && pgm_gld(J.tabhdr) == 0) return;
+    if (J.ghdr && pgm_gld(J.ghdr) != 0) return;
     auto row_of = [&](uint32_t v, uint32_t lane_) { return ((((v >> rsh) << 6) + lane_) << rsh) | (v & ((1u << rsh) - 1u)); };
     auto sblock_of = [&](uint32_t v, uint32_t tb_) { return ((((size_t)(v >> rsh) * J.nblk + tb_) << rsh) | (v & ((1u << rsh) - 1u))); };
     const uint32_t t0 = tb0 * PGM_BLOCK;
@@ -331,6 +408,123 @@
                 for (int q = 0; q < PGM_BLOCK / 4; ++q) dst[q] = pgm_v4f{out[r][4 * q], out[r][4 * q + 1], out[r][4 * q + 2], out[r][4 * q + 3]};
             }
         }
+    }
+}
+
+template <int DP>
+__global__ void __launch_bounds__(PGM_GC_THREADS) pgm_emission_class_kernel(const PgmJob *__restrict__ jobs) {
+    constexpr int NT = DP / 4;
+    extern __shared__ float ec_tab[];
+    uint16_t *const cx = (uint16_t *)(ec_tab + PGM_GC_LDS_BUDGET / 4u);
+    __shared__ uint16_t rcls[4 * PGM_ROWS], lcls[4 * PGM_ROWS], lrow[4 * PGM_ROWS];
+    __shared__ uint8_t isfirst[4 * PGM_ROWS];
+    const PgmJob &J = jobs[blockIdx.y];
+    if (!J.ghdr) return;
+    const uint32_t g = (uint32_t)pgm_gld(J.ghdr);
+    const uint32_t rsh = J.rshift, nvb = J.nb << rsh, v0 = g * blockIdx.x;
+    if (g == 0u || v0 >= nvb) return;
+    const uint32_t U2 = (uint32_t)pgm_gld(J.ghdr + 2), C = U2 + 1u, nblk = J.nblk;
+    const uint32_t tid = threadIdx.x, nrows = PGM_ROWS * g;
+    auto row_of = [&](uint32_t v, uint32_t lane_) { return ((((v >> rsh) << 6) + lane_) << rsh) | (v & ((1u << rsh) - 1u)); };
+    auto sblock_of = [&](uint32_t v, uint32_t tb_) { return ((((size_t)(v >> rsh) * nblk + tb_) << rsh) | (v & ((1u << rsh) - 1u))); };
+    for (uint32_t i = tid; i < PGM_GC_PAD + PGM_BLOCK * nblk; i += PGM_GC_THREADS) cx[i] = pgm_gld(J.gcls2 + i);
+    uint32_t mycls = 0xFFFFu;
+    if (tid < nrows) {
+        const uint32_t v = v0 + tid / PGM_ROWS;
+        if (v < nvb) {
+            const uint32_t y = row_of(v, tid % PGM_ROWS);
+            mycls = pgm_gld(J.gcls1 + ((y + 1 < J.n1) ? y : 0u));
+        }
+        rcls[tid] = (uint16_t)mycls;
+    }
+    __syncthreads();
+    if (tid < nrows) {
+        bool f = mycls != 0xFFFFu;
+#pragma unroll 8
+        for (uint32_t r = 0; r < nrows; ++r) f = f && (r >= tid || rcls[r] != mycls);
+        isfirst[tid] = f ? 1 : 0;
+    }
+    __syncthreads();
+    uint32_t L = 0;
+    {
+        uint32_t below = 0;
+#pragma unroll 8
+        for (uint32_t r = 0; r < nrows; ++r) {
+            const uint32_t fr = isfirst[r];
+            L += fr;
+            below += (fr != 0u && rcls[r] < mycls) ? 1u : 0u;
+        }
+        if (tid < nrows) {
+            lrow[tid] = (uint16_t)below;
+            if (isfirst[tid]) lcls[below] = (uint16_t)mycls;
+        }
+    }
+    __syncthreads();
+    {
+        const uint32_t P = PGM_GC_THREADS / L;
+        const uint32_t lr = tid % L, q = tid / L;
+        if (q < P) {
+            const uint32_t node = pgm_gld(J.grep1 + lcls[lr]);
+            const PGM_GLOBAL pgm_v4f *src = (const PGM_GLOBAL pgm_v4f *)(uintptr_t)(J.g1f + (size_t)DP * node);
+            float gy[DP];
+#pragma unroll
+            for (int k4 = 0; k4 < NT; ++k4) {
+                const pgm_v4f v = src[k4];
+                gy[4 * k4] = v.x; gy[4 * k4 + 1] = v.y; gy[4 * k4 + 2] = v.z; gy[4 * k4 + 3] = v.w;
+            }
+            const float ay = pgm_gld(J.a1 + node), mi = J.sc.match_init;
+            float *row = ec_tab + lr * C;
+            constexpr int NB = 4;
+            constexpr uint32_t NONE = 0xFFFFFFFFu;
+            auto rep_of = [&](uint32_t cc) { return cc < U2 ? (uint32_t)pgm_gld(J.grep2 + cc) : NONE; };
+            uint32_t cn[NB];
+#pragma unroll
+            for (int u = 0; u < NB; ++u) cn[u] = rep_of(q + (uint32_t)u * P);
+#pragma unroll 1
+            for (uint32_t cc0 = q; cc0 < C; cc0 += NB * P) {
+                pgm_v4f tv[NB][NT];
+                float bx[NB];
+#pragma unroll
+                for (int u = 0; u < NB; ++u) {
+                    const bool in = cn[u] != NONE;
+                    const PGM_GLOBAL pgm_v4f *tsrc = (const PGM_GLOBAL pgm_v4f *)(uintptr_t)(J.t2 + (size_t)DP * (in ? cn[u] : 0u));
+#pragma unroll
+                    for (int k4 = 0; k4 < NT; ++k4) tv[u][k4] = in ? tsrc[k4] : pgm_v4f{0.f, 0.f, 0.f, 0.f};
+                    bx[u] = in ? pgm_gld(J.b2 + cn[u]) : 0.f;
+                }
+#pragma unroll
+                for (int u = 0; u < NB; ++u) cn[u] = rep_of(cc0 + (uint32_t)(NB + u) * P);
+#pragma unroll
+                for (int u = 0; u < NB; ++u) {
+                    const uint32_t cc = cc0 + (uint32_t)u * P;
+                    float acc = 0.0f;
+#pragma unroll
+                    for (int k4 = 0; k4 < NT; ++k4) {
+                        acc = __fadd_rn(acc, __fmul_rn(gy[4 * k4], tv[u][k4].x));
+                        acc = __fadd_rn(acc, __fmul_rn(gy[4 * k4 + 1], tv[u][k4].y));
+                        acc = __fadd_rn(acc, __fmul_rn(gy[4 * k4 + 2], tv[u][k4].z));
+                        acc = __fadd_rn(acc, __fmul_rn(gy[4 * k4 + 3], tv[u][k4].w));
+                    }
+                    if (cc < C) row[cc] = pgm_emission_finish(acc, ay, bx[u], mi);
+                }
+            }
+        }
+    }
+    __syncthreads();
+    const uint32_t lane = tid % PGM_ROWS, gsh = g == 4u ? 2u : g == 2u ? 1u : 0u;
+    PGM_GLOBAL pgm_v4f *const Sq = (PGM_GLOBAL pgm_v4f *)(uintptr_t)J.S;
+#pragma unroll 1
+    for (uint32_t item = tid / PGM_ROWS; item < (nblk << gsh); item += PGM_GC_THREADS / PGM_ROWS) {
+        const uint32_t j = item & (g - 1u), tb = item >> gsh, v = v0 + j;
+        if (v >= nvb) continue;
+        const float *row = ec_tab + (uint32_t)lrow[j * PGM_ROWS + lane] * C;
+        const uint16_t *cxp = cx + (PGM_GC_PAD + tb * PGM_BLOCK - lane);
+        float out[PGM_BLOCK];
+#pragma unroll
+        for (int i = 0; i < PGM_BLOCK; ++i) out[i] = row[cxp[i]];
+        PGM_GLOBAL pgm_v4f *dst = Sq + (sblock_of(v, tb) * 64u + lane) * (PGM_BLOCK / 4);
+#pragma unroll
+        for (int q4 = 0; q4 < PGM_BLOCK / 4; ++q4) dst[q4] = pgm_v4f{out[4 * q4], out[4 * q4 + 1], out[4 * q4 + 2], out[4 * q4 + 3]};
     }
 }
 
diff --git a/prographmsa_amd/csrc/pgm_capi.hip b/prographmsa_amd/csrc/pgm_capi.hip
--- a/prographmsa_amd/csrc/pgm_capi.hip
+++ b/prographmsa_amd/csrc/pgm_capi.hip
@@ -30,6 +30,8 @@
 #include "pgm_pool.h"
 #include "pgm_plan.h"
 static_assert(kC3Bytes == PGM_C3_BYTES, "pgm_plan.h plans the LDS of a crit3 sweep with PGM_C3_BYTES");
+
+static constexpr size_t kClassLdsBytes = (size_t)PGM_GC_LDS_BUDGET + 2 * (size_t)(PGM_GC_PAD + PGM_GC_MAXN + PGM_GC_TAIL);
 
 static thread_local std::string g_err;
 static int fail(int code, const std::string &m) { g_err = m; return code; }
@@ -137,6 +139,7 @@
     PgmItem *d_bands = nullptr;
     int2 *d_tblist = nullptr;
     unsigned long long *d_times = nullptr;
+    bool class_jobs = false;
     int *d_tabhdr = nullptr;
     hipEvent_t ev_fork = nullptr, ev_join = nullptr;
     hipEvent_t ev_join_b = nullptr, ev_join_c = nullptr;
@@ -185,6 +188,8 @@
             HIPCHK(hipStreamCreateWithFlags(&c->stream4, hipStreamNonBlocking));
         }
     }
+    HIPCHK(hipFuncSetAttribute((const void *)pgm_emission_class_kernel<4>, hipFuncAttributeMaxDynamicSharedMemorySize, (int)kClassLdsBytes));
+    HIPCHK(hipFuncSetAttribute((const void *)pgm_emission_class_kernel<20>, hipFuncAttributeMaxDynamicSharedMemorySize, (int)kClassLdsBytes));
     hipLaunchKernelGGL(pgm_warm_kernel, dim3(1), dim3(64), 0, c->stream);
     HIPCHK(hipGetLastError());
     HIPCHK(hipStreamSynchronize(c->stream));
@@ -314,6 +319,15 @@
     hipLaunchKernelGGL(pgm_classify_kernel, dim3(b->njobs, 2, (b->maxn + 1023) / 1024), dim3(256), 0, ctx->stream, b->d_jobs);
     return hipGetLastError();
 }
+static bool batch_has_class_jobs(const pgm_align_batch *b) {
+    for (const PgmJob &J : b->jobs) if (J.ghdr) return true;
+    return false;
+}
+static hipError_t classify_general_jobs(pgm_ctx *ctx, pgm_align_batch *b) {
+    if (!batch_has_class_jobs(b)) return hipSuccess;
+    hipLaunchKernelGGL(pgm_classify_general_kernel, dim3(b->njobs), dim3(256), 0, ctx->stream, b->d_jobs, (uint32_t)PGM_GC_LDS_BUDGET);
+    return hipGetLastError();
+}
 
 #define PGM_STATUS_PENDING 0x7ffffff0
 struct PrepTier { uint32_t tier, threads; size_t lds; };
@@ -339,6 +353,12 @@
     else if (T.tier == 20) hipLaunchKernelGGL((pgm_emission_skew_kernel<20, 1>), eg, dim3(4 * PGM_ROWS), 0, s, b->d_jobs);
     else hipLaunchKernelGGL((pgm_emission_skew_kernel<64, 1>), eg, dim3(4 * PGM_ROWS), 0, s, b->d_jobs);
     if ((e = hipGetLastError()) != hipSuccess) return e;
+    if (b->class_jobs) {
+        const dim3 cg(b->maxnb, b->njobs);
+        if (T.tier == 4) hipLaunchKernelGGL((pgm_emission_class_kernel<4>), cg, dim3(PGM_GC_THREADS), kClassLdsBytes, s, b->d_jobs);
+        else hipLaunchKernelGGL((pgm_emission_class_kernel<20>), cg, dim3(PGM_GC_THREADS), kClassLdsBytes, s, b->d_jobs);
+        if ((e = hipGetLastError()) != hipSuccess) return e;
+    }
     if (timed && (e = hipEventRecord(b->ev[2], s)) != hipSuccess) return e;
     const uint32_t spin_limit = b->test_spin_limit ? b->test_spin_limit : PGM_SPIN_LIMIT, stall_job = b->test_stall_job, stall_band = b->test_stall_band;
     const bool fork = S.nlean != 0;
@@ -486,6 +506,12 @@
         J.endcell = (float4 *)(w + o.endcell);
         if (J.lean && !J.keep_cells && b->d_tabhdr) { J.cls1 = w + o.cls; J.cls2 = w + o.cls + J.n1; J.tabhdr = b->d_tabhdr + (size_t)PGM_TAB_HDR * i; }
         else { J.cls1 = nullptr; J.cls2 = nullptr; J.tabhdr = nullptr; }
+        if (pgm_gc_candidate(J.n1, J.n2, J.dp)) {
+            uint16_t *gw = (uint16_t *)(w + o.gcls + 16);
+            J.ghdr = (int *)(w + o.gcls);
+            J.gcls1 = gw; J.grep1 = gw + PGM_GC_R8(J.n1);
+            J.gcls2 = gw + 2u * PGM_GC_R8(J.n1); J.grep2 = J.gcls2 + PGM_GC_R8(PGM_GC_PAD + J.n2 + PGM_GC_TAIL);
+        } else { J.ghdr = nullptr; J.gcls1 = J.grep1 = J.gcls2 = J.grep2 = nullptr; }
         J.S = (float *)(b->d_S + o.S);
         J.prog = b->d_sync + o.prog;
         J.ltab = (uint16_t *)(w + o.ltab); J.lready = b->d_sync + o.lready; J.lrows = o.lrows; J.lcols = o.lcols;
@@ -616,6 +642,7 @@
     if (A.err != hipSuccess) return fail(A.err == hipErrorOutOfMemory ? PGM_ERR_NOMEM : PGM_ERR_DEVICE, std::string("hipMalloc: ") + hipGetErrorString(A.err));
     if (A.host_err != hipSuccess) return fail(PGM_ERR_DEVICE, std::string("hipHostMalloc: ") + hipGetErrorString(A.host_err));
     bind_job_pointers(b, Z.off, res1, res2, A.h_out_dev);
+    b->class_jobs = batch_has_class_jobs(b);
     b->order = size_order(b->jobs);
     b->sched = plan_schedule(b->jobs, b->order, cus);
     const BatchSchedule &S = b->sched;
@@ -632,6 +659,7 @@
         (e = hipMemcpyAsync(b->d_lean, S.lean_list.data(), 4 * S.lean_list.size(), hipMemcpyHostToDevice, ctx->stream)) != hipSuccess ||
         (e = hipMemcpyAsync(b->d_bands, S.bands.data(), sizeof(PgmItem) * S.bands.size(), hipMemcpyHostToDevice, ctx->stream)) != hipSuccess ||
         (e = classify_lean_jobs(ctx, b)) != hipSuccess ||
+        (e = classify_general_jobs(ctx, b)) != hipSuccess ||
         (e = hipStreamSynchronize(ctx->stream)) != hipSuccess)
         return fail(PGM_ERR_DEVICE, std::string("upload: ") + hipGetErrorString(e));
     for (int k = 0; k < 5; ++k) (void)hipEventCreate(&b->ev[k]);
@@ -817,6 +845,25 @@
     return rc;
 }
 
+int pgm_align_batch_emission_classes(pgm_ctx *ctx, pgm_align_batch *b, uint32_t job, uint32_t *U1, uint32_t *U2, uint32_t *eligible,
+                                     uint32_t *bands_per_group, uint16_t *cls1, uint16_t *cls2) {
+    if (!ctx || !b || job >= b->njobs) return fail(PGM_ERR_INVALID, "bad argument");
+    HIPCHK(hipSetDevice(ctx->device));
+    HIPCHK(hipStreamSynchronize(ctx->stream));
+    const PgmJob &J = b->jobs[job];
+    int hdr[4] = {0, 0, 0, 0};
+    if (J.ghdr) HIPCHK(hipMemcpy(hdr, J.ghdr, sizeof hdr, hipMemcpyDeviceToHost));
+    if (U1) *U1 = (uint32_t)hdr[1];
+    if (U2) *U2 = (uint32_t)hdr[2];
+    if (eligible) *eligible = hdr[0] != 0 ? 1u : 0u;
+    if (bands_per_group) *bands_per_group = (uint32_t)hdr[0];
+    const bool classified = J.ghdr && (hdr[1] != 0 || hdr[2] != 0);
+    if ((cls1 || cls2) && !classified) return fail(PGM_ERR_INVALID, "the job's nodes have no profile classes");
+    if (cls1) HIPCHK(hipMemcpy(cls1, J.gcls1, 2 * (size_t)J.n1, hipMemcpyDeviceToHost));
+    if (cls2) HIPCHK(hipMemcpy(cls2, J.gcls2 + PGM_GC_PAD, 2 * (size_t)J.n2, hipMemcpyDeviceToHost));
+    return PGM_OK;
+}
+
 int pgm_align_batch_read_matrices(pgm_ctx *ctx, pgm_align_batch *b, uint32_t job, float *M, float *X, float *Y, float *W, float *S) {
     if (!ctx || !b || job >= b->njobs) return fail(PGM_ERR_INVALID, "bad argument");
     HIPCHK(hipSetDevice(ctx->device));
diff --git a/prographmsa_amd/csrc/pgm_device.h b/prographmsa_amd/csrc/pgm_device.h
--- a/prographmsa_amd/csrc/pgm_device.h
+++ b/prographmsa_amd/csrc/pgm_device.h
@@ -34,6 +34,15 @@
 #define PGM_OV_ENT 16
 #define PGM_OV_REC 128
 #define PGM_NLONG 3
+#define PGM_GC_MAXN 4096u
+#define PGM_GC_PAD 64u
+#define PGM_GC_TAIL 72u
+#define PGM_GC_LDS_BUDGET 65536u
+#define PGM_GC_THREADS 512
+#define PGM_GC_R8(x) (((x) + 7u) / 8u * 8u)
+#define PGM_GC_WORDS(n1, n2) (2u * PGM_GC_R8(n1) + PGM_GC_R8(PGM_GC_PAD + (n2) + PGM_GC_TAIL) + PGM_GC_R8((n2) + 1u))
+static inline bool pgm_gc_candidate(uint32_t n1, uint32_t n2, uint32_t dp) { return dp <= 20u && n1 <= PGM_GC_MAXN && n2 <= PGM_GC_MAXN; }
+
 struct PgmNode2 {
     float cc, c2, c3;
     uint32_t flags;
@@ -100,6 +109,10 @@
     const uint8_t *cls1, *cls2;
     int *tabhdr;
 
+    int *ghdr;
+    const uint16_t *gcls1, *grep1;
+    const uint16_t *gcls2, *grep2;
+
     uint32_t *codes;
     float4 *endcell;
     uint32_t keep_cells;
diff --git a/prographmsa_amd/csrc/pgm_plan.h b/prographmsa_amd/csrc/pgm_plan.h
--- a/prographmsa_amd/csrc/pgm_plan.h
+++ b/prographmsa_amd/csrc/pgm_plan.h
@@ -227,7 +227,7 @@
     }
 }
 
-struct JobOff { SideOff s1, s2; size_t M, pi, g1f, a1, t2, aux2, map1, map2, ms, mp, res, cells, tb1, tb2, S, prog, codes, endcell, ltab, lready, cls; uint32_t lrows, lcols; };
+struct JobOff { SideOff s1, s2; size_t M, pi, g1f, a1, t2, aux2, map1, map2, ms, mp, res, cells, tb1, tb2, S, prog, codes, endcell, ltab, lready, cls, gcls; uint32_t lrows, lcols; };
 struct BatchLayout { DevLayout W, C, O, SL; size_t sync_ints = 64; };
 static void layout_job(BatchLayout &L, uint32_t n1, uint32_t n2, uint32_t dp, uint32_t rshift, bool lean, bool keep, JobOff &o) {
     const uint32_t R = 1u << rshift, rows = PGM_ROWS * R;
@@ -249,6 +249,7 @@
     o.endcell = L.W.take(16, 16);
     o.cls = L.W.take((lean && !keep) ? (size_t)n1 + n2 : 16, 16);
     o.S = L.SL.take(sizeof(float) * (size_t)nb * nblk * 64u * PGM_BLOCK * R, 1024);
+    o.gcls = L.W.take(pgm_gc_candidate(n1, n2, dp) ? 16 + 2 * (size_t)PGM_GC_WORDS(n1, n2) : 16, 16);
     o.prog = L.sync_ints;
     L.sync_ints += (nb + 3) / 4 * 4;
     o.lrows = (!lean && n1 - 1 >= PGM_LK_MIN_ROWS && n2 - 1 >= 4 * PGM_LK_T) ? (n1 - 1 + PGM_LK_T - 1) / PGM_LK_T : 0u;
```

Result: no change. 81.09 (-0.3%).
